# TrustworthyComputing/REDsec

Hardware: AMD Instinct MI355X
Metric: gate bootstraps/sec (N=1024) (higher is better)
Workload: dtype int32 torus; ring products in f64 (complex FFT, exact after rounding); 1 GPU; 65536 independent bootstrapped NAND gates per GPU per step, default128 (n=630 N=1024 l=3 Bgbit=7 t=8 basebit=2); gates_per_gpu=65536, total_gates=65536, params=default128, mode=fft, parallelism=gate-sharded x1

## Files before the change

### include/redsec_hip.h

```cpp
#ifndef REDSEC_HIP_H
#define REDSEC_HIP_H

#include <stddef.h>
#include <stdint.h>

#ifdef __cplusplus
extern "C" {
#endif

typedef enum rs_status {
  RS_OK = 0,
  RS_ERR_INVALID = -1,
  RS_ERR_NO_DEVICE = -2,
  RS_ERR_HIP = -3,
  RS_ERR_STATE = -4,
  RS_ERR_INEXACT = -5
} rs_status;

typedef struct rs_params {
  int32_t n;
  int32_t N;
  int32_t k;
  int32_t bk_l;
  int32_t bk_Bgbit;
// ... 49 lines not shown
int rs_pack_dev(rs_ctx* ctx, int32_t* rlwe, const int32_t* ct, size_t count,
                const int32_t* pack_key, int32_t basebit, int32_t t, void* stream);

int rs_pack_keygen_dev(rs_ctx* ctx, int32_t* body, const int32_t* lwe_key, const int32_t* tlwe_key,
                       const uint8_t* mask_seed, const uint8_t* noise_seed, int32_t basebit, int32_t t, double stdev);
int rs_pack_expand_dev(rs_ctx* ctx, int32_t* pack_key, const uint8_t* mask_seed, const int32_t* body, int32_t t, void* stream);

int rs_phase_dev(rs_ctx* ctx, int32_t* phase, const int32_t* ct, size_t B, const int32_t* key, int32_t dim);

typedef struct rs_key_audit {
  uint32_t bk_max_abs, ksk_max_abs;
  uint64_t bk_over, ksk_over;
  uint64_t ksk_zero_bad;
  uint64_t bk_words, ksk_words;
} rs_key_audit;

int rs_audit_keys_dev(rs_ctx* ctx, rs_key_audit* report, int32_t* bk_noise, int32_t* ksk_noise,
                      const int32_t* bk, const int32_t* ksk, const int32_t* lwe_key, const int32_t* tlwe_key,
                      uint32_t bk_limit, uint32_t ksk_limit);
int rs_audit_compressed_keys_dev(rs_ctx* ctx, rs_key_audit* report, int32_t* bk_noise, int32_t* ksk_noise,
                                 const uint8_t* mask_seed, const int32_t* bk_body, const int32_t* ksk_body,
                                 const int32_t* lwe_key, const int32_t* tlwe_key, uint32_t bk_limit, uint32_t ksk_limit);

typedef struct rs_pack_key_audit {
  uint32_t max_abs;
  uint64_t over;
  uint64_t words;
} rs_pack_key_audit;
int rs_audit_pack_key_dev(rs_ctx* ctx, rs_pack_key_audit* report, int32_t* noise, const int32_t* key, const uint8_t* mask_seed,
                          const int32_t* lwe_key, const int32_t* tlwe_key, int32_t basebit, int32_t t, uint32_t limit);

enum { RS_MODE_EXACT_NTT = 0, RS_MODE_FFT = 1, RS_MODE_FFT_SPLIT = 2 };
int rs_set_mode(rs_ctx* ctx, int mode);
int rs_get_mode(rs_ctx* ctx, int* mode);
int rs_split_bound(rs_ctx* ctx, double* bound);
#define RS_CERTIFICATE_LIMIT 0.25
int rs_set_certificate_limit(rs_ctx* ctx, double limit);
int rs_certify(rs_ctx* ctx, void* stream, double* max_distance, int64_t* recomputed_calls, int reset);
int rs_rounding_certificate(rs_ctx* ctx, double* max_distance, int reset);
int rs_fft_fallbacks(rs_ctx* ctx, int64_t* count);

int rs_reserve(rs_ctx* ctx, size_t max_batch);
int rs_reserve_stream(rs_ctx* ctx, size_t max_batch, void* stream);

int rs_bootstrap_dev(rs_ctx* ctx, int32_t* out, const int32_t* in, int32_t mu, size_t B, void* stream);
int rs_bootstrap(rs_ctx* ctx, int32_t* out, const int32_t* in, int32_t mu, size_t B);

int rs_bootstrap_sparse_dev(rs_ctx* ctx, int32_t* out, const int32_t* in, int32_t mu, size_t B, const int32_t* live, size_t n_live,
                            void* stream);

int rs_bootstrap_lut_dev(rs_ctx* ctx, int32_t* out, const int32_t* in, const int32_t* lut, size_t lut_count, size_t lut_first,
                         size_t B, void* stream);

int rs_gate_dev(rs_ctx* ctx, rs_gate_op op, int32_t* out, const int32_t* a, const int32_t* b, size_t B, void* stream);
int rs_gate(rs_ctx* ctx, rs_gate_op op, int32_t* out, const int32_t* a, const int32_t* b, size_t B);

int rs_gate_mu_dev(rs_ctx* ctx, rs_gate_op op, int32_t* out, const int32_t* a, const int32_t* b, int32_t mu, size_t B, void* stream);

typedef enum rs_row_op {
  RS_ROW_MAJ3  = 10,
  RS_ROW_XOR3  = 11,
  RS_ROW_MAJ3N = 12
} rs_row_op;
typedef struct rs_row_group { int32_t op; int32_t reserved; uint64_t count; } rs_row_group;

int rs_gate3_dev(rs_ctx* ctx, int op, int32_t* out, const int32_t* a, const int32_t* b, const int32_t* c, size_t B, void* stream);

int rs_gate_rows_dev(rs_ctx* ctx, int32_t* out, const int32_t* in, size_t in_rows, const int32_t* idx, const rs_row_group* groups,
                     int n_groups, int32_t mu, size_t B, void* stream);

typedef enum rs_cell_op { RS_CELL_MUX = 13 } rs_cell_op;
typedef struct rs_cell { int32_t src[3]; uint8_t op; uint8_t neg; uint16_t reserved; } rs_cell;
typedef struct rs_circuit rs_circuit;
int rs_circuit_create(rs_ctx* ctx, rs_circuit** out, const rs_cell* cells, size_t n_cells, const uint32_t* level_end, size_t n_levels,
                      size_t n_inputs);
int rs_circuit_destroy(rs_ctx* ctx, rs_circuit* circuit);
int rs_circuit_run_dev(rs_ctx* ctx, const rs_circuit* circuit, int32_t* arena, size_t lanes, void* stream);

int rs_mux_dev(rs_ctx* ctx, int32_t* out, const int32_t* a, const int32_t* b, const int32_t* c, size_t B, void* stream);
int rs_mux(rs_ctx* ctx, int32_t* out, const int32_t* a, const int32_t* b, const int32_t* c, size_t B);

int rs_bootstrap_wo_ks_dev(rs_ctx* ctx, int32_t* u, const int32_t* in, int32_t mu, size_t B, void* stream);
int rs_keyswitch_dev(rs_ctx* ctx, int32_t* out, const int32_t* u, size_t B, void* stream);

int rs_debug_polymul(rs_ctx* ctx, int32_t* out, const int32_t* a_small, const int32_t* b_torus, size_t count);
int rs_debug_cohort_table(rs_ctx* ctx, void* stream, int32_t* out);
int rs_debug_fp64_rate(rs_ctx* ctx, double* lane_ops_per_s);

int rs_linear_fc_dev(rs_ctx* ctx, int32_t* out, const int32_t* in, const uint8_t* sign, const uint8_t* zero,
                     int32_t K, int32_t M, int32_t zero_tap_b, const int32_t* bias_b, int32_t bias_depth,
                     void* stream);

typedef struct rs_conv_shape {
  int32_t H, Wd, Cin, Cout, fh, fw, stride_h, stride_w, off_h, off_w, Ho, Wo;
} rs_conv_shape;
int rs_conv_ternary_dev(rs_ctx* ctx, int32_t* out, const int32_t* in, const uint8_t* sign, const uint8_t* zero,
                        const rs_conv_shape* shape, int32_t zero_tap_b, int32_t pad_tap_b,
                        const int32_t* bias_b, int32_t bias_depth, void* stream);

typedef struct rs_pool_shape {
  int32_t H, Wd, C, win_h, win_w, stride_h, stride_w, off_h, off_w, Ho, Wo;
} rs_pool_shape;
int rs_sumpool_dev(rs_ctx* ctx, int32_t* out, const int32_t* in, const rs_pool_shape* shape,
                   const int32_t* bias_b, int32_t bias_depth, void* stream);

int rs_lincomb_dev(rs_ctx* ctx, int32_t* out, const int32_t* a, int32_t ca, const int32_t* b, int32_t cb,
                   int32_t bconst, size_t B, void* stream);

int rs_gather_rows_dev(rs_ctx* ctx, int32_t* out, const int32_t* in, const int32_t* row_index, size_t B, void* stream);

int rs_dev_alloc(rs_ctx* ctx, void** ptr, size_t bytes);
int rs_dev_free(rs_ctx* ctx, void* ptr);
int rs_copy_to_dev(rs_ctx* ctx, void* dst_dev, const void* src_host, size_t bytes);
int rs_copy_to_host(rs_ctx* ctx, void* dst_host, const void* src_dev, size_t bytes);
int rs_copy_dev_to_dev(rs_ctx* dst_ctx, void* dst_dev, rs_ctx* src_ctx, const void* src_dev, size_t bytes);
int rs_allgather_rows(rs_ctx* const* ctxs, int n_ctx, int32_t* const* bufs, size_t rows, size_t row_words);
int rs_sync(rs_ctx* ctx);
int rs_release_stream(rs_ctx* ctx, void* stream);

int rs_set_timing(rs_ctx* ctx, int enable);
int rs_last_kernel_ms(rs_ctx* ctx, float* blind_rotate_ms, float* keyswitch_ms);
int rs_last_kernel_ms_stream(rs_ctx* ctx, void* stream, float* blind_rotate_ms, float* keyswitch_ms);

int rs_last_launch(rs_ctx* ctx, void* stream, int32_t* form, int32_t* waves_per_block, int64_t* resident);
int rs_last_keyswitch(rs_ctx* ctx, void* stream, int32_t* form, int32_t* slices);
int rs_info(rs_ctx* ctx, int64_t* bk_device_bytes, int64_t* ksk_device_bytes, int32_t* waves_per_block,
            int32_t* num_cus);

#ifdef __cplusplus
}
#endif
#endif
```

### redsec_amd/backend.py

```python
import ctypes as C
import os

import numpy as np

from . import build as _build

_i32p = C.POINTER(C.c_int32)
_u8p = C.POINTER(C.c_uint8)

ABI_SYMBOLS = [
    "rs_last_error", "rs_version", "rs_params_default128", "rs_params_redsec_small_v2", "rs_create", "rs_destroy",
    "rs_load_keys", "rs_reserve", "rs_bootstrap_dev", "rs_bootstrap", "rs_gate_dev", "rs_gate", "rs_mux_dev", "rs_mux",
    "rs_gate_mu_dev", "rs_gather_rows_dev", "rs_bootstrap_wo_ks_dev", "rs_keyswitch_dev", "rs_debug_polymul", "rs_debug_cohort_table", "rs_debug_fp64_rate", "rs_linear_fc_dev", "rs_conv_ternary_dev",
    "rs_sumpool_dev", "rs_lincomb_dev", "rs_dev_alloc", "rs_dev_free", "rs_copy_to_dev", "rs_copy_to_host", "rs_sync",
    "rs_set_timing", "rs_last_kernel_ms", "rs_info", "rs_set_mode", "rs_get_mode", "rs_rounding_certificate", "rs_fft_fallbacks",
    "rs_bootstrap_lut_dev", "rs_set_certificate_limit", "rs_certify", "rs_reserve_stream", "rs_last_kernel_ms_stream", "rs_last_launch", "rs_last_keyswitch", "rs_copy_dev_to_dev",
    "rs_params_redsec_small", "rs_params_redsec_medium", "rs_params_redsec_large", "rs_split_bound",
    "rs_allgather_rows", "rs_release_stream", "rs_load_synthetic_keys", "rs_keygen_dev", "rs_load_keys_dev",
    "rs_keygen_compressed_dev", "rs_expand_keys_dev", "rs_load_compressed_keys", "rs_load_compressed_keys_dev",
    "rs_encrypt_seeded_dev", "rs_expand_ciphertexts_dev", "rs_pk_encrypt_dev", "rs_rlwe_pk_encrypt_dev", "rs_rlwe_extract_dev", "rs_pack_dev",
    "rs_pack_keygen_dev", "rs_pack_expand_dev", "rs_audit_pack_key_dev",
    "rs_phase_dev", "rs_audit_keys_dev", "rs_audit_compressed_keys_dev",
    "rs_gate3_dev", "rs_gate_rows_dev",
    "rs_circuit_create", "rs_circuit_destroy", "rs_circuit_run_dev",
    "rs_bootstrap_sparse_dev",
]

GATES = {"NAND": 0, "OR": 1, "AND": 2, "NOR": 3, "XOR": 4, "XNOR": 5, "ANDNY": 6, "ANDYN": 7, "ORNY": 8, "ORYN": 9}

ROW_OPS = dict(GATES, MAJ3=10, XOR3=11, MAJ3N=12)

CELL_OPS = dict(ROW_OPS, MUX=13)


class RedsecHipError(RuntimeError):
    pass


class RsParams(C.Structure):
    _fields_ = [("n", C.c_int32), ("N", C.c_int32), ("k", C.c_int32), ("bk_l", C.c_int32), ("bk_Bgbit", C.c_int32),
                ("ks_t", C.c_int32), ("ks_basebit", C.c_int32)]


class RsConvShape(C.Structure):
    _fields_ = [(f, C.c_int32) for f in
                ("H", "Wd", "Cin", "Cout", "fh", "fw", "stride_h", "stride_w", "off_h", "off_w", "Ho", "Wo")]


class RsPoolShape(C.Structure):
    _fields_ = [(f, C.c_int32) for f in
                ("H", "Wd", "C", "win_h", "win_w", "stride_h", "stride_w", "off_h", "off_w", "Ho", "Wo")]


class RsKeyAudit(C.Structure):
    _fields_ = [("bk_max_abs", C.c_uint32), ("ksk_max_abs", C.c_uint32), ("bk_over", C.c_uint64), ("ksk_over", C.c_uint64),
                ("ksk_zero_bad", C.c_uint64), ("bk_words", C.c_uint64), ("ksk_words", C.c_uint64)]


class RsPackKeyAudit(C.Structure):
    _fields_ = [("max_abs", C.c_uint32), ("over", C.c_uint64), ("words", C.c_uint64)]


class RsRowGroup(C.Structure):
    _fields_ = [("op", C.c_int32), ("reserved", C.c_int32), ("count", C.c_uint64)]


class RsCell(C.Structure):
    _fields_ = [("src", C.c_int32 * 3), ("op", C.c_uint8), ("neg", C.c_uint8), ("reserved", C.c_uint16)]


CELL_DTYPE = np.dtype([("src", np.int32, (3,)), ("op", np.uint8), ("neg", np.uint8), ("reserved", np.uint16)])

_lib = None


def load_library(path=None):
    global _lib
    if _lib is not None and path is None:
        return _lib
    path = path or os.environ.get("REDSEC_HIP_LIB")
    so = path or _build.build_hip()
    try:
        import torch
        if torch.cuda.is_available():
            torch.cuda.init()
    except ImportError:
        pass
    if not os.path.exists(so):
        raise RedsecHipError("libredsec_hip.so is missing: run `python -m redsec_amd.build`")
    try:
        L = C.CDLL(so)
    except OSError as e:
        raise RedsecHipError("cannot load %s: %s" % (so, e))
    L.rs_last_error.restype = C.c_char_p
    L.rs_version.restype = C.c_char_p
    P = C.POINTER(RsParams)
    vp = C.c_void_p
    L.rs_params_default128.argtypes = [P]
    L.rs_params_redsec_small_v2.argtypes = [P]
    L.rs_params_redsec_small.argtypes = [P]
    L.rs_params_redsec_medium.argtypes = [P]
    L.rs_params_redsec_large.argtypes = [P]
    L.rs_split_bound.argtypes = [vp, C.POINTER(C.c_double)]
    L.rs_create.argtypes = [C.POINTER(vp), P, C.c_int]
    L.rs_destroy.argtypes = [vp]
    L.rs_load_keys.argtypes = [vp, _i32p, _i32p]
    L.rs_load_synthetic_keys.argtypes = [vp, C.c_uint64]
    L.rs_load_keys_dev.argtypes = [vp, vp, vp]
    L.rs_keygen_dev.argtypes = [vp, vp, vp, _i32p, _i32p, C.c_char_p, C.c_double, C.c_double]
    L.rs_keygen_compressed_dev.argtypes = [vp, vp, vp, _i32p, _i32p, C.c_char_p, C.c_char_p, C.c_double, C.c_double]
    L.rs_expand_keys_dev.argtypes = [vp, vp, vp, C.c_char_p, vp, vp]
    L.rs_load_compressed_keys.argtypes = [vp, C.c_char_p, _i32p, _i32p]
    L.rs_load_compressed_keys_dev.argtypes = [vp, C.c_char_p, vp, vp]
    L.rs_encrypt_seeded_dev.argtypes = [vp, vp, vp, vp, C.c_size_t, _i32p, C.c_char_p, C.c_char_p, C.c_uint64, C.c_double]
    L.rs_expand_ciphertexts_dev.argtypes = [vp, vp, C.c_char_p, C.c_uint64, vp, C.c_size_t, vp]
    L.rs_pk_encrypt_dev.argtypes = [vp, vp, vp, C.c_size_t, vp, vp, C.c_size_t, C.c_char_p, C.c_uint64, vp]
    L.rs_rlwe_pk_encrypt_dev.argtypes = [vp, vp, vp, vp, C.c_size_t, C.c_char_p, C.c_uint64, C.c_double, vp]
    L.rs_rlwe_extract_dev.argtypes = [vp, vp, vp, C.c_size_t, vp]
    L.rs_pack_dev.argtypes = [vp, vp, vp, C.c_size_t, vp, C.c_int32, C.c_int32, vp]
    L.rs_pack_keygen_dev.argtypes = [vp, vp, _i32p, _i32p, C.c_char_p, C.c_char_p, C.c_int32, C.c_int32, C.c_double]
    L.rs_pack_expand_dev.argtypes = [vp, vp, C.c_char_p, vp, C.c_int32, vp]
    L.rs_audit_pack_key_dev.argtypes = [vp, C.POINTER(RsPackKeyAudit), vp, vp, C.c_char_p, _i32p, _i32p, C.c_int32, C.c_int32, C.c_uint32]
    L.rs_phase_dev.argtypes = [vp, vp, vp, C.c_size_t, _i32p, C.c_int32]
    L.rs_audit_keys_dev.argtypes = [vp, C.POINTER(RsKeyAudit), vp, vp, vp, vp, _i32p, _i32p, C.c_uint32, C.c_uint32]
    L.rs_audit_compressed_keys_dev.argtypes = [vp, C.POINTER(RsKeyAudit), vp, vp, C.c_char_p, vp, vp, _i32p, _i32p, C.c_uint32, C.c_uint32]
    L.rs_reserve.argtypes = [vp, C.c_size_t]
    L.rs_bootstrap_dev.argtypes = [vp, vp, vp, C.c_int32, C.c_size_t, vp]
    L.rs_bootstrap.argtypes = [vp, _i32p, _i32p, C.c_int32, C.c_size_t]
    L.rs_bootstrap_sparse_dev.argtypes = [vp, vp, vp, C.c_int32, C.c_size_t, vp, C.c_size_t, vp]
    L.rs_gate_dev.argtypes = [vp, C.c_int, vp, vp, vp, C.c_size_t, vp]
    L.rs_gate.argtypes = [vp, C.c_int, _i32p, _i32p, _i32p, C.c_size_t]
    L.rs_gate_mu_dev.argtypes = [vp, C.c_int, vp, vp, vp, C.c_int32, C.c_size_t, vp]
    L.rs_gather_rows_dev.argtypes = [vp, vp, vp, vp, C.c_size_t, vp]
    L.rs_gate3_dev.argtypes = [vp, C.c_int, vp, vp, vp, vp, C.c_size_t, vp]
    L.rs_gate_rows_dev.argtypes = [vp, vp, vp, C.c_size_t, vp, C.POINTER(RsRowGroup), C.c_int, C.c_int32, C.c_size_t, vp]
    L.rs_circuit_create.argtypes = [vp, C.POINTER(vp), vp, C.c_size_t, C.POINTER(C.c_uint32), C.c_size_t, C.c_size_t]
    L.rs_circuit_destroy.argtypes = [vp, vp]
    L.rs_circuit_run_dev.argtypes = [vp, vp, vp, C.c_size_t, vp]
    L.rs_mux_dev.argtypes = [vp, vp, vp, vp, vp, C.c_size_t, vp]
    L.rs_mux.argtypes = [vp, _i32p, _i32p, _i32p, _i32p, C.c_size_t]
    L.rs_bootstrap_wo_ks_dev.argtypes = [vp, vp, vp, C.c_int32, C.c_size_t, vp]
    L.rs_keyswitch_dev.argtypes = [vp, vp, vp, C.c_size_t, vp]
    L.rs_debug_polymul.argtypes = [vp, _i32p, _i32p, _i32p, C.c_size_t]
    L.rs_debug_cohort_table.argtypes = [vp, vp, _i32p]
    L.rs_debug_fp64_rate.argtypes = [vp, C.POINTER(C.c_double)]
    L.rs_linear_fc_dev.argtypes = [vp, vp, vp, vp, vp, C.c_int32, C.c_int32, C.c_int32, vp, C.c_int32, vp]
    L.rs_conv_ternary_dev.argtypes = [vp, vp, vp, vp, vp, C.POINTER(RsConvShape), C.c_int32, C.c_int32, vp, C.c_int32, vp]
    L.rs_sumpool_dev.argtypes = [vp, vp, vp, C.POINTER(RsPoolShape), vp, C.c_int32, vp]
    L.rs_lincomb_dev.argtypes = [vp, vp, vp, C.c_int32, vp, C.c_int32, C.c_int32, C.c_size_t, vp]
    L.rs_dev_alloc.argtypes = [vp, C.POINTER(vp), C.c_size_t]
    L.rs_dev_free.argtypes = [vp, vp]
    L.rs_copy_to_dev.argtypes = [vp, vp, vp, C.c_size_t]
    L.rs_copy_to_host.argtypes = [vp, vp, vp, C.c_size_t]
    L.rs_sync.argtypes = [vp]
    L.rs_set_timing.argtypes = [vp, C.c_int]
    L.rs_last_kernel_ms.argtypes = [vp, C.POINTER(C.c_float), C.POINTER(C.c_float)]
    L.rs_info.argtypes = [vp, C.POINTER(C.c_int64), C.POINTER(C.c_int64), C.POINTER(C.c_int32), C.POINTER(C.c_int32)]
    L.rs_set_mode.argtypes = [vp, C.c_int]
    L.rs_get_mode.argtypes = [vp, C.POINTER(C.c_int)]
    L.rs_rounding_certificate.argtypes = [vp, C.POINTER(C.c_double), C.c_int]
    L.rs_fft_fallbacks.argtypes = [vp, C.POINTER(C.c_int64)]
    L.rs_bootstrap_lut_dev.argtypes = [vp, vp, vp, vp, C.c_size_t, C.c_size_t, C.c_size_t, vp]
    L.rs_copy_dev_to_dev.argtypes = [vp, vp, vp, vp, C.c_size_t]
    L.rs_allgather_rows.argtypes = [C.POINTER(vp), C.c_int, C.POINTER(vp), C.c_size_t, C.c_size_t]
    L.rs_release_stream.argtypes = [vp, vp]
    L.rs_set_certificate_limit.argtypes = [vp, C.c_double]
    L.rs_certify.argtypes = [vp, vp, C.POINTER(C.c_double), C.POINTER(C.c_int64), C.c_int]
    L.rs_reserve_stream.argtypes = [vp, C.c_size_t, vp]
    L.rs_last_kernel_ms_stream.argtypes = [vp, vp, C.POINTER(C.c_float), C.POINTER(C.c_float)]
    L.rs_last_launch.argtypes = [vp, vp, C.POINTER(C.c_int32), C.POINTER(C.c_int32), C.POINTER(C.c_int64)]
    L.rs_last_keyswitch.argtypes = [vp, vp, C.POINTER(C.c_int32), C.POINTER(C.c_int32)]
    if path is None:
        _lib = L
    return L


def _check(L, rc):
    if rc != 0:
        raise RedsecHipError("redsec_hip error %d: %s" % (rc, (L.rs_last_error() or b"").decode()))


def params(name, n=None):
    L = load_library()
    p = RsParams()
    if name == "default128":
        _check(L, L.rs_params_default128(C.byref(p)))
    elif name == "redsec_small_v2":
        _check(L, L.rs_params_redsec_small_v2(C.byref(p)))
    elif name in ("redsec_small", "redsec_medium", "redsec_large"):
        _check(L, getattr(L, "rs_params_" + name)(C.byref(p)))
    else:
        raise KeyError(name)
    if n is not None:
        p.n = int(n)
    return p


def _np_i32(a):
    a = np.ascontiguousarray(a, dtype=np.int32)
    return a, a.ctypes.data_as(_i32p)


class Backend:

    def __init__(self, p, device=0):
        try:
            import torch
            if torch.cuda.is_available():
                torch.cuda.init()
        except ImportError:
            pass
        self.L = load_library()
        self.p = p
        self.W = p.n + 1
        self.device = device
        h = C.c_void_p()
        _check(self.L, self.L.rs_create(C.byref(h), C.byref(p), device))
        self.h = h

    @property
    def closed(self):
        return not getattr(self, "h", None)

    def close(self, check=None):
        if getattr(self, "h", None):
            h, self.h = self.h, None
            rc = self.L.rs_destroy(h)
            if check is None:
                import sys
                check = sys.exc_info()[0] is None
            if check:
                _check(self.L, rc)
            elif rc != 0:
                import warnings
                warnings.warn("rs_destroy reported error %d while another error was being handled: %s"
                              % (rc, (self.L.rs_last_error() or b"").decode()), RuntimeWarning, stacklevel=2)

    def __del__(self):
        try:
            self.close(check=False)
        except Exception:
            pass

    def load_keys(self, bk, ksk):
        bk, pbk = _np_i32(bk)
        ksk, pksk = _np_i32(ksk)
        p = self.p
        assert bk.size == p.n * 2 * p.bk_l * 2 * p.N, "bk has the wrong size"
        assert ksk.size == p.N * p.ks_t * (1 << p.ks_basebit) * (p.n + 1), "ksk has the wrong size"
        _check(self.L, self.L.rs_load_keys(self.h, pbk, pksk))

    def _key_sizes(self):
        p = self.p
        return p.n * 2 * p.bk_l * 2 * p.N, p.N * p.ks_t * (1 << p.ks_basebit) * (p.n + 1)
# ... 299 lines not shown
    def bootstrap_lut(self, x, lut, out=None, first=0):
        B = x.shape[0]
        out = self.empty(B, self.W) if out is None else out
        _check(self.L, self.L.rs_bootstrap_lut_dev(self.h, self._ck_dev(out, self.W), self._ck_dev(x, self.W),
                                                    self._ck_dev(lut, self.p.N), lut.shape[0], int(first), B, self._stream()))
        return out

    def gate(self, op, a, b, out=None):
        B = a.shape[0]
        out = self.empty(B, self.W) if out is None else out
        _check(self.L, self.L.rs_gate_dev(self.h, GATES[op], self._ck_dev(out, self.W), self._ck_dev(a, self.W),
                                           self._ck_dev(b, self.W), B, self._stream()))
        return out

    def gate_mu(self, op, a, b, mu, out=None):
        B = a.shape[0]
        out = self.empty(B, self.W) if out is None else out
        _check(self.L, self.L.rs_gate_mu_dev(self.h, GATES[op], self._ck_dev(out, self.W), self._ck_dev(a, self.W),
                                              self._ck_dev(b, self.W), int(mu), B, self._stream()))
        return out

    def gather_rows(self, x, index):
        B = index.numel()
        out = self.empty(B, self.W)
        _check(self.L, self.L.rs_gather_rows_dev(self.h, self._ck_dev(out), self._ck_dev(x, self.W), C.c_void_p(index.data_ptr()), B,
                                                  self._stream()))
        return out

    def gate3(self, op, a, b, c, out=None):
        B = a.shape[0]
        out = self.empty(B, self.W) if out is None else out
        _check(self.L, self.L.rs_gate3_dev(self.h, ROW_OPS[op] if isinstance(op, str) else int(op), self._ck_dev(out, self.W),
                                            self._ck_dev(a, self.W), self._ck_dev(b, self.W), self._ck_dev(c, self.W), B, self._stream()))
        return out

    def gate_rows(self, inp, idx, groups, mu=None, out=None):
        B = idx.numel() // 3
        assert idx.numel() == 3 * B, "idx must hold [B][3] indices"
        in_rows = inp.numel() // self.W
        out = self.empty(B, self.W) if out is None else out
        assert out.numel() == B * self.W, "out must hold [B][n+1] words"
        gs = (RsRowGroup * max(1, len(groups)))()
        for g, (op, count) in zip(gs, groups):
            g.op, g.reserved, g.count = (ROW_OPS[op] if isinstance(op, str) else int(op)), 0, int(count)
        _check(self.L, self.L.rs_gate_rows_dev(self.h, self._ck_dev(out, self.W), self._ck_dev(inp, self.W), in_rows, self._ck_dev(idx),
                                                gs, len(groups), (1 << 29) if mu is None else int(mu), B, self._stream()))
        return out

    def circuit_create(self, table, level_end, n_inputs):
        table = np.ascontiguousarray(table, dtype=CELL_DTYPE)
        level_end = np.ascontiguousarray(level_end, dtype=np.uint32)
        h = C.c_void_p()
        _check(self.L, self.L.rs_circuit_create(self.h, C.byref(h), table.ctypes.data_as(C.c_void_p), len(table),
                                                 level_end.ctypes.data_as(C.POINTER(C.c_uint32)), len(level_end), int(n_inputs)))
        return h

    def circuit_destroy(self, handle):
        _check(self.L, self.L.rs_circuit_destroy(self.h, handle))

    def circuit_run(self, handle, arena, lanes):
        assert arena.numel() % (self.W * max(1, int(lanes))) == 0, "arena must hold [wires][lanes][n+1] words"
        _check(self.L, self.L.rs_circuit_run_dev(self.h, handle, self._ck_dev(arena, self.W), int(lanes), self._stream()))
        return arena

    def mux(self, a, b, c, out=None):
        B = a.shape[0]
        out = self.empty(B, self.W) if out is None else out
        _check(self.L, self.L.rs_mux_dev(self.h, self._ck_dev(out, self.W), self._ck_dev(a, self.W), self._ck_dev(b, self.W),
                                          self._ck_dev(c, self.W), B, self._stream()))
        return out

    def bootstrap_wo_ks(self, x, mu):
        B = x.shape[0]
        u = self.empty(B, self.p.N + 1)
        _check(self.L, self.L.rs_bootstrap_wo_ks_dev(self.h, self._ck_dev(u), self._ck_dev(x, self.W), int(mu), B, self._stream()))
        return u

    def keyswitch(self, u):
        B = u.shape[0]
        out = self.empty(B, self.W)
        _check(self.L, self.L.rs_keyswitch_dev(self.h, self._ck_dev(out), self._ck_dev(u, self.p.N + 1), B, self._stream()))
        return out

    def lincomb(self, a, ca, b=None, cb=0, bconst=0):
        B = a.numel() // self.W
        out = self.empty(*a.shape)
        pb = self._ck_dev(b, self.W) if b is not None else None
        _check(self.L, self.L.rs_lincomb_dev(self.h, self._ck_dev(out), self._ck_dev(a, self.W), int(ca), pb, int(cb),
                                              int(bconst), B, self._stream()))
        return out

    def _u8(self, t):
        import torch
        if t is None:
            return None
        assert t.is_cuda and t.dtype == torch.uint8 and t.is_contiguous()
        return C.c_void_p(t.data_ptr())

    def linear_fc(self, x, sign, zero=None, zero_tap_b=0, bias_b=None):
        K = x.shape[0]
        M = sign.shape[1]
        out = self.empty(M, self.W)
        pbias = self._ck_dev(bias_b) if bias_b is not None else None
        depth = int(bias_b.numel()) if bias_b is not None else 0
        _check(self.L, self.L.rs_linear_fc_dev(self.h, self._ck_dev(out), self._ck_dev(x, self.W), self._u8(sign), self._u8(zero),
                                                K, M, int(zero_tap_b), pbias, depth, self._stream()))
        return out

    def conv_ternary(self, x, sign, zero, shape, zero_tap_b=0, pad_tap_b=0, bias_b=None):
        s = RsConvShape(**shape)
        out = self.empty(s.Ho, s.Wo, s.Cout, self.W)
        pbias = self._ck_dev(bias_b) if bias_b is not None else None
        depth = int(bias_b.numel()) if bias_b is not None else 0
        _check(self.L, self.L.rs_conv_ternary_dev(self.h, self._ck_dev(out), self._ck_dev(x, self.W), self._u8(sign),
                                                   self._u8(zero), C.byref(s), int(zero_tap_b), int(pad_tap_b), pbias, depth,
                                                   self._stream()))
        return out

    def sumpool(self, x, shape, bias_b=None):
        s = RsPoolShape(**shape)
        out = self.empty(s.Ho, s.Wo, s.C, self.W)
        pbias = self._ck_dev(bias_b) if bias_b is not None else None
        depth = int(bias_b.numel()) if bias_b is not None else 0
        _check(self.L, self.L.rs_sumpool_dev(self.h, self._ck_dev(out), self._ck_dev(x, self.W), C.byref(s), pbias, depth,
                                              self._stream()))
        return out

    def bootstrap_host(self, x, mu):
        x, px = _np_i32(x)
        out = np.empty_like(x)
        _check(self.L, self.L.rs_bootstrap(self.h, out.ctypes.data_as(_i32p), px, int(mu), x.shape[0]))
        return out

    def gate_host(self, op, a, b):
        a, pa = _np_i32(a)
        b, pb = _np_i32(b)
        out = np.empty_like(a)
        _check(self.L, self.L.rs_gate(self.h, GATES[op], out.ctypes.data_as(_i32p), pa, pb, a.shape[0]))
        return out

    def mux_host(self, a, b, c):
        a, pa = _np_i32(a)
        b, pb = _np_i32(b)
        c, pc = _np_i32(c)
        out = np.empty_like(a)
        _check(self.L, self.L.rs_mux(self.h, out.ctypes.data_as(_i32p), pa, pb, pc, a.shape[0]))
        return out

    def polymul_host(self, a_small, b_torus):
        a, pa = _np_i32(a_small)
        b, pb = _np_i32(b_torus)
        out = np.empty_like(b)
        _check(self.L, self.L.rs_debug_polymul(self.h, out.ctypes.data_as(_i32p), pa, pb, a.size // self.p.N))
        return out

    def set_mode(self, mode):
        _check(self.L, self.L.rs_set_mode(self.h, {"exact": 0, "ntt": 0, "fft": 1, "split": 2}[mode]))

    def mode(self):
        m = C.c_int()
        _check(self.L, self.L.rs_get_mode(self.h, C.byref(m)))
        return {0: "exact", 1: "fft", 2: "split"}[m.value]

    def split_bound(self):
        d = C.c_double()
        _check(self.L, self.L.rs_split_bound(self.h, C.byref(d)))
        return d.value

    def rounding_certificate(self, reset=True):
        d = C.c_double()
        _check(self.L, self.L.rs_rounding_certificate(self.h, C.byref(d), 1 if reset else 0))
        return d.value

    def fft_fallbacks(self):
        n = C.c_int64()
        _check(self.L, self.L.rs_fft_fallbacks(self.h, C.byref(n)))
        return n.value

    def set_certificate_limit(self, limit):
        _check(self.L, self.L.rs_set_certificate_limit(self.h, float(limit)))

    def certify(self, reset=True):
        d, n = C.c_double(), C.c_int64()
        _check(self.L, self.L.rs_certify(self.h, self._stream(), C.byref(d), C.byref(n), 1 if reset else 0))
        return d.value, n.value

    def last_launch(self):
        f, w, r = C.c_int32(), C.c_int32(), C.c_int64()
        _check(self.L, self.L.rs_last_launch(self.h, self._stream(), C.byref(f), C.byref(w), C.byref(r)))
        return {"form": ["per_wave", "workgroup", "duo", "coop2", "coop4", "general", "split_workgroup", "split_coop", "split_duo", "coop8", "coop8_listed"][f.value], "waves_per_block": w.value, "resident": r.value}

    def last_keyswitch(self):
        f, n = C.c_int32(), C.c_int32()
        _check(self.L, self.L.rs_last_keyswitch(self.h, self._stream(), C.byref(f), C.byref(n)))
        return {"form": ["gather", "tiled", "sliced", "wide"][f.value], "slices": n.value}

    def fp64_rate(self):
        v = C.c_double()
        _check(self.L, self.L.rs_debug_fp64_rate(self.h, C.byref(v)))
        return v.value

    def cohort_table(self):
        out = np.empty((8, 64), dtype=np.int32)
        _check(self.L, self.L.rs_debug_cohort_table(self.h, self._stream(), out.ctypes.data_as(_i32p)))
        return out

    def set_timing(self, on=True):
        _check(self.L, self.L.rs_set_timing(self.h, 1 if on else 0))

    def last_kernel_ms(self):
        a, b = C.c_float(), C.c_float()
        _check(self.L, self.L.rs_last_kernel_ms_stream(self.h, self._stream(), C.byref(a), C.byref(b)))
        return a.value, b.value

    def info(self):
        bk, ksk, wpb, cus = C.c_int64(), C.c_int64(), C.c_int32(), C.c_int32()
        _check(self.L, self.L.rs_info(self.h, C.byref(bk), C.byref(ksk), C.byref(wpb), C.byref(cus)))
        return {"bk_device_bytes": bk.value, "ksk_device_bytes": ksk.value, "waves_per_block": wpb.value, "num_cus": cus.value}

    def sync(self):
        _check(self.L, self.L.rs_sync(self.h))
```

### redsec_amd/build.py

```python
import os
import shutil
import subprocess

HERE = os.path.dirname(os.path.abspath(__file__))
ROOT = os.path.dirname(HERE)
CSRC = os.path.join(HERE, "csrc")
INCLUDE = os.path.join(ROOT, "include")

HIP_LIB = os.path.join(HERE, "libredsec_hip.so")
EMU_LIB = os.path.join(HERE, "librs_emulate.so")

HIP_SOURCES = ["rs_bootstrap.hip", "rs_bootstrap_split.hip", "rs_bootstrap_listed.hip", "rs_general.hip", "rs_kernels.hip", "rs_keyswitch_wide.hip", "rs_seeded.hip", "rs_pubkey.hip", "rs_rlwe.hip", "rs_pack.hip", "rs_packkey.hip", "rs_audit.hip", "rs_rows.hip", "rs_circuit.hip", "rs_sparse.hip", "rs_api.cpp"]
HIP_DEPS = HIP_SOURCES + ["rs_bootstrap.h", "rs_kernels.h", "rs_cohort.h", "rs_diag.h", "rs_launch_plan.h", "rs_lds_plan.h", "rs_ntt.h", "rs_fft.h", "rs_general.h", "rs_keygen.h", "rs_rlwe.h", "rs_pack.h", "rs_packkey.h", "rs_audit.h", "rs_rows.h", "rs_circuit.h", "rs_sparse.h", "rs_host.h", os.path.join(INCLUDE, "redsec_hip.h")]
HIP_COMMON_FLAGS = ["-O3", "--offload-arch=gfx950", "-std=c++17", "-ffp-contract=off", "-fPIC"]
HIP_OBJECTS = [
    ("rs_bootstrap", "rs_bootstrap.hip", ["-mllvm", "-enable-post-misched=0"]),
    ("rs_bootstrap_split", "rs_bootstrap_split.hip", ["-mllvm", "-amdgpu-sched-strategy=max-memory-clause"]),
    ("rs_bootstrap_listed", "rs_bootstrap_listed.hip", ["-mllvm", "-enable-post-misched=0"]),
    ("rs_general", "rs_general.hip", []),
    ("rs_kernels", "rs_kernels.hip", []),
    ("rs_keyswitch_wide", "rs_keyswitch_wide.hip", []),
    ("rs_seeded", "rs_seeded.hip", []),
    ("rs_pubkey", "rs_pubkey.hip", []),
    ("rs_rlwe", "rs_rlwe.hip", []),
    ("rs_pack", "rs_pack.hip", []),
    ("rs_packkey", "rs_packkey.hip", []),
    ("rs_audit", "rs_audit.hip", []),
    ("rs_rows", "rs_rows.hip", []),
    ("rs_circuit", "rs_circuit.hip", []),
    ("rs_sparse", "rs_sparse.hip", []),
    ("rs_api", "rs_api.cpp", []),
]
EMU_SOURCES = ["rs_emulate.cpp"]
EMU_DEPS = EMU_SOURCES + ["rs_launch_plan.h", "rs_lds_plan.h", "rs_ntt.h", "rs_fft.h", "rs_general.h", "rs_keygen.h", "rs_rlwe.h", "rs_pack.h", "rs_packkey.h", "rs_audit.h", "rs_rows.h", "rs_circuit.h", "rs_sparse.h", "rs_host.h"]


def _abs(paths):
    return [p if os.path.isabs(p) else os.path.join(CSRC, p) for p in paths]


def fingerprint(paths, extra=""):
    import hashlib
    h = hashlib.sha256(extra.encode())
    for p in paths:
        h.update(os.path.basename(p).encode() + b"\0")
        with open(p, "rb") as f:
            h.update(f.read())
    return h.hexdigest()


def is_stale(target, deps, extra=""):
    stamp = target + ".stamp"
    if not (os.path.exists(target) and os.path.exists(stamp)):
        return True
    try:
        return open(stamp).read().strip() != fingerprint(deps, extra)
    except OSError:
        return True


def write_stamp(target, deps, extra=""):
    with open(target + ".stamp", "w") as f:
        f.write(fingerprint(deps, extra) + "\n")


def _stale(target, deps):
    return is_stale(target, _abs(deps) + [os.path.abspath(__file__)])



def find_hipcc():
    for cand in (shutil.which("hipcc"), "/opt/rocm/bin/hipcc"):
        if cand and os.path.exists(cand):
            return cand
    return None


def _locked(name):
    import fcntl
    os.makedirs(os.path.join(ROOT, "build"), exist_ok=True)
    f = open(os.path.join(ROOT, "build", "." + name + ".lock"), "w")
    fcntl.flock(f, fcntl.LOCK_EX)
    return f


def _publish(tmp, target, deps):
    write_stamp(tmp, _abs(deps) + [os.path.abspath(__file__)])
    os.replace(tmp, target)
    os.replace(tmp + ".stamp", target + ".stamp")


def _recipe(src_root):
    path = os.path.join(src_root, "redsec_amd", "build.py")
    if os.path.realpath(path) == os.path.realpath(__file__):
        return HIP_COMMON_FLAGS, HIP_OBJECTS
    import importlib.util
    spec = importlib.util.spec_from_file_location("_redsec_build_recipe", path)
    other = importlib.util.module_from_spec(spec)
    spec.loader.exec_module(other)
    return getattr(other, "HIP_COMMON_FLAGS", HIP_COMMON_FLAGS), other.HIP_OBJECTS


def object_flags(name, src_root=ROOT):
    common, objects = _recipe(src_root)
    for obj, _, extra in objects:
        if obj == name:
            return common + ["-I" + os.path.join(src_root, "include"), "-I" + os.path.join(src_root, "redsec_amd", "csrc")] + extra
    raise KeyError("no object %r in HIP_OBJECTS (%s)" % (name, ", ".join(o[0] for o in objects)))


def build_tree(src_root, out, extra=(), per_object=None, verbose=False):
    hipcc = find_hipcc()
    if hipcc is None:
        raise RuntimeError("hipcc not found")
    per_object = per_object or {}
    _, objects = _recipe(src_root)
    unknown = set(per_object) - {o[0] for o in objects}
# ... 137 lines not shown
```

### redsec_amd/csrc/rs_api.cpp

```cpp
#include "redsec_hip.h"

#include <hip/hip_runtime.h>

#include <algorithm>
#include <cstdarg>
#include <cstdio>
#include <cstdlib>
#include <cstring>
#include <atomic>
#include <climits>
#include <map>
#include <memory>
#include <mutex>
#include <new>
#include <set>
#include <string>
#include <vector>

#include "rs_circuit.h"
#include "rs_diag.h"
#include "rs_host.h"
#include "rs_general.h"
#include "rs_kernels.h"
#include "rs_keygen.h"
#include "rs_pack.h"
#include "rs_packkey.h"
#include "rs_rlwe.h"
#include "rs_sparse.h"

namespace {

thread_local std::string g_err;

int fail(int code, const char* fmt, ...) {
  char buf[512];
  va_list ap;
  va_start(ap, fmt);
  vsnprintf(buf, sizeof buf, fmt, ap);
  va_end(ap);
  g_err = buf;
  return code;
}

#define RS_HIP(call)                                                                              \
  do {                                                                                            \
    hipError_t e_ = (call);                                                                       \
    if (e_ != hipSuccess) return fail(RS_ERR_HIP, "%s failed: %s", #call, hipGetErrorString(e_)); \
  } while (0)

}

constexpr unsigned kCertSlots = 1024;
struct Lane {
  hipStream_t stream = nullptr;
  int32_t* d_u0 = nullptr;
  int32_t* d_u1 = nullptr;
  size_t ws_batch = 0;
  size_t sample_words = rs::kN + 1;
  unsigned int* d_counter = nullptr;
  unsigned long long* d_cert = nullptr;
  unsigned slot_next = 0;
  uint32_t* d_conv_scratch = nullptr;
  size_t conv_scratch_words = 0;
  uint32_t* d_ks_scratch = nullptr;
  size_t ks_scratch_words = 0;
  int* d_progress = nullptr;
  int32_t* d_rows = nullptr;
  size_t rows_batch = 0;
  hipEvent_t ev[3] = {nullptr, nullptr, nullptr};
  bool ev_valid = false;
  rs::LaunchInfo last;
  rs::KsPlan last_ks; bool ks_ran = false;
  unsigned long long* h_split_max = nullptr;
};

struct rs_circuit {
  rs::Cell* d_cells = nullptr;
  std::vector<uint32_t> level_end, level_mux;
  size_t n_cells = 0, n_inputs = 0;
  size_t widest = 0;
};

struct rs_ctx {
  rs_params p{};
  int device = 0;
  int cfg = 0;
  rs::Tables tables;
  int mode = 1;
  double cert_limit = RS_CERTIFICATE_LIMIT;
  rs::LaunchOpts opts;
  int ks_force = rs::kKsAuto;
  double* d_tw = nullptr;
  double* d_tw_fft = nullptr;
  double* d_bk_ntt = nullptr;
  double* d_bk_fft = nullptr;
  bool general = false;
  int wgs_cfg = -1;
  int logn = 10;
  double split_bound = 0.0;
  double split_cert_limit = 0.25;
  std::atomic<bool> inexact{false};
  double* d_tw_gen = nullptr;
  double* d_bk_gen = nullptr;
  int32_t* d_ksk = nullptr;
  size_t bk_bytes = 0, ksk_bytes = 0;
  bool keys = false;
  int num_cus = 256;
  bool timing = false;
  std::mutex lanes_mu;
  std::map<hipStream_t, std::unique_ptr<Lane>> lanes;
  std::mutex host_mu;
  int32_t* d_io[4] = {nullptr, nullptr, nullptr, nullptr};
  size_t io_batch = 0;
  hipStream_t copy_stream = nullptr;
  hipEvent_t ev_slice = nullptr, ev_copied = nullptr, ev_staged = nullptr;
  bool copied_recorded = false;
  std::vector<int> peers_enabled, peers_denied;
  int32_t* h_stage = nullptr;
  size_t h_stage_bytes = 0;
  std::mutex circuits_mu;
  std::set<rs_circuit*> circuits;
};

namespace {

struct GateCoef { int32_t bconst, sa, sb; };

bool gate_coef(rs_gate_op op, GateCoef* g) {
  const int32_t e8 = 1 << 29, e4 = 1 << 30;
  switch (op) {
    case RS_NAND:  *g = {e8, -1, -1}; return true;
    case RS_OR:    *g = {e8, 1, 1}; return true;
    case RS_AND:   *g = {-e8, 1, 1}; return true;
    case RS_NOR:   *g = {-e8, -1, -1}; return true;
    case RS_XOR:   *g = {e4, 2, 2}; return true;
    case RS_XNOR:  *g = {-e4, -2, -2}; return true;
    case RS_ANDNY: *g = {-e8, -1, 1}; return true;
    case RS_ANDYN: *g = {-e8, 1, -1}; return true;
    case RS_ORNY:  *g = {e8, -1, 1}; return true;
    case RS_ORYN:  *g = {e8, 1, -1}; return true;
  }
  return false;
}

int use_device(rs_ctx* c) {
  if (!c) return fail(RS_ERR_INVALID, "null context");
  RS_HIP(hipSetDevice(c->device));
  return RS_OK;
}

void free_lane(Lane* ln) {
  if (ln->h_split_max) (void)hipHostFree(ln->h_split_max);
  (void)hipFree(ln->d_u0); (void)hipFree(ln->d_u1); (void)hipFree(ln->d_counter); (void)hipFree(ln->d_cert);
  (void)hipFree(ln->d_conv_scratch); (void)hipFree(ln->d_ks_scratch); (void)hipFree(ln->d_progress);
  (void)hipFree(ln->d_rows);
  for (auto& e : ln->ev) if (e) (void)hipEventDestroy(e);
}

int lane_of(rs_ctx* c, hipStream_t st, Lane** out) {
  std::lock_guard<std::mutex> g(c->lanes_mu);
  auto it = c->lanes.find(st);
  if (it != c->lanes.end()) { *out = it->second.get(); return RS_OK; }
  std::unique_ptr<Lane> ln(new Lane);
  ln->stream = st;
  ln->sample_words = (size_t)c->p.N + 1;
  const size_t cert_bytes = sizeof(unsigned long long) * (kCertSlots + 2);
  if (hipMalloc(&ln->d_cert, cert_bytes) != hipSuccess || hipMemset(ln->d_cert, 0, cert_bytes) != hipSuccess ||
      hipHostMalloc((void**)&ln->h_split_max, sizeof(unsigned long long), hipHostMallocDefault) != hipSuccess ||
      (!c->opts.no_persist && hipMalloc(&ln->d_counter, 256) != hipSuccess)) {
    free_lane(ln.get());
    return fail(RS_ERR_HIP, "per-stream state allocation failed");
  }
  *ln->h_split_max = 0;
  for (auto& e : ln->ev) (void)hipEventCreate(&e);
  *out = ln.get();
  c->lanes[st] = std::move(ln);
  return RS_OK;
}

int ensure_ws(Lane* ln, size_t B) {
  if (B <= ln->ws_batch) return RS_OK;
  if (ln->d_u0) { (void)hipFree(ln->d_u0); ln->d_u0 = nullptr; }
  if (ln->d_u1) { (void)hipFree(ln->d_u1); ln->d_u1 = nullptr; }
  ln->ws_batch = 0;
  const size_t bytes = B * ln->sample_words * sizeof(int32_t);
  RS_HIP(hipMalloc(&ln->d_u0, bytes));
  RS_HIP(hipMalloc(&ln->d_u1, bytes));
  ln->ws_batch = B;
  return RS_OK;
}

int ensure_rows(Lane* ln, size_t B, size_t W) {
  if (B <= ln->rows_batch) return RS_OK;
  if (ln->d_rows) { (void)hipFree(ln->d_rows); ln->d_rows = nullptr; }
  ln->rows_batch = 0;
  RS_HIP(hipMalloc(&ln->d_rows, B * W * sizeof(int32_t)));
  ln->rows_batch = B;
  return RS_OK;
}

void attach_ks_scratch(const rs_ctx* c, Lane* ln, rs::KeyswitchArgs& k) {
  const size_t need = rs::keyswitch_scratch_words(k);
  if (need == 0 || c->opts.ks_atomics) return;
  if (need > ln->ks_scratch_words) {
    if (ln->d_ks_scratch) { (void)hipFree(ln->d_ks_scratch); ln->d_ks_scratch = nullptr; ln->ks_scratch_words = 0; }
    if (hipMalloc(&ln->d_ks_scratch, need * sizeof(uint32_t)) != hipSuccess) { (void)hipGetLastError(); ln->d_ks_scratch = nullptr; return; }
    ln->ks_scratch_words = need;
  }
  k.scratch = ln->d_ks_scratch;
  k.scratch_words = ln->ks_scratch_words;
}

int* lane_progress(Lane* ln) {
  if (!ln->d_progress) {
    if (hipMalloc(&ln->d_progress, 8 * rs::kCohortSlots * sizeof(int)) != hipSuccess ||
        hipMemset(ln->d_progress, 0x7f, 8 * rs::kCohortSlots * sizeof(int)) != hipSuccess) {
      (void)hipGetLastError();
      if (ln->d_progress) (void)hipFree(ln->d_progress);
      ln->d_progress = nullptr;
    }
  }
  return ln->d_progress;
}

int ensure_io(rs_ctx* c, size_t B) {
  if (B <= c->io_batch) return RS_OK;
  for (auto& p : c->d_io) { if (p) { (void)hipFree(p); p = nullptr; } }
  c->io_batch = 0;
  const size_t bytes = B * (size_t)(c->p.n + 1) * sizeof(int32_t);
  for (auto& p : c->d_io) RS_HIP(hipMalloc(&p, bytes));
  c->io_batch = B;
  return RS_OK;
}

int ready(rs_ctx* c) {
  int rc = use_device(c);
  if (rc) return rc;
  if (!c->keys) return fail(RS_ERR_STATE, "rs_load_keys has not been called");
  return RS_OK;
}

bool split_distance_ok(const rs_ctx* c, unsigned long long bits) {
  if (rs::diag::kWrongOnPurpose) return true;
  double d;
  memcpy(&d, &bits, sizeof d);
  return d < c->split_cert_limit;
}
int inexact_error(rs_ctx* c) {
  return fail(RS_ERR_INEXACT, "split-key mode: a rounding distance of 1/4 or more was observed (a-priori bound %.3g): results of this context are not certified; "
                              "rs_certify(reset = 1) clears the flag", c->split_bound);
}

int split_check_lane(rs_ctx* c, Lane* ln) {
  if (c->mode != RS_MODE_FFT_SPLIT) return RS_OK;
  if (!split_distance_ok(c, *(volatile unsigned long long*)ln->h_split_max)) c->inexact.store(true);
  return c->inexact.load() ? inexact_error(c) : RS_OK;
}

struct Combo { const int32_t* in0; const int32_t* in1; int32_t c0, c1, bconst; int32_t* u; };

struct Lut { const int32_t* table = nullptr; size_t count = 0, first = 0; };

rs::BlindRotateArgs br_args(rs_ctx* c, Lane* ln, int mode, const Combo& x, int32_t mu, const Lut& lut, size_t B) {
  rs::BlindRotateArgs a;
  a.in0 = x.in0; a.in1 = x.in1; a.c0 = x.c0; a.c1 = x.c1; a.bconst = x.bconst; a.mu = mu;
  a.bk_x = mode == 1 ? c->d_bk_fft : c->d_bk_ntt;
  a.tw = mode == 1 ? c->d_tw_fft : c->d_tw;
  a.f = c->tables.f;
  a.n = c->p.n; a.W = c->p.n + 1; a.B = (long)B; a.u_out = x.u;
  a.counter = ln->d_counter;
  a.dev_flag = nullptr;
  a.lut = lut.table; a.lut_count = (int32_t)lut.count; a.lut_first = (int32_t)lut.first;
  return a;
}

int rotate_rows(rs_ctx* c, hipStream_t st, Lane* ln, const Combo* combos, int count, int32_t mu, const Lut& lut, size_t B) {
  const int mode = c->mode;
  Combo cs[2];
  for (int k = 0; k < count; ++k) { cs[k] = combos[k]; cs[k].u = k == 0 ? ln->d_u0 : ln->d_u1; }
  if (c->timing) RS_HIP(hipEventRecord(ln->ev[0], st));
  if (mode == RS_MODE_FFT_SPLIT) {
    if (!split_distance_ok(c, *(volatile unsigned long long*)ln->h_split_max)) c->inexact.store(true);
    if (c->inexact.load()) return inexact_error(c);
    bool split_wg = false;
    for (int k = 0; k < count; ++k) {
      if (c->wgs_cfg >= 0 && !c->opts.no_wg) {
        rs::BlindRotateArgs w = br_args(c, ln, 1, cs[k], mu, lut, B);
        w.bk_x = c->d_bk_gen; w.tw = c->d_tw_fft;
        w.progress = lane_progress(ln);
        const hipError_t e = rs::launch_blind_rotate_split_wg(c->wgs_cfg, w, c->num_cus, c->opts, st, &ln->last);
        if (e == hipSuccess) { split_wg = true; continue; }
        if (e != hipErrorNotSupported) return fail(RS_ERR_HIP, "split workgroup launch failed: %s", hipGetErrorString(e));
      }
      rs::GenArgs a;
      a.in0 = cs[k].in0; a.in1 = cs[k].in1; a.c0 = cs[k].c0; a.c1 = cs[k].c1; a.bconst = cs[k].bconst; a.mu = mu;
      a.bk_x = c->d_bk_gen; a.tw = c->d_tw_gen;
      a.n = c->p.n; a.W = c->p.n + 1; a.l = c->p.bk_l; a.bgbit = c->p.bk_Bgbit; a.B = (long)B; a.u_out = cs[k].u;
      a.lut = lut.table; a.lut_count = (int32_t)lut.count; a.lut_first = (int32_t)lut.first;
      a.dev_flag = ln->d_cert + kCertSlots;
      RS_HIP(rs::launch_gen_blind_rotate(c->logn, a, c->num_cus, st));
    }
    if (!split_wg) RS_HIP(hipMemcpyAsync(ln->h_split_max, ln->d_cert + kCertSlots, sizeof(unsigned long long), hipMemcpyDeviceToHost, st));
    if (!split_wg) {
      ln->last.form = rs::kFormGeneral; ln->last.waves_per_block = (c->p.N / 16) / 64;
      ln->last.resident = std::min<long>((long)B, rs::gen_resident_ciphertexts(c->logn, c->num_cus));
    }
  } else if (mode == RS_MODE_FFT) {
    unsigned long long* slot = ln->d_cert + (ln->slot_next++ % kCertSlots);
    RS_HIP(hipMemsetAsync(slot, 0, sizeof *slot, st));
    for (int k = 0; k < count; ++k) {
      rs::BlindRotateArgs a = br_args(c, ln, 1, cs[k], mu, lut, B);
      a.dev_flag = slot;
      a.progress = lane_progress(ln);
      RS_HIP(rs::launch_blind_rotate(c->cfg, 1, a, c->num_cus, c->opts, st, &ln->last));
    }
    unsigned long long limit_bits;
    const double lim = rs::diag::kWrongOnPurpose ? 1e300 : c->cert_limit;
    memcpy(&limit_bits, &lim, sizeof limit_bits);
    for (int k = 0; k < count; ++k) {
      rs::BlindRotateArgs a = br_args(c, ln, 0, cs[k], mu, lut, B);
      a.gate_flag = slot; a.gate_limit_bits = limit_bits;
      a.running_flag = k == 0 ? ln->d_cert + kCertSlots : nullptr;
      a.fallback_count = k == 0 ? ln->d_cert + kCertSlots + 1 : nullptr;
      RS_HIP(rs::launch_blind_rotate(c->cfg, 0, a, c->num_cus, c->opts, st, nullptr));
    }
  } else {
    for (int k = 0; k < count; ++k)
      RS_HIP(rs::launch_blind_rotate(c->cfg, 0, br_args(c, ln, 0, cs[k], mu, lut, B), c->num_cus, c->opts, st, &ln->last));
  }
  if (c->timing) RS_HIP(hipEventRecord(ln->ev[1], st));
  return RS_OK;
}

int keyswitch_rows(rs_ctx* c, hipStream_t st, Lane* ln, int32_t* out, int count, int32_t ks_bconst, size_t B) {
  rs::KeyswitchArgs k;
  k.u0 = ln->d_u0; k.u1 = count == 2 ? ln->d_u1 : nullptr; k.bconst = ks_bconst; k.ksk = c->d_ksk;
  k.W = c->p.n + 1; k.t = c->p.ks_t; k.basebit = c->p.ks_basebit; k.B = (long)B; k.out = out; k.N = c->p.N;
  attach_ks_scratch(c, ln, k);
  RS_HIP(rs::launch_keyswitch(k, st, c->num_cus, c->ks_force, &ln->last_ks));
  ln->ks_ran = true;
  return RS_OK;
}

int finish_timing(rs_ctx* c, hipStream_t st, Lane* ln) {
  if (c->timing) { RS_HIP(hipEventRecord(ln->ev[2], st)); ln->ev_valid = true; }
  return RS_OK;
}

int run_bootstrap(rs_ctx* c, hipStream_t st, int32_t* out, const Combo* combos, int count, int32_t ks_bconst, int32_t mu,
                  const Lut& lut, size_t B) {
  Lane* ln = nullptr;
  int rc = lane_of(c, st, &ln);
  if (rc) return rc;
  rc = ensure_ws(ln, B);
  if (rc) return rc;
  rc = rotate_rows(c, st, ln, combos, count, mu, lut, B);
  if (rc) return rc;
  if (out) {
    rc = keyswitch_rows(c, st, ln, out, count, ks_bconst, B);
    if (rc) return rc;
  }
  return finish_timing(c, st, ln);
}

void destroy_ctx(rs_ctx* c) {
  (void)hipFree(c->d_tw); (void)hipFree(c->d_tw_fft); (void)hipFree(c->d_bk_ntt); (void)hipFree(c->d_bk_fft); (void)hipFree(c->d_ksk);
  (void)hipFree(c->d_tw_gen); (void)hipFree(c->d_bk_gen);
  for (auto& kv : c->lanes) free_lane(kv.second.get());
  for (rs_circuit* q : c->circuits) { (void)hipFree(q->d_cells); delete q; }
  for (auto& p : c->d_io) (void)hipFree(p);
  if (c->ev_slice) (void)hipEventDestroy(c->ev_slice);
  if (c->ev_copied) (void)hipEventDestroy(c->ev_copied);
  if (c->ev_staged) (void)hipEventDestroy(c->ev_staged);
  if (c->h_stage) (void)hipHostFree(c->h_stage);
  if (c->copy_stream) (void)hipStreamDestroy(c->copy_stream);
  delete c;
}

bool env_on(const char* name) { const char* v = getenv(name); return v && *v && strcmp(v, "0") != 0; }

int pack_key_bits(const int32_t* key, int count, std::vector<uint32_t>& bits) {
  const size_t base = bits.size();
  bits.resize(base + (size_t)(count + 31) / 32, 0u);
  for (int i = 0; i < count; ++i) {
    if (key[i] != 0 && key[i] != 1) return i;
    bits[base + ((size_t)i >> 5)] |= (uint32_t)key[i] << (i & 31);
  }
  return -1;
}

template <class Run>
int with_secret_copy(std::vector<uint32_t>& words, size_t extra, Run run) {
  const size_t key_bytes = (words.size() * sizeof(uint32_t) + 15) & ~(size_t)15, bytes = key_bytes + extra;
  char* d = nullptr;
  auto body = [&]() -> int {
    RS_HIP(hipMalloc(&d, bytes));
    RS_HIP(hipMemset(d, 0, bytes));
    RS_HIP(hipMemcpy(d, words.data(), words.size() * sizeof(uint32_t), hipMemcpyHostToDevice));
    return run(reinterpret_cast<const uint32_t*>(d), d + key_bytes);
  };
  const int rc = body();
  std::fill(words.begin(), words.end(), 0u);
  if (!d) return rc;
  (void)hipDeviceSynchronize();
  const hipError_t ez = hipMemset(d, 0, bytes);
  const hipError_t es = hipDeviceSynchronize();
  (void)hipFree(d);
  if (rc != RS_OK) return rc;
  if (ez != hipSuccess || es != hipSuccess) return fail(RS_ERR_HIP, "clearing the device copy of the secret key failed");
  return RS_OK;
}

}

extern "C" {

const char* rs_last_error(void) { return g_err.c_str(); }
const char* rs_version(void) { return "redsec_hip 0.4 (gfx950; fp64 fft with on-device exact recomputation + exact fp64-carried ntt + split-key fft, N up to 8192)"; }

int rs_params_default128(rs_params* p) {
  if (!p) return fail(RS_ERR_INVALID, "null params");
  *p = {630, 1024, 1, 3, 7, 8, 2};
  return RS_OK;
}
int rs_params_redsec_small_v2(rs_params* p) {
  if (!p) return fail(RS_ERR_INVALID, "null params");
  *p = {350, 1024, 1, 10, 3, 9, 3};
  return RS_OK;
}

int rs_params_redsec_small(rs_params* p) {
  if (!p) return fail(RS_ERR_INVALID, "null params");
  *p = {500, 1024, 1, 3, 10, 18, 1};
  return RS_OK;
}
int rs_params_redsec_medium(rs_params* p) {
  if (!p) return fail(RS_ERR_INVALID, "null params");
// ... 4 lines not shown
  if (!p) return fail(RS_ERR_INVALID, "null params");
  *p = {6144, 8192, 1, 3, 10, 18, 1};
  return RS_OK;
}

int rs_create(rs_ctx** out, const rs_params* p, int device) {
  if (!out || !p) return fail(RS_ERR_INVALID, "null argument");
  *out = nullptr;
  int logn = 0;
  while ((1 << logn) < p->N) ++logn;
  if (p->k != 1 || (1 << logn) != p->N || logn < rs::kGenMinLogN || logn > rs::kGenMaxLogN)
    return fail(RS_ERR_INVALID, "unsupported ring: N=%d k=%d (need k=1 and N in {1024, 2048, 4096, 8192})", p->N, p->k);
  if (p->n < 1 || p->n > 16384) return fail(RS_ERR_INVALID, "unsupported LWE dimension n=%d", p->n);
  if (p->ks_t < 1 || p->ks_basebit < 1 || p->ks_t * p->ks_basebit > 31) return fail(RS_ERR_INVALID, "bad keyswitch parameters");
  if (p->bk_l < 1 || p->bk_Bgbit < 1 || p->bk_l * p->bk_Bgbit > 32) return fail(RS_ERR_INVALID, "bad gadget l=%d Bgbit=%d", p->bk_l, p->bk_Bgbit);
  rs::PrimeSpec ps{};
  const bool special = p->N == rs::kN && rs::prime_for(p->bk_l, p->bk_Bgbit, &ps);
  const double split_bound = rs::gen_error_bound(logn, p->bk_l, p->bk_Bgbit);
  if (!special && !(split_bound < rs::kSplitBoundOffer))
    return fail(RS_ERR_INVALID, "gadget l=%d Bgbit=%d on N=%d: split-key product bound %.3g is not below 1/2", p->bk_l, p->bk_Bgbit, p->N, split_bound);
  int count = 0;
  if (hipGetDeviceCount(&count) != hipSuccess || count <= 0) return fail(RS_ERR_NO_DEVICE, "no HIP device visible");
  if (device < 0 || device >= count) return fail(RS_ERR_NO_DEVICE, "device %d out of range (%d visible)", device, count);
  rs_ctx* c = new (std::nothrow) rs_ctx();
  if (!c) return fail(RS_ERR_INVALID, "out of host memory");
  c->p = *p;
  c->device = device;
  c->general = !special;
  c->logn = logn;
  c->split_bound = split_bound;
  c->cfg = special ? ((p->bk_l == 3) ? 0 : 1) : -1;
  if (special) {
    const unsigned fwd_mask = c->cfg == 0 ? rs::CfgDefault128::FWD_MASK : rs::CfgRedsecV2::FWD_MASK;
    const unsigned inv_mask = c->cfg == 0 ? rs::CfgDefault128::INV_MASK : rs::CfgRedsecV2::INV_MASK;
    const int fuse = c->cfg == 0 ? rs::CfgDefault128::FUSE : rs::CfgRedsecV2::FUSE;
    const bool mid = c->cfg == 0 ? rs::CfgDefault128::MID_REDUCE : rs::CfgRedsecV2::MID_REDUCE;
    c->tables = rs::make_tables(ps, fuse);
    const std::string why = rs::validate_schedule(c->tables.f.p, p->bk_l, p->bk_Bgbit, fwd_mask, inv_mask, fuse, mid);
    if (!why.empty()) { destroy_ctx(c); return fail(RS_ERR_INVALID, "transform schedule not exact: %s", why.c_str()); }
  } else {
    c->mode = RS_MODE_FFT_SPLIT;
  }
  if (hipSetDevice(device) != hipSuccess) { destroy_ctx(c); return fail(RS_ERR_NO_DEVICE, "hipSetDevice(%d) failed", device); }
  hipDeviceProp_t prop;
  if (hipGetDeviceProperties(&prop, device) == hipSuccess) {
    c->num_cus = prop.multiProcessorCount;
    if (!strstr(prop.gcnArchName, "gfx950")) {
      destroy_ctx(c);
      return fail(RS_ERR_NO_DEVICE, "device %d is %s; this library ships gfx950 code only", device, prop.gcnArchName);
    }
  }
  if (special) {
    if (hipMalloc(&c->d_tw, sizeof(double) * rs::kTwTotal) != hipSuccess ||
        hipMemcpy(c->d_tw, c->tables.tw.data(), sizeof(double) * rs::kTwTotal, hipMemcpyHostToDevice) != hipSuccess) {
      destroy_ctx(c);
      return fail(RS_ERR_HIP, "twiddle table upload failed");
    }
  }
  c->wgs_cfg = special ? c->cfg : ((p->N == rs::kN && p->bk_l == 3 && p->bk_Bgbit == 10) ? 2 : -1);
  if (special || c->wgs_cfg >= 0) {
    const std::vector<double> fft_tw = rs::make_fft_tables();
    if (hipMalloc(&c->d_tw_fft, sizeof(double) * rs::kFftTwDoubles) != hipSuccess ||
        hipMemcpy(c->d_tw_fft, fft_tw.data(), sizeof(double) * rs::kFftTwDoubles, hipMemcpyHostToDevice) != hipSuccess) {
      destroy_ctx(c);
      return fail(RS_ERR_HIP, "twiddle table upload failed");
    }
  }
  if (split_bound < rs::kSplitBoundOffer) {
    std::vector<double> gtw((size_t)p->N);
    rs::gen_make_twiddles(logn, gtw.data());
    if (hipMalloc(&c->d_tw_gen, sizeof(double) * gtw.size()) != hipSuccess ||
        hipMemcpy(c->d_tw_gen, gtw.data(), sizeof(double) * gtw.size(), hipMemcpyHostToDevice) != hipSuccess) {
      destroy_ctx(c);
      return fail(RS_ERR_HIP, "twiddle table upload failed");
    }
  }
  if (const char* m = getenv("REDSEC_MODE")) {
    if (special) c->mode = (strcmp(m, "exact") == 0 || strcmp(m, "ntt") == 0) ? RS_MODE_EXACT_NTT : (strcmp(m, "split") == 0 && c->d_tw_gen ? RS_MODE_FFT_SPLIT : RS_MODE_FFT);
  }
  if (const char* v = getenv("REDSEC_SPLIT_CERT_LIMIT")) { const double x = atof(v); if (x > 0.0 && x < 0.25) c->split_cert_limit = x; }
  c->opts.no_coop = env_on("RS_NO_COOP"); c->opts.no_wg = env_on("RS_NO_WG"); c->opts.no_duo = env_on("RS_NO_DUO");
  c->opts.no_persist = env_on("RS_NO_PERSIST"); c->opts.no_conv_tiled = env_on("RS_NO_CONV_TILED");
  c->opts.no_wg4 = env_on("RS_NO_WG4"); c->opts.no_tail = env_on("RS_NO_TAIL"); c->opts.no_coop8 = env_on("RS_NO_COOP8"); c->opts.no_coop8_listed = env_on("RS_NO_COOP8_LISTED"); c->opts.ks_atomics = env_on("RS_KS_ATOMICS"); c->opts.force_host_staged = env_on("RS_FORCE_HOST_STAGED"); c->opts.no_cohort = env_on("RS_NO_COHORT");
  if (const char* v = getenv("RS_KS_FORM")) c->ks_force = strcmp(v, "wide") == 0 ? rs::kKsWide : strcmp(v, "tiled") == 0 ? rs::kKsTiled : rs::kKsAuto;
  Lane* ln = nullptr;
  if (lane_of(c, nullptr, &ln) != RS_OK) { destroy_ctx(c); return RS_ERR_HIP; }
  *out = c;
  return RS_OK;
}

int rs_destroy(rs_ctx* c) {
  if (!c) return RS_OK;
  (void)hipSetDevice(c->device);
  (void)hipDeviceSynchronize();
  int rc = RS_OK;
  {
    std::lock_guard<std::mutex> g(c->lanes_mu);
    for (auto& kv : c->lanes) { const int r = split_check_lane(c, kv.second.get()); if (r) rc = r; }
  }
  if (rc == RS_OK && c->inexact.load()) rc = inexact_error(c);
  destroy_ctx(c);
  return rc;
}

enum class KeySource { kHost, kDevice, kSynthetic, kCompressedHost, kCompressedDevice };

static void free_keys(rs_ctx* c) {
  c->keys = false;
  if (c->d_bk_ntt) { (void)hipFree(c->d_bk_ntt); c->d_bk_ntt = nullptr; }
  if (c->d_bk_fft) { (void)hipFree(c->d_bk_fft); c->d_bk_fft = nullptr; }
  if (c->d_bk_gen) { (void)hipFree(c->d_bk_gen); c->d_bk_gen = nullptr; }
  if (c->d_ksk) { (void)hipFree(c->d_ksk); c->d_ksk = nullptr; }
  c->bk_bytes = c->ksk_bytes = 0;
}

static rs::ExpandArgs expand_args(const rs_ctx* c, const uint8_t* mask_seed) {
  rs::ExpandArgs e{};
  rs::kg_seed_words(mask_seed, e.seed);
  e.n = c->p.n; e.N = c->p.N; e.l = c->p.bk_l; e.t = c->p.ks_t; e.basebit = c->p.ks_basebit;
  return e;
}

static int load_keys_impl(rs_ctx* c, KeySource src, const int32_t* bk, const int32_t* ksk, uint64_t seed,
                          const uint8_t* mask_seed = nullptr) {
  int rc = use_device(c);
  if (rc) return rc;
  if (src != KeySource::kSynthetic && (!bk || !ksk)) return fail(RS_ERR_INVALID, "null key pointer");
  const bool compressed = src == KeySource::kCompressedHost || src == KeySource::kCompressedDevice;
  if (compressed && !mask_seed) return fail(RS_ERR_INVALID, "null mask seed");
  const rs_params& p = c->p;
  const size_t n_polys = (size_t)p.n * (size_t)(2 * p.bk_l) * 2;
  const size_t bk_words = n_polys * (size_t)p.N;
  const size_t ksk_samples = (size_t)p.N * p.ks_t * ((size_t)1 << p.ks_basebit);
  const size_t ksk_words = ksk_samples * (size_t)(p.n + 1);
  free_keys(c);
  int32_t* d_bk = nullptr;
  int32_t* d_body = nullptr;
  auto body = [&]() -> int {
    RS_HIP(hipMalloc(&d_bk, bk_words * sizeof(int32_t)));
    if (src == KeySource::kSynthetic) RS_HIP(rs::launch_synthetic_words(d_bk, seed, bk_words, nullptr));
    else if (compressed) {
      const int32_t* bk_body = bk;
      if (src == KeySource::kCompressedHost) {
        RS_HIP(hipMalloc(&d_body, bk_words / 2 * sizeof(int32_t)));
        RS_HIP(hipMemcpy(d_body, bk, bk_words / 2 * sizeof(int32_t), hipMemcpyHostToDevice));
        bk_body = d_body;
      }
      rs::ExpandArgs e = expand_args(c, mask_seed);
      e.bk = d_bk; e.bk_body = bk_body;
      RS_HIP(rs::launch_expand_bk(c->logn, e, c->num_cus, nullptr));
      RS_HIP(hipDeviceSynchronize());
      if (d_body) { RS_HIP(hipFree(d_body)); d_body = nullptr; }
    } else RS_HIP(hipMemcpy(d_bk, bk, bk_words * sizeof(int32_t), src == KeySource::kHost ? hipMemcpyHostToDevice : hipMemcpyDeviceToDevice));
    if (!c->general) {
      RS_HIP(hipMalloc(&c->d_bk_ntt, bk_words * sizeof(double)));
      RS_HIP(hipMalloc(&c->d_bk_fft, bk_words * sizeof(double)));
      RS_HIP(rs::launch_bk_transform(c->cfg, 0, d_bk, c->d_bk_ntt, c->d_tw, c->tables.f, c->tables.ninv, (long)n_polys, nullptr));
      RS_HIP(rs::launch_bk_transform(c->cfg, 1, d_bk, c->d_bk_fft, c->d_tw_fft, c->tables.f, 0.0, (long)n_polys, nullptr));
      c->bk_bytes = bk_words * sizeof(double);
    }
    if (c->d_tw_gen) {
      RS_HIP(hipMalloc(&c->d_bk_gen, 2 * bk_words * sizeof(double)));
      RS_HIP(rs::launch_gen_bk_transform(c->logn, d_bk, c->d_bk_gen, c->d_tw_gen, (long)n_polys, c->num_cus, nullptr));
      if (c->general) c->bk_bytes = 2 * bk_words * sizeof(double);
    }
    RS_HIP(hipDeviceSynchronize());
    RS_HIP(hipFree(d_bk));
    d_bk = nullptr;
    RS_HIP(hipMalloc(&c->d_ksk, ksk_words * sizeof(int32_t)));
    if (src == KeySource::kSynthetic) { RS_HIP(rs::launch_synthetic_words(c->d_ksk, seed ^ 0x6b73ull, ksk_words, nullptr)); RS_HIP(hipDeviceSynchronize()); }
    else if (src == KeySource::kHost) RS_HIP(hipMemcpy(c->d_ksk, ksk, ksk_words * sizeof(int32_t), hipMemcpyHostToDevice));
    else if (src == KeySource::kDevice) { RS_HIP(hipMemcpy(c->d_ksk, ksk, ksk_words * sizeof(int32_t), hipMemcpyDeviceToDevice)); RS_HIP(hipDeviceSynchronize()); }
    else {
      const int32_t* ksk_body = ksk;
      if (src == KeySource::kCompressedHost) {
        RS_HIP(hipMalloc(&d_body, ksk_samples * sizeof(int32_t)));
        RS_HIP(hipMemcpy(d_body, ksk, ksk_samples * sizeof(int32_t), hipMemcpyHostToDevice));
        ksk_body = d_body;
      }
      rs::ExpandArgs e = expand_args(c, mask_seed);
      e.ksk = c->d_ksk; e.ksk_body = ksk_body;
      RS_HIP(rs::launch_expand_ksk(e, c->num_cus, nullptr));
      RS_HIP(hipDeviceSynchronize());
      if (d_body) { RS_HIP(hipFree(d_body)); d_body = nullptr; }
    }
    c->ksk_bytes = ksk_words * sizeof(int32_t);
    return RS_OK;
  };
  rc = body();
  if (rc != RS_OK) {
    (void)hipDeviceSynchronize();
    if (d_bk) (void)hipFree(d_bk);
    if (d_body) (void)hipFree(d_body);
    free_keys(c);
    return rc;
  }
  c->keys = true;
  return RS_OK;
}

int rs_load_keys(rs_ctx* c, const int32_t* bk, const int32_t* ksk) {
  if (!bk || !ksk) return fail(RS_ERR_INVALID, "null key pointer");
  return load_keys_impl(c, KeySource::kHost, bk, ksk, 0);
}
int rs_load_keys_dev(rs_ctx* c, const int32_t* bk, const int32_t* ksk) {
  if (!bk || !ksk) return fail(RS_ERR_INVALID, "null key pointer");
  return load_keys_impl(c, KeySource::kDevice, bk, ksk, 0);
}
int rs_load_synthetic_keys(rs_ctx* c, uint64_t seed) { return load_keys_impl(c, KeySource::kSynthetic, nullptr, nullptr, seed); }
static int load_compressed(rs_ctx* c, KeySource src, const uint8_t* mask_seed, const int32_t* bk_body, const int32_t* ksk_body) {
  int rc = use_device(c);
  if (rc) return rc;
  if (!mask_seed || !bk_body || !ksk_body) { free_keys(c); return fail(RS_ERR_INVALID, "null pointer"); }
  return load_keys_impl(c, src, bk_body, ksk_body, 0, mask_seed);
}
int rs_load_compressed_keys(rs_ctx* c, const uint8_t* mask_seed, const int32_t* bk_body, const int32_t* ksk_body) {
  return load_compressed(c, KeySource::kCompressedHost, mask_seed, bk_body, ksk_body);
}
int rs_load_compressed_keys_dev(rs_ctx* c, const uint8_t* mask_seed, const int32_t* bk_body, const int32_t* ksk_body) {
  return load_compressed(c, KeySource::kCompressedDevice, mask_seed, bk_body, ksk_body);
}

static int keygen_impl(rs_ctx* c, int32_t* bk, int32_t* ksk, const int32_t* lwe_key, const int32_t* tlwe_key, const uint8_t* seed,
                       const uint8_t* noise_seed, double bk_stdev, double ks_stdev) {
  int rc = use_device(c);
  if (rc) return rc;
  const bool compressed = noise_seed != nullptr;
  if (!bk || !ksk || !lwe_key || !tlwe_key || !seed) return fail(RS_ERR_INVALID, "null pointer");
  if (((uintptr_t)bk & 15u) != 0) return fail(RS_ERR_INVALID, "bk must be 16-byte aligned");
  if (compressed && memcmp(seed, noise_seed, 32) == 0)
    return fail(RS_ERR_INVALID, "mask seed and noise seed are equal: the public mask seed would reveal the noise");
  if (!(std::isfinite(bk_stdev) && bk_stdev >= 0.0) || !(std::isfinite(ks_stdev) && ks_stdev >= 0.0))
    return fail(RS_ERR_INVALID, "noise deviations must be finite and non-negative (bk %g, ks %g)", bk_stdev, ks_stdev);
  if (!c->d_tw_gen) return fail(RS_ERR_INVALID, "split-key product not offered for this set: a-priori bound %.3g", c->split_bound);
  const rs_params& p = c->p;
  for (int i = 0; i < p.n; ++i)
    if (lwe_key[i] != 0 && lwe_key[i] != 1) return fail(RS_ERR_INVALID, "lwe_key[%d] = %d is not 0 or 1", i, lwe_key[i]);
  for (int i = 0; i < p.N; ++i)
    if (tlwe_key[i] != 0 && tlwe_key[i] != 1) return fail(RS_ERR_INVALID, "tlwe_key[%d] = %d is not 0 or 1", i, tlwe_key[i]);
  const size_t key_bytes = ((size_t)(p.n + p.N) * sizeof(int32_t) + 15) & ~(size_t)15;
  const size_t bytes = key_bytes + sizeof(unsigned long long);
  char* d_sec = nullptr;
  RS_HIP(hipMalloc(&d_sec, bytes));
  rs::KeygenArgs a{};
  a.bk = bk; a.ksk = ksk;
  a.lwe_key = reinterpret_cast<const int32_t*>(d_sec);
  a.tlwe_key = a.lwe_key + p.n;
  rs::kg_seed_words(seed, a.seed);
  if (compressed) rs::kg_seed_words(noise_seed, a.noise_seed);
  a.compressed = compressed ? 1 : 0;
  a.n = p.n; a.N = p.N; a.l = p.bk_l; a.bgbit = p.bk_Bgbit; a.t = p.ks_t; a.basebit = p.ks_basebit;
  a.bk_sigma = bk_stdev; a.ks_sigma = ks_stdev;
  a.dev_flag = reinterpret_cast<unsigned long long*>(d_sec + key_bytes);
  unsigned long long flag = 0;
  auto body = [&]() -> int {
    RS_HIP(hipMemcpy(d_sec, lwe_key, (size_t)p.n * sizeof(int32_t), hipMemcpyHostToDevice));
    RS_HIP(hipMemcpy(d_sec + (size_t)p.n * sizeof(int32_t), tlwe_key, (size_t)p.N * sizeof(int32_t), hipMemcpyHostToDevice));
    RS_HIP(hipMemset(a.dev_flag, 0, sizeof(unsigned long long)));
    RS_HIP(rs::launch_keygen_bk(c->logn, a, c->d_tw_gen, c->num_cus, nullptr));
    RS_HIP(rs::launch_keygen_ksk(a, c->num_cus, nullptr));
    RS_HIP(hipDeviceSynchronize());
    RS_HIP(hipMemcpy(&flag, a.dev_flag, sizeof flag, hipMemcpyDeviceToHost));
    return RS_OK;
  };
  rc = body();
  (void)hipDeviceSynchronize();
  const hipError_t ez = hipMemset(d_sec, 0, bytes);
  const hipError_t es = hipDeviceSynchronize();
  (void)hipFree(d_sec);
// ... 262 lines not shown
  int bad = pack_key_bits(lwe_key, p.n, bits);
  if (bad >= 0) { std::fill(bits.begin(), bits.end(), 0u); return fail(RS_ERR_INVALID, "lwe_key[%d] = %d is not 0 or 1", bad, lwe_key[bad]); }
  const size_t lwe_words = bits.size();
  bad = pack_key_bits(tlwe_key, p.N, bits);
  if (bad >= 0) { std::fill(bits.begin(), bits.end(), 0u); return fail(RS_ERR_INVALID, "tlwe_key[%d] = %d is not 0 or 1", bad, tlwe_key[bad]); }
  rs::AuditReportDev dev{};
  rc = with_secret_copy(bits, sizeof(rs::AuditReportDev), [&](const uint32_t* d_bits, char* d_report) -> int {
    RS_HIP(hipDeviceSynchronize());
    rs::AuditArgs a{};
    a.bk = bk; a.ksk = ksk; a.bk_noise = bk_noise; a.ksk_noise = ksk_noise;
    a.lwe_bits = d_bits; a.tlwe_bits = d_bits + lwe_words;
    if (compressed) rs::kg_seed_words(mask_seed, a.seed);
    a.n = p.n; a.N = p.N; a.l = p.bk_l; a.bgbit = p.bk_Bgbit; a.t = p.ks_t; a.basebit = p.ks_basebit;
    a.bk_limit = bk_limit; a.ksk_limit = ksk_limit;
    a.report = reinterpret_cast<rs::AuditReportDev*>(d_report);
    if (bk) RS_HIP(rs::launch_audit_bk(a, compressed, c->num_cus, nullptr));
    if (ksk) RS_HIP(rs::launch_audit_ksk(a, compressed, c->num_cus, nullptr));
    RS_HIP(hipDeviceSynchronize());
    RS_HIP(hipMemcpy(&dev, d_report, sizeof dev, hipMemcpyDeviceToHost));
    return RS_OK;
  });
  if (rc != RS_OK) return rc;
  report->bk_max_abs = dev.bk_max_abs; report->ksk_max_abs = dev.ksk_max_abs;
  report->bk_over = dev.bk_over; report->ksk_over = dev.ksk_over; report->ksk_zero_bad = dev.ksk_zero_bad;
  report->bk_words = bk ? (uint64_t)p.n * (uint64_t)(2 * p.bk_l) * (uint64_t)p.N : 0u;
  report->ksk_words = ksk ? (uint64_t)p.N * (uint64_t)p.ks_t * (((uint64_t)1 << p.ks_basebit) - 1u) : 0u;
  return RS_OK;
}

int rs_audit_keys_dev(rs_ctx* c, rs_key_audit* report, int32_t* bk_noise, int32_t* ksk_noise, const int32_t* bk, const int32_t* ksk,
                      const int32_t* lwe_key, const int32_t* tlwe_key, uint32_t bk_limit, uint32_t ksk_limit) {
  return audit_impl(c, report, bk_noise, ksk_noise, nullptr, false, bk, ksk, lwe_key, tlwe_key, bk_limit, ksk_limit);
}
int rs_audit_compressed_keys_dev(rs_ctx* c, rs_key_audit* report, int32_t* bk_noise, int32_t* ksk_noise, const uint8_t* mask_seed,
                                 const int32_t* bk_body, const int32_t* ksk_body, const int32_t* lwe_key, const int32_t* tlwe_key,
                                 uint32_t bk_limit, uint32_t ksk_limit) {
  return audit_impl(c, report, bk_noise, ksk_noise, mask_seed, true, bk_body, ksk_body, lwe_key, tlwe_key, bk_limit, ksk_limit);
}

int rs_audit_pack_key_dev(rs_ctx* c, rs_pack_key_audit* report, int32_t* noise, const int32_t* key, const uint8_t* mask_seed,
                          const int32_t* lwe_key, const int32_t* tlwe_key, int32_t basebit, int32_t t, uint32_t limit) {
  int rc = use_device(c);
  if (rc) return rc;
  if (!report || !key || !lwe_key || !tlwe_key) return fail(RS_ERR_INVALID, "null pointer");
  size_t rows = 0;
  rc = pack_key_shape(c, basebit, t, true, &rows);
  if (rc) return rc;
  const rs_params& p = c->p;
  std::vector<uint32_t> bits;
  int bad = pack_key_bits(lwe_key, p.n, bits);
  if (bad >= 0) { std::fill(bits.begin(), bits.end(), 0u); return fail(RS_ERR_INVALID, "lwe_key[%d] = %d is not 0 or 1", bad, lwe_key[bad]); }
  const size_t lwe_words = bits.size();
  bad = pack_key_bits(tlwe_key, p.N, bits);
  if (bad >= 0) { std::fill(bits.begin(), bits.end(), 0u); return fail(RS_ERR_INVALID, "tlwe_key[%d] = %d is not 0 or 1", bad, tlwe_key[bad]); }
  rs::AuditReportDev dev{};
  rc = with_secret_copy(bits, sizeof(rs::AuditReportDev), [&](const uint32_t* d_bits, char* d_report) -> int {
    RS_HIP(hipDeviceSynchronize());
    rs::AuditPackArgs a{};
    a.key = key; a.noise = noise;
    a.lwe_bits = d_bits; a.tlwe_bits = d_bits + lwe_words;
    if (mask_seed) rs::kg_seed_words(mask_seed, a.seed);
    a.n = p.n; a.N = p.N; a.t = t; a.basebit = basebit; a.limit = limit;
    a.report = reinterpret_cast<rs::AuditReportDev*>(d_report);
    RS_HIP(rs::launch_audit_pack(a, mask_seed != nullptr, c->num_cus, nullptr));
    RS_HIP(hipDeviceSynchronize());
    RS_HIP(hipMemcpy(&dev, d_report, sizeof dev, hipMemcpyDeviceToHost));
    return RS_OK;
  });
  if (rc != RS_OK) return rc;
  report->max_abs = dev.bk_max_abs;
  report->over = dev.bk_over;
  report->words = (uint64_t)rows * (uint64_t)p.N;
  return RS_OK;
}

int rs_reserve(rs_ctx* c, size_t max_batch) { return rs_reserve_stream(c, max_batch, nullptr); }

int rs_reserve_stream(rs_ctx* c, size_t max_batch, void* stream) {
  int rc = use_device(c);
  if (rc) return rc;
  Lane* ln = nullptr;
  rc = lane_of(c, (hipStream_t)stream, &ln);
  if (rc) return rc;
  return ensure_ws(ln, max_batch);
}

int rs_bootstrap_dev(rs_ctx* c, int32_t* out, const int32_t* in, int32_t mu, size_t B, void* stream) {
  int rc = ready(c);
  if (rc) return rc;
  if (B == 0) return RS_OK;
  if (!out || !in) return fail(RS_ERR_INVALID, "null ciphertext pointer");
  const Combo x{in, nullptr, 1, 0, 0, nullptr};
  return run_bootstrap(c, (hipStream_t)stream, out, &x, 1, 0, mu, Lut{}, B);
}

int rs_bootstrap_lut_dev(rs_ctx* c, int32_t* out, const int32_t* in, const int32_t* lut, size_t lut_count, size_t lut_first, size_t B,
                         void* stream) {
  int rc = ready(c);
  if (rc) return rc;
  if (B == 0) return RS_OK;
  if (!out || !in || !lut) return fail(RS_ERR_INVALID, "null pointer");
  if (lut_count < 1 || lut_count > 0x7fffffffu) return fail(RS_ERR_INVALID, "lut_count must be >= 1");
  const Combo x{in, nullptr, 1, 0, 0, nullptr};
  Lut l;
  l.table = lut; l.count = lut_count; l.first = lut_first % lut_count;
  return run_bootstrap(c, (hipStream_t)stream, out, &x, 1, 0, 0, l, B);
}

int rs_gate_mu_dev(rs_ctx* c, rs_gate_op op, int32_t* out, const int32_t* a, const int32_t* b, int32_t mu, size_t B, void* stream) {
  int rc = ready(c);
  if (rc) return rc;
  GateCoef g;
  if (!gate_coef(op, &g)) return fail(RS_ERR_INVALID, "unknown gate %d", (int)op);
  if (B == 0) return RS_OK;
  if (!out || !a || !b) return fail(RS_ERR_INVALID, "null ciphertext pointer");
  const Combo x{a, b, g.sa, g.sb, g.bconst, nullptr};
  return run_bootstrap(c, (hipStream_t)stream, out, &x, 1, 0, mu, Lut{}, B);
}

int rs_gate_dev(rs_ctx* c, rs_gate_op op, int32_t* out, const int32_t* a, const int32_t* b, size_t B, void* stream) {
  return rs_gate_mu_dev(c, op, out, a, b, 1 << 29, B, stream);
}

namespace {

int rows_ready(rs_ctx* c) {
  if (!c) {
    int count = 0;
    if (hipGetDeviceCount(&count) != hipSuccess || count <= 0) { (void)hipGetLastError(); return fail(RS_ERR_NO_DEVICE, "no HIP device visible"); }
  }
  return ready(c);
}

int run_gate_rows(rs_ctx* c, hipStream_t st, int32_t* out, rs::GateRowsArgs& a, int32_t mu) {
  Lane* ln = nullptr;
  int rc = lane_of(c, st, &ln);
  if (rc) return rc;
  rc = ensure_rows(ln, (size_t)a.B, (size_t)a.W);
  if (rc) return rc;
  a.out = ln->d_rows;
  RS_HIP(rs::launch_gate_rows(a, c->num_cus, st));
  const Combo x{ln->d_rows, nullptr, 1, 0, 0, nullptr};
  return run_bootstrap(c, st, out, &x, 1, 0, mu, Lut{}, (size_t)a.B);
}

}

int rs_gate_rows_dev(rs_ctx* c, int32_t* out, const int32_t* in, size_t in_rows, const int32_t* idx, const rs_row_group* groups,
                     int n_groups, int32_t mu, size_t B, void* stream) {
  int rc = rows_ready(c);
  if (rc) return rc;
  if (!groups) return fail(RS_ERR_INVALID, "null group list");
  if (n_groups < 1 || n_groups > rs::kRowMaxGroups) return fail(RS_ERR_INVALID, "n_groups %d outside 1..%d", n_groups, rs::kRowMaxGroups);
  rs::GateRowsArgs a{};
  uint64_t total = 0;
  for (int g = 0; g < n_groups; ++g) {
    rs::RowCoef unused;
    if (!rs::row_coef(groups[g].op, &unused)) return fail(RS_ERR_INVALID, "group %d: unknown row op %d", g, (int)groups[g].op);
    if (groups[g].reserved != 0) return fail(RS_ERR_INVALID, "group %d: reserved must be 0", g);
    if (groups[g].count > (uint64_t)B - total) return fail(RS_ERR_INVALID, "the group counts pass B = %zu", B);
    total += groups[g].count;
    a.groups.end[g] = (long)total;
    a.groups.op[g] = groups[g].op;
  }
  if (total != (uint64_t)B) return fail(RS_ERR_INVALID, "the group counts sum to %llu, not B = %zu", (unsigned long long)total, B);
  if (B == 0) return RS_OK;
  if (!out || !in || !idx) return fail(RS_ERR_INVALID, "null pointer");
// ... 54 lines not shown
  if (rc) return rc;
  RS_HIP(rs::launch_sparse_scatter(a, c->num_cus, st));
  return RS_OK;
}

static_assert(sizeof(rs_cell) == sizeof(rs::Cell) && offsetof(rs_cell, op) == offsetof(rs::Cell, op) && offsetof(rs_cell, neg) == offsetof(rs::Cell, neg) &&
              offsetof(rs_cell, reserved) == offsetof(rs::Cell, reserved), "rs_cell and rs::Cell are one layout");

namespace {

int circuit_ctx(rs_ctx* c) {
  if (!c) {
    int count = 0;
    if (hipGetDeviceCount(&count) != hipSuccess || count <= 0) { (void)hipGetLastError(); return fail(RS_ERR_NO_DEVICE, "no HIP device visible"); }
  }
  return use_device(c);
}

bool circuit_alive(rs_ctx* c, const rs_circuit* q) {
  std::lock_guard<std::mutex> g(c->circuits_mu);
  return q && c->circuits.count(const_cast<rs_circuit*>(q)) != 0;
}

}

int rs_circuit_create(rs_ctx* c, rs_circuit** out, const rs_cell* cells, size_t n_cells, const uint32_t* level_end, size_t n_levels,
                      size_t n_inputs) {
  int rc = circuit_ctx(c);
  if (rc) return rc;
  if (!out) return fail(RS_ERR_INVALID, "null pointer");
  *out = nullptr;
  const char* why = "";
  const rs::Cell* table = reinterpret_cast<const rs::Cell*>(cells);
  if (rs::circuit_check(table, n_cells, level_end, n_levels, n_inputs, &why) != 0) return fail(RS_ERR_INVALID, "circuit refused: %s", why);
  std::unique_ptr<rs_circuit> q(new rs_circuit);
  q->n_cells = n_cells; q->n_inputs = n_inputs;
  q->level_end.assign(level_end, level_end + n_levels);
  size_t lo = 0;
  for (size_t v = 0; v < n_levels; ++v) {
    size_t mux = 0;
    for (size_t i = lo; i < level_end[v]; ++i) mux += table[i].op == rs::kCellMux;
    q->level_mux.push_back((uint32_t)mux);
    q->widest = std::max(q->widest, level_end[v] - lo + mux);
    lo = level_end[v];
  }
  RS_HIP(hipMalloc((void**)&q->d_cells, n_cells * sizeof(rs::Cell)));
  if (hipMemcpy(q->d_cells, table, n_cells * sizeof(rs::Cell), hipMemcpyHostToDevice) != hipSuccess) {
    (void)hipGetLastError();
    (void)hipFree(q->d_cells);
    return fail(RS_ERR_HIP, "copying the cell table to the device failed");
  }
  std::lock_guard<std::mutex> g(c->circuits_mu);
  c->circuits.insert(q.get());
  *out = q.release();
  return RS_OK;
}

int rs_circuit_destroy(rs_ctx* c, rs_circuit* q) {
  int rc = circuit_ctx(c);
  if (rc) return rc;
  {
    std::lock_guard<std::mutex> g(c->circuits_mu);
    if (!q || c->circuits.erase(q) == 0) return fail(RS_ERR_INVALID, "not a live circuit of this context");
  }
  (void)hipFree(q->d_cells);
  delete q;
  return RS_OK;
}

int rs_circuit_run_dev(rs_ctx* c, const rs_circuit* q, int32_t* arena, size_t lanes, void* stream) {
  int rc = rows_ready(c);
  if (rc) return rc;
  if (!circuit_alive(c, q)) return fail(RS_ERR_INVALID, "not a live circuit of this context");
  if (lanes == 0) return RS_OK;
  if (!arena) return fail(RS_ERR_INVALID, "null arena");
  const size_t W = (size_t)c->p.n + 1;
  hipStream_t st = (hipStream_t)stream;
  Lane* ln = nullptr;
  rc = lane_of(c, st, &ln);
  if (rc) return rc;
  if (!rs::circuit_sizes_ok(q->n_inputs + q->n_cells, q->widest, lanes, W, ln->sample_words)) return fail(RS_ERR_INVALID, "circuit too large for this lane count");
  rc = ensure_rows(ln, q->widest * lanes, W);
  if (rc) return rc;
  rc = ensure_ws(ln, q->widest * lanes);
  if (rc) return rc;
  size_t lo = 0;
  for (size_t v = 0; v < q->level_end.size(); ++v) {
    const size_t cells = q->level_end[v] - lo, mux = q->level_mux[v], B = cells * lanes, R = B + mux * lanes;
    rs::CircuitLevelArgs a{};
    a.cells = q->d_cells; a.arena = arena; a.out = ln->d_rows;
    a.first = (long)lo; a.C = (long)cells; a.M = (long)mux; a.lanes = (long)lanes; a.W = (int)W;
    RS_HIP(rs::launch_circuit_rows(a, c->num_cus, st));
    const Combo x{ln->d_rows, nullptr, 1, 0, 0, nullptr};
    rc = rotate_rows(c, st, ln, &x, 1, 1 << 29, Lut{}, R);
    if (rc) return rc;
    rs::CircuitFoldArgs f{};
    f.u = ln->d_u0; f.B = (long)B; f.mux_rows = (long)(mux * lanes); f.words = (int)ln->sample_words;
    RS_HIP(rs::launch_circuit_fold(f, c->num_cus, st));
    rc = keyswitch_rows(c, st, ln, arena + (q->n_inputs + lo) * lanes * W, 1, 0, B);
    if (rc) return rc;
    rc = finish_timing(c, st, ln);
    if (rc) return rc;
    lo = q->level_end[v];
  }
  return RS_OK;
}

int rs_gather_rows_dev(rs_ctx* c, int32_t* out, const int32_t* in, const int32_t* row_index, size_t B, void* stream) {
  int rc = use_device(c);
  if (rc) return rc;
  if (B == 0) return RS_OK;
  if (!out || !in || !row_index) return fail(RS_ERR_INVALID, "null pointer");
  RS_HIP(rs::launch_gather_rows(out, in, row_index, c->p.n + 1, (long)B, (hipStream_t)stream));
  return RS_OK;
}

int rs_mux_dev(rs_ctx* c, int32_t* out, const int32_t* a, const int32_t* b, const int32_t* cc, size_t B, void* stream) {
  int rc = ready(c);
  if (rc) return rc;
  if (B == 0) return RS_OK;
  if (!out || !a || !b || !cc) return fail(RS_ERR_INVALID, "null ciphertext pointer");
  const int32_t e8 = 1 << 29;
  const Combo xs[2] = {{a, b, 1, 1, -e8, nullptr}, {a, cc, -1, 1, -e8, nullptr}};
  return run_bootstrap(c, (hipStream_t)stream, out, xs, 2, e8, e8, Lut{}, B);
}

int rs_bootstrap_wo_ks_dev(rs_ctx* c, int32_t* u, const int32_t* in, int32_t mu, size_t B, void* stream) {
  int rc = ready(c);
  if (rc) return rc;
  if (B == 0) return RS_OK;
  if (!u || !in) return fail(RS_ERR_INVALID, "null ciphertext pointer");
  const Combo x{in, nullptr, 1, 0, 0, nullptr};
  hipStream_t st = (hipStream_t)stream;
  rc = run_bootstrap(c, st, nullptr, &x, 1, 0, mu, Lut{}, B);
  if (rc) return rc;
  Lane* ln = nullptr;
  rc = lane_of(c, st, &ln);
  if (rc) return rc;
  RS_HIP(hipMemcpyAsync(u, ln->d_u0, B * ln->sample_words * sizeof(int32_t), hipMemcpyDeviceToDevice, st));
  return RS_OK;
}

int rs_keyswitch_dev(rs_ctx* c, int32_t* out, const int32_t* u, size_t B, void* stream) {
  int rc = ready(c);
  if (rc) return rc;
  if (B == 0) return RS_OK;
  if (!out || !u) return fail(RS_ERR_INVALID, "null ciphertext pointer");
  rs::KeyswitchArgs k;
  k.u0 = u; k.u1 = nullptr; k.bconst = 0; k.ksk = c->d_ksk;
  k.W = c->p.n + 1; k.t = c->p.ks_t; k.basebit = c->p.ks_basebit; k.B = (long)B; k.out = out; k.N = c->p.N;
  Lane* ln = nullptr;
  rc = lane_of(c, (hipStream_t)stream, &ln);
  if (rc) return rc;
  attach_ks_scratch(c, ln, k);
  RS_HIP(rs::launch_keyswitch(k, (hipStream_t)stream, c->num_cus, c->ks_force, &ln->last_ks));
  ln->ks_ran = true;
  return RS_OK;
}

static int host_roundtrip(rs_ctx* c, int32_t* out, const int32_t* const* ins, int n_in, size_t B,
                          int (*run)(rs_ctx*, int32_t*, int32_t* const*, size_t, void*), void* extra) {
  int rc = ready(c);
  if (rc) return rc;
  if (B == 0) return RS_OK;
  std::lock_guard<std::mutex> g(c->host_mu);
  rc = ensure_io(c, B);
  if (rc) return rc;
  const size_t bytes = B * (size_t)(c->p.n + 1) * sizeof(int32_t);
  for (int i = 0; i < n_in; ++i)
    if (!ins[i]) return fail(RS_ERR_INVALID, "null ciphertext pointer");
  for (int i = 0; i < n_in; ++i) RS_HIP(hipMemcpy(c->d_io[i], ins[i], bytes, hipMemcpyHostToDevice));
  rc = run(c, c->d_io[3], c->d_io, B, extra);
  if (rc) return rc;
  RS_HIP(hipStreamSynchronize(nullptr));
  {
    Lane* ln = nullptr;
    rc = lane_of(c, nullptr, &ln);
    if (rc) return rc;
    rc = split_check_lane(c, ln);
    if (rc) return rc;
  }
  RS_HIP(hipMemcpy(out, c->d_io[3], bytes, hipMemcpyDeviceToHost));
  return RS_OK;
}

int rs_bootstrap(rs_ctx* c, int32_t* out, const int32_t* in, int32_t mu, size_t B) {
  if (!out) return fail(RS_ERR_INVALID, "null output");
  const int32_t* ins[1] = {in};
  return host_roundtrip(c, out, ins, 1, B,
                        [](rs_ctx* cc, int32_t* o, int32_t* const* d, size_t b, void* ex) {
                          return rs_bootstrap_dev(cc, o, d[0], *(int32_t*)ex, b, nullptr);
                        }, &mu);
}

int rs_gate(rs_ctx* c, rs_gate_op op, int32_t* out, const int32_t* a, const int32_t* b, size_t B) {
  if (!out) return fail(RS_ERR_INVALID, "null output");
  const int32_t* ins[2] = {a, b};
  return host_roundtrip(c, out, ins, 2, B,
                        [](rs_ctx* cc, int32_t* o, int32_t* const* d, size_t bb, void* ex) {
                          return rs_gate_dev(cc, *(rs_gate_op*)ex, o, d[0], d[1], bb, nullptr);
                        }, &op);
}

int rs_mux(rs_ctx* c, int32_t* out, const int32_t* a, const int32_t* b, const int32_t* cc, size_t B) {
  if (!out) return fail(RS_ERR_INVALID, "null output");
  const int32_t* ins[3] = {a, b, cc};
  return host_roundtrip(c, out, ins, 3, B,
                        [](rs_ctx* c2, int32_t* o, int32_t* const* d, size_t bb, void*) {
                          return rs_mux_dev(c2, o, d[0], d[1], d[2], bb, nullptr);
                        }, nullptr);
}

int rs_debug_polymul(rs_ctx* c, int32_t* out, const int32_t* a_small, const int32_t* b_torus, size_t count) {
  int rc = use_device(c);
  if (rc) return rc;
  if (count == 0) return RS_OK;
  if (!out || !a_small || !b_torus) return fail(RS_ERR_INVALID, "null pointer");
  Lane* ln = nullptr;
  rc = lane_of(c, nullptr, &ln);
  if (rc) return rc;
  const size_t bytes = count * (size_t)c->p.N * sizeof(int32_t);
  int32_t *da = nullptr, *db = nullptr, *dout = nullptr;
  double* scratch = nullptr;
  RS_HIP(hipMalloc(&da, bytes)); RS_HIP(hipMalloc(&db, bytes)); RS_HIP(hipMalloc(&dout, bytes));
  RS_HIP(hipMalloc(&scratch, 2 * count * (size_t)c->p.N * sizeof(double)));
  RS_HIP(hipMemcpy(da, a_small, bytes, hipMemcpyHostToDevice));
  RS_HIP(hipMemcpy(db, b_torus, bytes, hipMemcpyHostToDevice));
  if (c->mode == RS_MODE_FFT_SPLIT) {
    RS_HIP(rs::launch_gen_polymul(c->logn, da, db, dout, scratch, c->d_tw_gen, (long)count, ln->d_cert + kCertSlots, c->num_cus, nullptr));
  } else {
    RS_HIP(rs::launch_polymul(c->cfg, c->mode, da, db, dout, scratch, c->mode == 1 ? c->d_tw_fft : c->d_tw, c->tables.f, c->tables.ninv,
                              (long)count, c->mode == 1 ? ln->d_cert + kCertSlots : nullptr, nullptr));
  }
  RS_HIP(hipDeviceSynchronize());
  RS_HIP(hipMemcpy(out, dout, bytes, hipMemcpyDeviceToHost));
  (void)hipFree(da); (void)hipFree(db); (void)hipFree(dout); (void)hipFree(scratch);
  return RS_OK;
}

// ... 263 lines not shown
  for (int d = 0; d < n; ++d) {
    RS_HIP(hipSetDevice(ctxs[d]->device));
    for (int e = 0; e < n; ++e) RS_HIP(hipStreamWaitEvent(nullptr, ctxs[e]->ev_copied, 0));
  }
  return RS_OK;
}
int rs_release_stream(rs_ctx* c, void* stream) {
  int rc = use_device(c);
  if (rc) return rc;
  if (!stream) return fail(RS_ERR_INVALID, "the default stream's state lives as long as the context");
  RS_HIP(hipStreamSynchronize((hipStream_t)stream));
  std::unique_ptr<Lane> ln;
  {
    std::lock_guard<std::mutex> g(c->lanes_mu);
    auto it = c->lanes.find((hipStream_t)stream);
    if (it == c->lanes.end()) return RS_OK;
    ln = std::move(it->second);
    c->lanes.erase(it);
  }
  rc = split_check_lane(c, ln.get());
  free_lane(ln.get());
  return rc;
}
int rs_sync(rs_ctx* c) {
  int rc = use_device(c);
  if (rc) return rc;
  RS_HIP(hipDeviceSynchronize());
  std::lock_guard<std::mutex> g(c->lanes_mu);
  for (auto& kv : c->lanes) {
    rc = split_check_lane(c, kv.second.get());
    if (rc) return rc;
  }
  return RS_OK;
}

int rs_set_timing(rs_ctx* c, int enable) {
  if (!c) return fail(RS_ERR_INVALID, "null context");
  c->timing = enable != 0;
  std::lock_guard<std::mutex> g(c->lanes_mu);
  for (auto& kv : c->lanes) kv.second->ev_valid = false;
  return RS_OK;
}

int rs_last_kernel_ms_stream(rs_ctx* c, void* stream, float* br_ms, float* ks_ms) {
  int rc = use_device(c);
  if (rc) return rc;
  Lane* ln = nullptr;
  rc = lane_of(c, (hipStream_t)stream, &ln);
  if (rc) return rc;
  if (!ln->ev_valid) return fail(RS_ERR_STATE, "no timed launch recorded on this stream");
  RS_HIP(hipEventSynchronize(ln->ev[2]));
  float a = -1.f, b = -1.f;
  RS_HIP(hipEventElapsedTime(&a, ln->ev[0], ln->ev[1]));
  RS_HIP(hipEventElapsedTime(&b, ln->ev[1], ln->ev[2]));
  if (br_ms) *br_ms = a;
  if (ks_ms) *ks_ms = b;
  return RS_OK;
}
int rs_last_kernel_ms(rs_ctx* c, float* br_ms, float* ks_ms) { return rs_last_kernel_ms_stream(c, nullptr, br_ms, ks_ms); }

int rs_last_launch(rs_ctx* c, void* stream, int32_t* form, int32_t* waves_per_block, int64_t* resident) {
  if (!c) return fail(RS_ERR_INVALID, "null context");
  Lane* ln = nullptr;
  int rc = lane_of(c, (hipStream_t)stream, &ln);
  if (rc) return rc;
  if (ln->last.form < 0) return fail(RS_ERR_STATE, "no blind rotation launched on this stream yet");
  if (form) *form = ln->last.form;
  if (waves_per_block) *waves_per_block = ln->last.waves_per_block;
  if (resident) *resident = ln->last.resident;
  return RS_OK;
}

int rs_last_keyswitch(rs_ctx* c, void* stream, int32_t* form, int32_t* slices) {
  if (!c) return fail(RS_ERR_INVALID, "null context");
  Lane* ln = nullptr;
  int rc = lane_of(c, (hipStream_t)stream, &ln);
  if (rc) return rc;
  if (!ln->ks_ran) return fail(RS_ERR_STATE, "no keyswitch launched on this stream yet");
  if (form) *form = ln->last_ks.form;
  if (slices) *slices = (int32_t)ln->last_ks.slices;
  return RS_OK;
}

int rs_debug_fp64_rate(rs_ctx* c, double* lane_ops_per_s) {
  if (!c || !lane_ops_per_s) return fail(RS_ERR_INVALID, "null argument");
  RS_HIP(hipSetDevice(c->device));
  double* d_out = nullptr;
  RS_HIP(hipMalloc(&d_out, (size_t)c->num_cus * 512 * sizeof(double)));
  hipEvent_t e0 = nullptr, e1 = nullptr;
  hipError_t err = hipEventCreate(&e0);
  if (err == hipSuccess) err = hipEventCreate(&e1);
  double ops = 0.0, best_ms = 1e30;
  for (int rep = 0; rep < 4 && err == hipSuccess; ++rep) {
    err = hipEventRecord(e0, nullptr);
    if (err == hipSuccess) err = rs::launch_fp64_rate(d_out, c->num_cus, 1 << 17, &ops, nullptr);
    if (err == hipSuccess) err = hipEventRecord(e1, nullptr);
    if (err == hipSuccess) err = hipEventSynchronize(e1);
    float ms = 0.f;
    if (err == hipSuccess) err = hipEventElapsedTime(&ms, e0, e1);
    if (err == hipSuccess && rep > 0 && ms < best_ms) best_ms = ms;
  }
  if (e0) (void)hipEventDestroy(e0);
  if (e1) (void)hipEventDestroy(e1);
  (void)hipFree(d_out);
  if (err != hipSuccess) return fail(RS_ERR_HIP, "rs_debug_fp64_rate: %s", hipGetErrorString(err));
  *lane_ops_per_s = ops / (best_ms * 1e-3);
  return RS_OK;
}

int rs_debug_cohort_table(rs_ctx* c, void* stream, int32_t* out) {
  if (!c || !out) return fail(RS_ERR_INVALID, "null argument");
  Lane* ln = nullptr;
  int rc = lane_of(c, (hipStream_t)stream, &ln);
  if (rc) return rc;
  if (!ln->d_progress) return fail(RS_ERR_STATE, "no lock-step launch with XCD cohorts on this stream yet");
  RS_HIP(hipStreamSynchronize(ln->stream));
  RS_HIP(hipMemcpy(out, ln->d_progress, 8 * rs::kCohortSlots * sizeof(int), hipMemcpyDeviceToHost));
  return RS_OK;
}

int rs_info(rs_ctx* c, int64_t* bk_bytes, int64_t* ksk_bytes, int32_t* wpb, int32_t* cus) {
  if (!c) return fail(RS_ERR_INVALID, "null context");
  if (bk_bytes) *bk_bytes = (int64_t)c->bk_bytes;
  if (ksk_bytes) *ksk_bytes = (int64_t)c->ksk_bytes;
  if (wpb) {
    Lane* ln = nullptr;
    *wpb = (lane_of(c, nullptr, &ln) == RS_OK && ln->last.form >= 0) ? ln->last.waves_per_block : 8;
  }
  if (cus) *cus = c->num_cus;
  return RS_OK;
}

}
```

### redsec_amd/csrc/rs_diag.h

```cpp
#pragma once

namespace rs {
namespace diag {
#ifdef RS_DIAG
constexpr int kBits = RS_DIAG;
#else
constexpr int kBits = 0;
#endif
constexpr bool kNoKeyProbe = (kBits & 16) != 0;
constexpr bool kHalfExchangeProbe = (kBits & 32) != 0;
constexpr bool kHalfExchangeSwaps = (kBits & 64) == 0;
constexpr bool kHalfKeyProbe = (kBits & 128) != 0;
constexpr bool kKsSampleProbe = (kBits & 512) != 0;
constexpr bool kWrongOnPurpose = kNoKeyProbe || kHalfExchangeProbe || kHalfKeyProbe || kKsSampleProbe;
#if defined(__HIPCC__)
__host__ __device__
#endif
constexpr int key_step(int i) { return kNoKeyProbe ? 0 : i; }
constexpr int kStampPhases = 8;
}
}

#ifdef RS_DIAG
#define RS_STAMPS_ON(bit) (((RS_DIAG) & (bit)) != 0)
#if defined(__HIPCC__)
namespace rs { extern __device__ unsigned long long g_rs_stamps[256 * 8 * diag::kStampPhases]; }
#endif
#define RS_STAMP_DECL_ unsigned long long st_sum_[rs::diag::kStampPhases] = {0, 0, 0, 0, 0, 0, 0, 0}; unsigned long long st_last_; \
  asm volatile("s_memtime %0\n\ts_waitcnt lgkmcnt(0)" : "=s"(st_last_) :: "memory")
#define RS_STAMP_(k) do { __builtin_amdgcn_sched_barrier(0); unsigned long long t_; \
  asm volatile("s_memtime %0\n\ts_waitcnt lgkmcnt(0)" : "=s"(t_) :: "memory"); __builtin_amdgcn_sched_barrier(0); \
  st_sum_[k] += t_ - st_last_; st_last_ = t_; } while (0)
#define RS_STAMP_FLUSH_(wave) do { if (lane == 0 && blockIdx.x < 256) { for (int k_ = 0; k_ < rs::diag::kStampPhases; ++k_) \
  rs::g_rs_stamps[((size_t)blockIdx.x * 8 + (wave)) * rs::diag::kStampPhases + k_] = st_sum_[k_]; } } while (0)
#else
#define RS_STAMPS_ON(bit) 0
#endif

#if RS_STAMPS_ON(1)
#define RS_STAMP_DECL RS_STAMP_DECL_
#define RS_STAMP(k) RS_STAMP_(k)
#define RS_STAMP_FLUSH(wave) RS_STAMP_FLUSH_(wave)
#else
#define RS_STAMP_DECL ((void)0)
#define RS_STAMP(k) ((void)0)
#define RS_STAMP_FLUSH(wave) ((void)0)
#endif
#if RS_STAMPS_ON(2)
#define RS_WGS_STAMP_DECL RS_STAMP_DECL_
#define RS_WGS_STAMP(k) RS_STAMP_(k)
#define RS_WGS_STAMP_FLUSH(wave) RS_STAMP_FLUSH_(wave)
#else
#define RS_WGS_STAMP_DECL ((void)0)
#define RS_WGS_STAMP(k) ((void)0)
#define RS_WGS_STAMP_FLUSH(wave) ((void)0)
#endif
#if RS_STAMPS_ON(4)
#define RS_DUO_STAMP_DECL RS_STAMP_DECL_
#define RS_DUO_STAMP(k) RS_STAMP_(k)
#define RS_DUO_STAMP_FLUSH(wave) RS_STAMP_FLUSH_(wave)
#else
#define RS_DUO_STAMP_DECL ((void)0)
#define RS_DUO_STAMP(k) ((void)0)
#define RS_DUO_STAMP_FLUSH(wave) ((void)0)
#endif
#if RS_STAMPS_ON(8)
#define RS_C8_STAMP_DECL RS_STAMP_DECL_
#define RS_C8_STAMP(k) RS_STAMP_(k)
#define RS_C8_STAMP_FLUSH(wave) RS_STAMP_FLUSH_(wave)
#else
#define RS_C8_STAMP_DECL ((void)0)
#define RS_C8_STAMP(k) ((void)0)
#define RS_C8_STAMP_FLUSH(wave) ((void)0)
#endif
#if RS_STAMPS_ON(256)
#define RS_C8L_STAMP_DECL RS_STAMP_DECL_
#define RS_C8L_STAMP(k) RS_STAMP_(k)
#define RS_C8L_STAMP_FLUSH(wave) RS_STAMP_FLUSH_(wave)
#else
#define RS_C8L_STAMP_DECL ((void)0)
#define RS_C8L_STAMP(k) ((void)0)
#define RS_C8L_STAMP_FLUSH(wave) ((void)0)
#endif
#if RS_STAMPS_ON(1 | 4 | 8) + RS_STAMPS_ON(2) + RS_STAMPS_ON(256) > 1
#error "RS_DIAG: stamp bits of one unit per build (1, 4, 8: rs_bootstrap.hip; 2: rs_bootstrap_split.hip; 256: rs_bootstrap_listed.hip)"
#endif
```

### redsec_amd/csrc/rs_emulate.cpp

```cpp
#include <algorithm>
#include <cstdint>
#include <cstring>
#include <type_traits>
#include <vector>

#include "rs_audit.h"
#include "rs_general.h"
#include "rs_host.h"
#include "rs_keygen.h"
#include "rs_pack.h"
#include "rs_packkey.h"
#include "rs_rlwe.h"
#include "rs_launch_plan.h"
#include "rs_lds_plan.h"
#include "rs_ntt.h"
#include "rs_circuit.h"
#include "rs_rows.h"
#include "rs_sparse.h"

namespace {

using rs::Field;
using rs::kLanes;
using rs::kN;
using rs::kRegs;

struct Wave {
  double x[kLanes][kRegs];
};

template <class C>
void emu_forward(Wave& w, const double* tw, double* buf, const Field& f) {
  for (int l = 0; l < kLanes; ++l) rs::fwd_F1<C>(l, w.x[l], tw, buf, f);
  for (int l = 0; l < kLanes; ++l) rs::fwd_F2<C>(l, w.x[l], tw, buf, f);
  for (int l = 0; l < kLanes; ++l) rs::fwd_F3(l, w.x[l], buf);
  for (int l = 0; l < kLanes; ++l) rs::fwd_F4<C>(l, w.x[l], tw, buf, f);
}
template <class C>
void emu_forward_digits(Wave& w, const int32_t (*d)[kRegs], int q, uint32_t offset, const double* tw, double* buf, const Field& f) {
  for (int l = 0; l < kLanes; ++l) rs::fwd_F1_digits<C>(l, w.x[l], d[l], q, offset, tw, buf, f);
  for (int l = 0; l < kLanes; ++l) rs::fwd_F2<C>(l, w.x[l], tw, buf, f);
  for (int l = 0; l < kLanes; ++l) rs::fwd_F3(l, w.x[l], buf);
  for (int l = 0; l < kLanes; ++l) rs::fwd_F4<C>(l, w.x[l], tw, buf, f);
}
template <class C>
void emu_inverse(Wave& w, const double* twi, double* buf, const Field& f) {
  for (int l = 0; l < kLanes; ++l) rs::inv_I1<C>(l, w.x[l], twi, buf, f);
  for (int l = 0; l < kLanes; ++l) rs::inv_I2<C>(l, w.x[l], twi, buf, f);
  for (int l = 0; l < kLanes; ++l) rs::inv_I3(l, w.x[l], buf);
  for (int l = 0; l < kLanes; ++l) rs::inv_I4<C>(l, w.x[l], twi, buf, f);
}

template <class C>
void emu_key_transform(const int32_t* poly, double* dst, const rs::Tables& t, double* buf) {
  Wave w;
  for (int l = 0; l < kLanes; ++l)
    for (int r = 0; r < kRegs; ++r) w.x[l][r] = (double)poly[l + 64 * r];
  emu_forward<C>(w, t.tw.data(), buf, t.f);
  for (int l = 0; l < kLanes; ++l)
    for (int v = 0; v < 8; ++v)
      for (int e = 0; e < 2; ++e) {
        double a = rs::f_reduce(rs::f_mulmod(rs::f_reduce(w.x[l][2 * v + e], t.f), t.ninv, t.f), t.f);
        dst[(v * 64 + l) * 2 + e] = a;
      }
}

template <class C>
int emu_polymul(const int32_t* a_small, const int32_t* b_torus, int32_t* out) {
  rs::PrimeSpec ps;
  if (!rs::prime_for(C::L, C::BGBIT, &ps)) return -1;
  rs::Tables t = rs::make_tables(ps, C::FUSE);
  std::vector<double> buf(rs::kBufDoubles), bkd(kN);
  emu_key_transform<C>(b_torus, bkd.data(), t, buf.data());
  Wave w;
  for (int l = 0; l < kLanes; ++l)
    for (int r = 0; r < kRegs; ++r) w.x[l][r] = (double)a_small[l + 64 * r];
  emu_forward<C>(w, t.tw.data(), buf.data(), t.f);
  for (int l = 0; l < kLanes; ++l)
    for (int u = 0; u < kRegs; ++u) w.x[l][u] = rs::f_mulmod(w.x[l][u], bkd[((u >> 1) * 64 + l) * 2 + (u & 1)], t.f);
  emu_inverse<C>(w, t.tw.data() + kN, buf.data(), t.f);
  for (int l = 0; l < kLanes; ++l)
    for (int r = 0; r < kRegs; ++r) out[l + 64 * r] = rs::f_to_torus32(w.x[l][r]);
  return 0;
}

template <class C>
int emu_blind_rotate(int n, const int32_t* in0, const int32_t* in1, int32_t c0, int32_t c1, int32_t bconst, int32_t mu,
                     const int32_t* bk, int32_t* u_out, int32_t* acc_out, int steps) {
  rs::PrimeSpec ps;
  if (!rs::prime_for(C::L, C::BGBIT, &ps)) return -1;
  rs::Tables t = rs::make_tables(ps, C::FUSE);
  const Field f = t.f;
// ... 830 lines not shown
      for (int w = 0; w < 4; ++w) m.wr(w, buf(broken == 1 ? (g & 1) : ((g + 1) & 1)) + w * 4096, 4096);
      if (broken != 2) m.barrier();
    } else {
      for (int w = 0; w < 4; ++w) m.rd(w, tab, bytes);
      for (int w = 0; w < 4; ++w) m.wr(w, base + w * 4096, 4096);
      if (broken == 1) for (int w = 0; w < 4; ++w) { m.rd(w, base, bytes); m.wr(w, tab + w * 4096, 4096); }
      m.barrier();
      if (broken != 1) for (int w = 0; w < 4; ++w) { m.rd(w, base, bytes); m.wr(w, tab + w * 4096, 4096); }
      if (broken != 2) m.barrier();
    }
  }
  return m.conflicts();
}
long rs_emu_lds_protocol_conflicts(int form, int broken) {
  switch (form) {
    case 0: return model_coop(2, broken);
    case 1: return model_coop(4, broken);
    case 4: return model_coops<2>(broken);
    case 5: return model_coops<4>(broken);
    case 6: return model_duo(10, broken);
    case 7: return model_duos(10, broken);
    case 8: return model_wgs(8, 3, broken);
    case 9: return model_wgs(4, 10, broken);
    case 10: return model_wg(3, broken);
    case 11: return model_coop8_atomics(10, broken);
    case 12: return model_coop8_atomics(3, broken);
    case 13: return model_keyswitch(false, broken);
    case 14: return model_keyswitch(true, broken);
  }
  return -1;
}
long rs_emu_coop8_row_split_violations(int L) {
  long bad = 0;
  std::vector<int> owner(2 * L, 0);
  for (int w = 0; w < rs::kCoop8Waves; ++w)
    for (int r = 0; r < rs::coop8_row_count(L, w); ++r) {
      const int q = rs::coop8_row_first(L, w) + r;
      if (q < 0 || q >= L) { ++bad; continue; }
      ++owner[rs::coop8_comp(L, w) * L + q];
    }
  for (int v : owner) bad += v != 1;
  int lo = 1 << 30, hi = 0;
  for (int s = 0; s < 4; ++s) {
    const int older = rs::coop8_row_count(L, s), younger = rs::coop8_row_count(L, s + 4);
    bad += rs::coop8_by_age(L) && younger > older;
    lo = std::min(lo, older + younger); hi = std::max(hi, older + younger);
  }
  bad += hi - lo > 1;
  bad += (rs::coop8_inv_a(L) & 3) == (rs::coop8_inv_b(L) & 3);
  for (int w = 0; w < rs::kCoop8Waves; ++w) bad += rs::coop8_row_count(L, w) < rs::coop8_row_count(L, rs::coop8_inv_a(L)) || rs::coop8_row_count(L, w) < rs::coop8_row_count(L, rs::coop8_inv_b(L));
  return bad;
}

long rs_emu_coop8_diff_cover_violations() {
  long bad = 0;
  std::vector<int> hits(2 * kN, 0);
  for (int t = 0; t < 64 * rs::kCoop8Waves; ++t)
    for (int m = 0; m < rs::kCoop8DiffPerThread; ++m) {
      const int c = rs::coop8_diff_comp(t >> 6), j = rs::coop8_diff_coeff(t, m);
      if (c < 0 || c > 1 || j < 0 || j >= kN) { ++bad; continue; }
      ++hits[c * kN + j];
    }
  for (int v : hits) bad += v != 1;
  return bad;
}

long rs_emu_ks_comb_violations(uint32_t aibar, int t, int basebit, int D) {
  long bad = 0;
  const int NG = (t + D - 1) / D, DL = t - (NG - 1) * D;
  for (int gq = 0; gq < NG; ++gq) {
    const int dl = gq == NG - 1 ? DL : D;
    const uint32_t comb = rs::ks_comb_index(aibar, gq, D, dl, basebit);
    bad += comb >= (1u << (basebit * dl));
    for (int k = 0; k < dl; ++k) bad += (uint32_t)rs::ks_comb_digit((int)comb, k, dl, basebit) != rs::ks_digit(aibar, gq * D + k, basebit);
  }
  return bad;
}
long rs_emu_keyswitch_slices(long B, int W, int N) { return (long)rs::keyswitch_slices(B, W, N); }
long rs_emu_keyswitch_scratch_words(long B, int W, int N) { return (long)rs::keyswitch_scratch_words_for(B, W, N); }
long rs_emu_keyswitch_form(long B, int W, int N, int t, int basebit, int num_cus, int force) {
  const rs::KsPlan p = rs::keyswitch_form(B, W, N, t, basebit, num_cus, force);
  return (long)p.form + 16L * (long)p.slices;
}
long rs_emu_exchange_plan(long rows, int n, const int* devices, const unsigned char* peer, int force_staged, long* out) {
  const std::vector<rs::ExchangeOp> ops = rs::exchange_plan((size_t)rows, n, devices, peer, force_staged != 0);
  if (out) for (size_t i = 0; i < ops.size(); ++i) {
    out[6 * i] = ops[i].kind; out[6 * i + 1] = ops[i].ctx; out[6 * i + 2] = ops[i].other; out[6 * i + 3] = ops[i].path;
    out[6 * i + 4] = (long)ops[i].lo; out[6 * i + 5] = (long)ops[i].hi;
  }
  return (long)ops.size();
}
long rs_emu_launch_plan(const int* traits, int n, long B, int num_cus, unsigned switches, int cohort_table_offered, long* out) {
  const rs::FormTraits t{traits[0] != 0, traits[1], traits[2] != 0, traits[3], traits[4] != 0};
  rs::LaunchOpts o;
  bool* const bits[9] = {&o.no_coop, &o.no_wg, &o.no_duo, &o.no_persist, &o.no_wg4, &o.no_tail, &o.no_coop8, &o.no_coop8_listed, &o.no_cohort};
  for (int k = 0; k < 9; ++k) *bits[k] = (switches >> k) & 1;
  const rs::LaunchPlan p = rs::plan_blind_rotate(t, n, B, num_cus, o, cohort_table_offered != 0);
  out[0] = p.info.form; out[1] = p.info.waves_per_block; out[2] = p.info.resident;
  for (int k = 0; k < p.steps; ++k) {
    const rs::LaunchStep& s = p.step[k];
    const long row[10] = {s.form, s.waves, s.grid, s.block, s.first, s.rows, s.persistent, s.cohort, s.cohort_every, s.cohort_lag};
    std::copy(row, row + 10, out + 3 + 10 * k);
  }
  return p.steps;
}
int rs_emu_gen_transform_errors(int logn, uint64_t seed, int amplitude, double* measured2, double* bounds2) {
  const double u = std::ldexp(1.0, -53), r2 = std::sqrt(2.0);
  bounds2[0] = std::pow(1.0 + 8.3 * u / r2, logn - 1) - 1.0;
  bounds2[1] = std::pow(1.0 + 5.8 * u / r2, logn - 1) - 1.0;
  switch (logn) {
    case 10: { GenEmu<10> e; e.transform_error_ratios(seed, amplitude, measured2); return 0; }
    case 11: { GenEmu<11> e; e.transform_error_ratios(seed, amplitude, measured2); return 0; }
    case 12: { GenEmu<12> e; e.transform_error_ratios(seed, amplitude, measured2); return 0; }
    case 13: { GenEmu<13> e; e.transform_error_ratios(seed, amplitude, measured2); return 0; }
  }
  return -1;
}
long rs_emu_gen_digit_mismatches(int l, int bgbit, uint32_t start, uint32_t step, long count) {
  long bad = 0;
  const uint32_t off = rs::gen_gadget_offset(l, bgbit);
  uint32_t d = start;
  for (long t = 0; t < count; ++t, d += step) {
    const int32_t dx = rs::gen_gadget_prepare((int32_t)d, off);
    for (int q = 0; q < l; ++q) {
      const int decal = 32 - (q + 1) * bgbit;
      const int32_t want = (int32_t)(((d + off) >> decal) & ((1u << bgbit) - 1u)) - (1 << (bgbit - 1));
      bad += rs::gen_gadget_digit(dx, q, bgbit) != want;
    }
  }
  return bad;
}

void rs_emu_chacha_block(const uint32_t* key8, uint32_t domain, uint64_t row, uint32_t block, uint32_t* out16) {
  uint32_t key[8], out[16];
  for (int k = 0; k < 8; ++k) key[k] = key8[k];
  rs::kg_chacha_block(key, domain, row, block, out);
  for (int k = 0; k < 16; ++k) out16[k] = out[k];
}
void rs_emu_keygen_uniforms(const uint32_t* w4, double* u1u2) {
  u1u2[0] = rs::kg_u1(w4[0], w4[1]);
  u1u2[1] = rs::kg_u2(w4[2], w4[3]);
}
int32_t rs_emu_keygen_noise(const uint32_t* w4, double sigma) { return rs::kg_noise32(w4[0], w4[1], w4[2], w4[3], sigma); }

void rs_emu_expand_bk_row(const uint8_t* mask_seed, int N, uint64_t row, const int32_t* body_row, int32_t* out) {
  uint32_t key[8];
  rs::kg_seed_words(mask_seed, key);
  const int T = N / 16;
  for (int t = 0; t < T; ++t) {
    uint32_t w[16];
    rs::kg_bk_mask_block(key, row, t, w);
    for (int k = 0; k < 16; ++k) out[16 * t + k] = (int32_t)w[k];
    for (int r = 0; r < 16; ++r) out[N + t + T * r] = body_row[t + T * r];
  }
}
void rs_emu_expand_ksk_sample(const uint8_t* mask_seed, int n, int basebit, uint64_t s, int32_t body, int32_t* out) {
  if ((s & ((1ull << basebit) - 1)) == 0) {
    for (int k = 0; k <= n; ++k) out[k] = 0;
    return;
  }
  uint32_t key[8];
  rs::kg_seed_words(mask_seed, key);
  std::vector<uint32_t> buf(rs::kKgChunk);
  for (int k0 = 0; k0 < n; k0 += rs::kKgChunk) {
    for (int lane = 0; lane < 64; ++lane) {
      uint32_t w[16] = {};
// ... 461 lines not shown
```

### redsec_amd/csrc/rs_host.h

```cpp
#pragma once

#include <cmath>
#include <cstdint>
#include <string>
#include <vector>

#include "rs_fft.h"
#include "rs_ntt.h"

namespace rs {

typedef unsigned __int128 u128_t;

struct PrimeSpec {
  uint64_t p;
  uint64_t psi;
};

inline bool prime_for(int l, int bgbit, PrimeSpec* out) {
  if (l == 3 && bgbit == 7) { *out = {1722626857492481ull, 1197309855254028ull}; return true; }
  if (l == 10 && bgbit == 3) { *out = {358880595312641ull, 57304311327783ull}; return true; }
  return false;
}

struct SliceCopy { int dst, src, round; size_t lo, hi; };
inline void slice_range(size_t total, int d, int D, size_t* lo, size_t* hi) {
  const size_t base = total / (size_t)D, rem = total % (size_t)D;
  *lo = (size_t)d * base + ((size_t)d < rem ? (size_t)d : rem);
  *hi = *lo + base + ((size_t)d < rem ? 1 : 0);
}
inline std::vector<SliceCopy> exchange_schedule(size_t rows, int n) {
  std::vector<SliceCopy> out;
  for (int d = 0; d < n; ++d)
    for (int k = 1; k < n; ++k) {
      const int e = (d + k) % n;
      SliceCopy c{d, e, k, 0, 0};
      slice_range(rows, e, n, &c.lo, &c.hi);
      if (c.hi > c.lo) out.push_back(c);
    }
  return out;
}

#ifndef RS_HD
#ifdef __HIPCC__
#define RS_HD __host__ __device__ inline
#else
#define RS_HD inline
#endif
#endif
RS_HD constexpr uint32_t ks_digit(uint32_t aibar, int j, int basebit) { return (aibar >> (32 - (j + 1) * basebit)) & ((1u << basebit) - 1u); }
RS_HD constexpr uint32_t ks_comb_index(uint32_t aibar, int gq, int D, int dl, int basebit) {
  return (aibar >> (32 - (gq * D + dl) * basebit)) & ((1u << (basebit * dl)) - 1u);
}
RS_HD constexpr int ks_comb_digit(int comb, int k, int dl, int basebit) { return (comb >> (basebit * (dl - 1 - k))) & ((1 << basebit) - 1); }

inline unsigned keyswitch_slices(long B, int W, int N) {
  if (B <= 0) return 1;
  const unsigned gx = (unsigned)((B + 255) / 256), gy = (unsigned)((W + 31) / 32);
  unsigned split = 1;
  constexpr unsigned kWantWorkgroups = 1024;
  while (split < 64 && gx * gy * split < kWantWorkgroups && N / (int)(2 * split) >= 4) split *= 2;
  return split;
}
inline size_t keyswitch_scratch_words_for(long B, int W, int N) {
  const unsigned split = keyswitch_slices(B, W, N);
  return split > 1 ? (size_t)split * (size_t)W * (size_t)B : 0;
}

enum KsForm { kKsAuto = -1, kKsGather = 0, kKsTiled = 1, kKsSliced = 2, kKsWide = 3 };
constexpr int kKsWideTile = 1024;
constexpr int kKsWideMinTilesPerCu = 1;
struct KsPlan { int form = kKsGather; unsigned slices = 1; };
inline bool ks_tiled_shape(int t, int basebit) { return (t == 8 && basebit == 2) || (t == 9 && basebit == 3) || (t == 18 && basebit == 1); }
inline bool ks_wide_shape(int t, int basebit) { return (t == 8 && basebit == 2) || (t == 9 && basebit == 3); }
inline KsPlan keyswitch_form(long B, int W, int N, int t, int basebit, int num_cus, int force = kKsAuto) {
  KsPlan p;
  if (B <= 0 || !ks_tiled_shape(t, basebit)) return p;
  if (force == kKsWide && ks_wide_shape(t, basebit)) { p.form = kKsWide; return p; }
  p.slices = keyswitch_slices(B, W, N);
  p.form = p.slices > 1 ? kKsSliced : kKsTiled;
  const long columns = (W + 31) / 32;
  if (force == kKsAuto && p.slices == 1 && ks_wide_shape(t, basebit) && (B / kKsWideTile) * columns >= (long)kKsWideMinTilesPerCu * num_cus)
    p.form = kKsWide;
  return p;
}

enum CopyPath { kPathSameDevice = 0, kPathPeer = 1, kPathHostStaged = 2 };
inline CopyPath choose_copy_path(int dst_device, int src_device, bool peer_access, bool force_staged) {
  if (force_staged) return kPathHostStaged;
  if (dst_device == src_device) return kPathSameDevice;
  return peer_access ? kPathPeer : kPathHostStaged;
}
enum { kOpWaitSlice = 0, kOpWaitCopied = 1, kOpStageOut = 2, kOpWaitStaged = 3, kOpCopy = 4, kOpRecordCopied = 5 };
struct ExchangeOp { int kind, ctx, other, path; size_t lo, hi; };
inline std::vector<ExchangeOp> exchange_plan(size_t rows, int n, const int* devices, const unsigned char* peer, bool force_staged) {
  std::vector<ExchangeOp> ops;
  const std::vector<SliceCopy> copies = exchange_schedule(rows, n);
  auto path_of = [&](const SliceCopy& c) { return choose_copy_path(devices[c.dst], devices[c.src], peer[c.dst * n + c.src] != 0, force_staged); };
  for (int s = 0; s < n; ++s) {
    bool staged = false;
    size_t lo = 0, hi = 0;
    for (const SliceCopy& c : copies) if (c.src == s && path_of(c) == kPathHostStaged) { staged = true; lo = c.lo; hi = c.hi; }
    if (!staged) continue;
    ops.push_back({kOpWaitSlice, s, s, 0, 0, 0});
    for (int e = 0; e < n; ++e) ops.push_back({kOpWaitCopied, s, e, 0, 0, 0});
    ops.push_back({kOpStageOut, s, s, kPathHostStaged, lo, hi});
  }
  for (int d = 0; d < n; ++d) {
    ops.push_back({kOpWaitSlice, d, d, 0, 0, 0});
    for (const SliceCopy& c : copies) {
      if (c.dst != d) continue;
      const CopyPath path = path_of(c);
      ops.push_back({path == kPathHostStaged ? kOpWaitStaged : kOpWaitSlice, d, c.src, 0, 0, 0});
      ops.push_back({kOpCopy, d, c.src, (int)path, c.lo, c.hi});
    }
    ops.push_back({kOpRecordCopied, d, d, 0, 0, 0});
  }
  return ops;
}

inline uint64_t mulmod_u64(uint64_t a, uint64_t b, uint64_t p) { return (uint64_t)((u128_t)a * b % p); }
inline uint64_t powmod_u64(uint64_t b, uint64_t e, uint64_t p) {
  uint64_t r = 1;
  while (e) { if (e & 1) r = mulmod_u64(r, b, p); b = mulmod_u64(b, b, p); e >>= 1; }
  return r;
}
inline double centered(uint64_t v, uint64_t p) { return v > p / 2 ? -(double)(p - v) : (double)v; }
inline uint32_t bitrev10(uint32_t x) {
  uint32_t r = 0;
  for (int i = 0; i < 10; ++i) { r = (r << 1) | (x & 1); x >>= 1; }
  return r;
}

struct Tables {
  Field f;
  std::vector<double> tw;
  double ninv;
// ... 103 lines not shown
```

### redsec_amd/csrc/rs_kernels.h

```cpp
#pragma once

#include <hip/hip_runtime.h>

#include <cstdint>

#include "rs_launch_plan.h"
#include "rs_ntt.h"
#include "rs_rows.h"

namespace rs {

struct BlindRotateArgs {
  const int32_t* in0;
  const int32_t* in1;
  int32_t c0, c1;
  int32_t bconst;
  int32_t mu;
  const double* bk_x;
  const double* tw;
  Field f;
  int32_t n;
  int32_t W;
  long B;
  int32_t* u_out;
  unsigned int* counter;
  unsigned long long* dev_flag;
  const int32_t* lut = nullptr;
  int32_t lut_count = 0;
  int32_t lut_first = 0;
  const unsigned long long* gate_flag = nullptr;
  unsigned long long gate_limit_bits = 0;
  unsigned long long* running_flag = nullptr;
  unsigned long long* fallback_count = nullptr;
  int* progress = nullptr;
  int32_t cohort_every = 0, cohort_lag = 0;
};

struct KeyswitchArgs {
  const int32_t* u0;
  const int32_t* u1;
  int32_t bconst;
  const int32_t* ksk;
  int32_t W, t, basebit;
  long B;
  int32_t* out;
  int32_t N = kN;
  uint32_t* scratch = nullptr;
  size_t scratch_words = 0;
};
size_t keyswitch_scratch_words(const KeyswitchArgs& a);

struct GenArgs {
  const int32_t* in0;
  const int32_t* in1;
  int32_t c0, c1, bconst, mu;
  const double* bk_x;
  const double* tw;
  int32_t n, W, l, bgbit;
  long B;
  int32_t* u_out;
  const int32_t* lut = nullptr;
  int32_t lut_count = 0, lut_first = 0;
  unsigned long long* dev_flag = nullptr;
};

struct ConvShape { int32_t H, Wd, Cin, Cout, fh, fw, stride_h, stride_w, off_h, off_w, Ho, Wo; };
struct PoolShape { int32_t H, Wd, C, win_h, win_w, stride_h, stride_w, off_h, off_w, Ho, Wo; };

hipError_t launch_blind_rotate(int cfg, int mode, const BlindRotateArgs& a, int num_cus, const LaunchOpts& opts, hipStream_t st,
                               LaunchInfo* info = nullptr);
hipError_t launch_blind_rotate_split_wg(int cfg, const BlindRotateArgs& a, int num_cus, const LaunchOpts& opts, hipStream_t st, LaunchInfo* info);
hipError_t launch_bk_transform(int cfg, int mode, const int32_t* bk, double* bk_x, const double* tw, Field f, double scale,
                               long n_polys, hipStream_t st);
struct KsPlan;
hipError_t launch_keyswitch(const KeyswitchArgs& a, hipStream_t st, int num_cus, int force = -1, KsPlan* ran = nullptr);
hipError_t launch_keyswitch_wide(const KeyswitchArgs& a, hipStream_t st);
hipError_t launch_gen_blind_rotate(int logn, const GenArgs& a, int num_cus, hipStream_t st);
long gen_resident_ciphertexts(int logn, int num_cus);
hipError_t launch_gen_bk_transform(int logn, const int32_t* bk, double* bk_x, const double* tw, long n_polys, int num_cus, hipStream_t st);
hipError_t launch_gen_polymul(int logn, const int32_t* a_small, const int32_t* b_torus, int32_t* out, double* scratch, const double* tw,
                              long count, unsigned long long* dev_flag, int num_cus, hipStream_t st);
struct KeygenArgs {
  int32_t* bk; int32_t* ksk;
  const int32_t* lwe_key; const int32_t* tlwe_key;
  uint32_t seed[8];
  uint32_t noise_seed[8];
  int compressed;
  int n, N, l, bgbit, t, basebit;
  double bk_sigma, ks_sigma;
  unsigned long long* dev_flag;
};
hipError_t launch_keygen_bk(int logn, const KeygenArgs& a, const double* tw, int num_cus, hipStream_t st);
hipError_t launch_keygen_ksk(const KeygenArgs& a, int num_cus, hipStream_t st);
struct ExpandArgs {
  int32_t* bk; int32_t* ksk;
  const int32_t* bk_body; const int32_t* ksk_body;
  uint32_t seed[8];
  int n, N, l, t, basebit;
};
hipError_t launch_expand_bk(int logn, const ExpandArgs& a, int num_cus, hipStream_t st);
hipError_t launch_expand_ksk(const ExpandArgs& a, int num_cus, hipStream_t st);
struct SeededArgs {
  int32_t* ct;
  int32_t* body;
  const int32_t* mu;
  const uint32_t* key_bits;
  uint32_t seed[8];
  uint32_t noise_seed[8];
  uint64_t first;
  long B;
  int n, tile;
  double sigma;
};
hipError_t launch_encrypt_seeded(const SeededArgs& a, int num_cus, hipStream_t st);
hipError_t launch_expand_ciphertexts(const SeededArgs& a, int num_cus, hipStream_t st);
struct PkArgs {
  int32_t* ct;
  const int32_t* pk;
  const int32_t* mu;
  const int32_t* base;
  uint32_t seed[8];
  uint64_t first;
  long B, m;
  int n;
};
hipError_t launch_pk_encrypt(const PkArgs& a, hipStream_t st);
struct RlweEncArgs {
  int32_t* rlwe;
  const int32_t* pk;
  const int32_t* mu;
  uint32_t seed[8];
  uint64_t first;
  long count;
  int N;
  double sigma;
};
hipError_t launch_rlwe_pk_encrypt(const RlweEncArgs& a, hipStream_t st);
struct RlweExtractArgs {
  int32_t* u;
  const int32_t* rlwe;
  long count;
  int N;
};
hipError_t launch_rlwe_extract(const RlweExtractArgs& x, hipStream_t st);
struct PackArgs {
  int32_t* rlwe;
  const int32_t* ct;
  const int32_t* key;
  long count;
  int n, N, basebit, t;
};
hipError_t launch_pack(const PackArgs& a, hipStream_t st);
struct PackKeygenArgs {
  int32_t* body;
  const uint32_t* lwe_bits; const uint32_t* tlwe_bits;
  uint32_t seed[8];
  uint32_t noise_seed[8];
  int n, N, basebit, t;
  double sigma;
// ... 69 lines not shown
```

### redsec_amd/csrc/rs_kernels.hip

```cpp
#include <hip/hip_runtime.h>

#include <cstdlib>

#include "rs_host.h"
#include "rs_kernels.h"
#include "rs_ntt.h"

namespace rs {

constexpr int KS_THREADS = 256;
constexpr int KS_MAXR = 4;

__global__ __launch_bounds__(KS_THREADS) void keyswitch_kernel(KeyswitchArgs a) {
  const long ct = blockIdx.x;
  const int tid = threadIdx.x;
  const int N = a.N, w_base = (int)blockIdx.y * KS_THREADS * KS_MAXR;
  const int32_t* u0 = a.u0 + ct * (N + 1);
  const int32_t* u1 = a.u1 ? a.u1 + ct * (N + 1) : nullptr;
  uint32_t acc[KS_MAXR];
#pragma unroll
  for (int k = 0; k < KS_MAXR; ++k) acc[k] = 0;
  const int W = a.W, t = a.t, basebit = a.basebit;
  const uint32_t prec_offset = 1u << (32 - (1 + basebit * t));
  const uint32_t mask = (1u << basebit) - 1u;
// ... 415 lines not shown
  masks[2 * i] = nz;
  masks[2 * i + 1] = ng;
}
__global__ __launch_bounds__(256) void conv_negtotal_kernel(uint32_t* __restrict__ negtotal, const uint32_t* __restrict__ masks, int K, int Cpad) {
  const int od = blockIdx.x * 256 + threadIdx.x;
  if (od >= Cpad) return;
  uint32_t n = 0;
  for (int k = 0; k < K; ++k) n += masks[2 * ((size_t)k * Cpad + od) + 1] & 1u;
  negtotal[od] = n;
}

__global__ __launch_bounds__(128) void conv_ternary_tiled_kernel(int32_t* __restrict__ out, const int32_t* __restrict__ in,
                                                                 const uint32_t* __restrict__ masks, const uint32_t* __restrict__ negtotal,
                                                                 ConvShape s, int Cpad, int W, const int32_t* __restrict__ bias_b, int bias_depth) {
  const int w = blockIdx.x * 128 + threadIdx.x;
  const int od0 = blockIdx.y * kConvTile;
  const int pix = blockIdx.z;
  const int oh = pix / s.Wo, ow = pix % s.Wo;
  const int wc = w < W ? w : W - 1;
  uint32_t acc[kConvTile];
#pragma unroll
  for (int c = 0; c < kConvTile; ++c) acc[c] = 0;
  const uint32_t* mrow = masks + 2 * (size_t)od0;
  for (int fh = 0; fh < s.fh; ++fh) {
    const int ih = fh + oh * s.stride_h - s.off_h;
    for (int fw = 0; fw < s.fw; ++fw) {
      const int iw = fw + ow * s.stride_w - s.off_w;
      const bool oob = (unsigned)ih >= (unsigned)s.H || (unsigned)iw >= (unsigned)s.Wd;
      const int32_t* src = in + (((size_t)(oob ? 0 : ih) * s.Wd + (oob ? 0 : iw)) * s.Cin) * W + wc;
      for (int di = 0; di < s.Cin; ++di) {
        const uint32_t v = oob ? 0u : (uint32_t)src[(size_t)di * W];
        const uint32_t* m = mrow + 2 * (size_t)((fh * s.fw + fw) * s.Cin + di) * Cpad;
#pragma unroll
        for (int c = 0; c < kConvTile; ++c) {
          const uint32_t t = v & m[2 * c];
          asm("v_xad_u32 %0, %1, %2, %0" : "+v"(acc[c]) : "v"(t), "s"(m[2 * c + 1]));
        }
      }
    }
  }
  if (w >= W) return;
#pragma unroll
  for (int c = 0; c < kConvTile; ++c) {
    const int od = od0 + c;
    if (od >= s.Cout) break;
    uint32_t r = acc[c] + negtotal[od];
    if (w == W - 1 && bias_b) r += (uint32_t)bias_b[od % bias_depth];
    out[(((size_t)oh * s.Wo + ow) * s.Cout + od) * W + w] = (int32_t)r;
  }
}

__global__ __launch_bounds__(256) void sumpool_kernel(int32_t* __restrict__ out, const int32_t* __restrict__ in, PoolShape s, int W,
                                                      const int32_t* __restrict__ bias_b, int bias_depth) {
  const int w = blockIdx.x * 256 + threadIdx.x;
  const int c = blockIdx.y;
  const int pix = blockIdx.z;
  if (w >= W) return;
  const int oh = pix / s.Wo, ow = pix % s.Wo;
  uint32_t acc = 0;
  for (int fh = 0; fh < s.win_h; ++fh) {
    const int ih = oh * s.stride_h - s.off_h + fh;
    if (ih < 0 || ih >= s.H) continue;
    for (int fw = 0; fw < s.win_w; ++fw) {
      const int iw = ow * s.stride_w - s.off_w + fw;
      if (iw < 0 || iw >= s.Wd) continue;
      acc += (uint32_t)in[(((size_t)ih * s.Wd + iw) * s.C + c) * W + w];
    }
  }
  if (w == W - 1 && bias_b) acc += (uint32_t)bias_b[c % bias_depth];
  out[(((size_t)oh * s.Wo + ow) * s.C + c) * W + w] = (int32_t)acc;
}

static bool ks_tiled_shape(const KeyswitchArgs& a) { return ks_tiled_shape(a.t, a.basebit); }
static_assert(KS_TILE_THREADS == 256 && KS_CH == 32, "rs_host.h keyswitch_slices() restates this grid");
static unsigned ks_slices(const KeyswitchArgs& a) {
  if (!ks_tiled_shape(a) || a.B <= 0) return 1;
  return keyswitch_slices(a.B, a.W, a.N);
}
size_t keyswitch_scratch_words(const KeyswitchArgs& a) {
  const unsigned split = ks_slices(a);
  return split > 1 ? (size_t)split * (size_t)a.W * (size_t)a.B : 0;
}

hipError_t launch_keyswitch(const KeyswitchArgs& a_in, hipStream_t st, int num_cus, int force, KsPlan* ran) {
  if (a_in.B <= 0) return hipSuccess;
  KeyswitchArgs a = a_in;
  const KsPlan plan = keyswitch_form(a.B, a.W, a.N, a.t, a.basebit, num_cus, force);
  if (ran) *ran = plan;
  if (plan.form == kKsWide) return launch_keyswitch_wide(a, st);
  dim3 grid((unsigned)((a.B + KS_TILE_THREADS - 1) / KS_TILE_THREADS), (unsigned)((a.W + KS_CH - 1) / KS_CH), 1);
  const bool tiled = plan.form != kKsGather;
  const unsigned split = plan.slices;
  grid.z = split;
  const bool two_step = split > 1 && a.scratch && a.scratch_words >= keyswitch_scratch_words(a);
  if (!two_step) a.scratch = nullptr;
  if (split > 1 && !two_step) {
    hipError_t e = hipMemsetAsync(a.out, 0, (size_t)a.B * a.W * sizeof(int32_t), st);
    if (e != hipSuccess) return e;
  }
  if (tiled && a.t == 8) {
    hipLaunchKernelGGL((keyswitch_tiled_comb_kernel<8, 2, 4, 2>), grid, dim3(KS_TILE_THREADS), 0, st, a);
  } else if (tiled && a.t == 9) {
    hipLaunchKernelGGL((keyswitch_tiled_kernel<9, 3, 2>), grid, dim3(KS_TILE_THREADS), 0, st, a);
  } else if (tiled) {
    hipLaunchKernelGGL((keyswitch_tiled_comb_kernel<18, 1, 4, 4>), grid, dim3(KS_TILE_THREADS), 0, st, a);
  } else {
    const unsigned wy = (unsigned)((a.W + KS_THREADS * KS_MAXR - 1) / (KS_THREADS * KS_MAXR));
    hipLaunchKernelGGL(keyswitch_kernel, dim3((unsigned)a.B, wy), dim3(KS_THREADS), 0, st, a);
  }
  if (hipError_t e = hipGetLastError(); e != hipSuccess) return e;
  if (two_step) {
    const dim3 rgrid((unsigned)((a.B + KS_RT - 1) / KS_RT), (unsigned)((a.W + KS_RT - 1) / KS_RT));
    hipLaunchKernelGGL(keyswitch_reduce_kernel, rgrid, dim3(KS_RT * KS_RT), 0, st, a, (int)split);
  }
  return hipGetLastError();
}

hipError_t launch_lincomb(int32_t* out, const int32_t* x, int32_t cx, const int32_t* y, int32_t cy, int32_t bconst, int W, long B,
                          hipStream_t st) {
  const long total = B * W;
  if (total <= 0) return hipSuccess;
  long blocks = (total + 255) / 256;
  if (blocks > 8192) blocks = 8192;
  hipLaunchKernelGGL(lincomb_kernel, dim3((unsigned)blocks), dim3(256), 0, st, out, x, cx, y, cy, bconst, W, total);
  return hipGetLastError();
}

hipError_t launch_synthetic_words(int32_t* out, uint64_t seed, size_t total, hipStream_t st) {
  if (total == 0) return hipSuccess;
  size_t blocks = (total + 255) / 256;
  if (blocks > 16384) blocks = 16384;
  hipLaunchKernelGGL(synthetic_words_kernel, dim3((unsigned)blocks), dim3(256), 0, st, out, seed, total);
  return hipGetLastError();
}

hipError_t launch_gather_rows(int32_t* out, const int32_t* in, const int32_t* idx, int W, long B, hipStream_t st) {
  const long total = B * W;
  if (total <= 0) return hipSuccess;
  long blocks = (total + 255) / 256;
  if (blocks > 8192) blocks = 8192;
  hipLaunchKernelGGL(gather_rows_kernel, dim3((unsigned)blocks), dim3(256), 0, st, out, in, idx, W, total);
  return hipGetLastError();
}

hipError_t launch_linear_fc(int32_t* out, const int32_t* in, const uint8_t* sign, const uint8_t* zero, int K, int M, int W,
                            int32_t zero_tap_b, const int32_t* bias_b, int bias_depth, hipStream_t st) {
  const int wblocks = (W + FC_WORDS - 1) / FC_WORDS;
  long S = (1024 + (long)wblocks * M - 1) / ((long)wblocks * M);
  const long max_s = (K + 4 * FC_KL - 1) / (4 * FC_KL);
  if (S > max_s) S = max_s;
  if (S < 1) S = 1;
  int kslice = (int)((K + S - 1) / S);
  kslice = (kslice + FC_KL - 1) / FC_KL * FC_KL;
  if (kslice < FC_KL) kslice = FC_KL;
  S = (K + kslice - 1) / kslice;
  if (S < 1) S = 1;
  if (S > 1) {
    hipError_t e = hipMemsetAsync(out, 0, sizeof(int32_t) * (size_t)M * W, st);
    if (e != hipSuccess) return e;
  }
  hipLaunchKernelGGL(linear_fc_kernel, dim3(wblocks, M, (unsigned)S), dim3(FC_WORDS * FC_KL), 0, st, out, in, sign, zero, K, M, W,
                     zero_tap_b, bias_b, bias_depth, kslice);
  return hipGetLastError();
}

hipError_t launch_conv_ternary(int32_t* out, const int32_t* in, const uint8_t* sign, const uint8_t* zero, const ConvShape& s, int W,
                               int32_t zero_tap_b, int32_t pad_tap_b, const int32_t* bias_b, int bias_depth, hipStream_t st) {
  hipLaunchKernelGGL(conv_ternary_kernel, dim3((W + 255) / 256, s.Cout, s.Ho * s.Wo), dim3(256), 0, st, out, in, sign, zero, s, W,
                     zero_tap_b, pad_tap_b, bias_b, bias_depth);
  return hipGetLastError();
}

// ... 44 lines not shown
```

### redsec_amd/csrc/rs_keyswitch_wide.hip

```cpp
#include <hip/hip_runtime.h>

#include "rs_diag.h"
#include "rs_host.h"
#include "rs_kernels.h"

namespace rs {

constexpr int KSW_CH = 32;
constexpr int KSW_CHP = KSW_CH + 4;
constexpr int KSW_THREADS = kKsWideTile;

template <int T, int BASEBIT, int KS_IG, int D, bool TWO>
__global__ __launch_bounds__(KSW_THREADS) void keyswitch_wide_kernel(KeyswitchArgs a) {
  constexpr int BASE = 1 << BASEBIT;
  constexpr int NG = (T + D - 1) / D;
  constexpr int RG = 1 << (BASEBIT * D);
  constexpr int DL = T - (NG - 1) * D;
  constexpr bool kBuild = D > 1;
  constexpr int BROWS = KS_IG * T * BASE, TROWS = KS_IG * NG * RG;
  constexpr int LEAD = kBuild ? 2 : 1;
  __shared__ __attribute__((aligned(16))) int32_t s_tab[2][TROWS * KSW_CHP];
  __shared__ __attribute__((aligned(16))) int32_t s_base[2][kBuild ? BROWS * KSW_CHP : 4];
  __shared__ __attribute__((aligned(16))) int32_t s_idle[4];
  static_assert(sizeof(int32_t) * (2 * (TROWS + (kBuild ? BROWS : 0)) * KSW_CHP + 8) <= 111 * 1024, "one workgroup per CU, <= 111 KB");
  const int tid = threadIdx.x;
  const long ct = (long)blockIdx.x * KSW_THREADS + tid;
  const bool live = ct < a.B;
  const int w0 = (int)blockIdx.y * KSW_CH;
  const int W = a.W, N = a.N;
  const int32_t* u0 = a.u0 + (live ? ct : 0) * (size_t)(N + 1);
  const int32_t* u1 = TWO ? a.u1 + (live ? ct : 0) * (size_t)(N + 1) : nullptr;
  constexpr int STAGE_WORDS = BROWS * KSW_CHP;
  int32_t* const s_stage = kBuild ? &s_base[0][0] : &s_tab[0][0];
  for (int e = tid; e < 2 * STAGE_WORDS; e += KSW_THREADS) s_stage[e] = 0;

  uint32_t acc[KSW_CH];
#pragma unroll
  for (int k = 0; k < KSW_CH; ++k) acc[k] = 0;
  constexpr uint32_t prec_offset = 1u << (32 - (1 + BASEBIT * T));
  constexpr int SEGS = KS_IG * T * (BASE - 1);
  static_assert(SEGS * 8 <= KSW_THREADS, "one 16-byte piece per thread at most");
  int32_t st[4];
  const int s_seg = tid >> 3, s_part = tid & 7;
  const int s_v = s_seg % (BASE - 1) + 1, s_ij = s_seg / (BASE - 1);
  const bool s_on = tid < SEGS * 8;
  const int s_row = ((s_on ? s_ij : 0) * BASE + s_v) * W;
  int s_off[4];
#pragma unroll
  for (int e = 0; e < 4; ++e) s_off[e] = s_row + (w0 + s_part * 4 + e < W ? w0 + s_part * 4 + e : W - 1);
  auto stage_load = [&](int i0) {
    const int32_t* src = a.ksk + (size_t)i0 * T * BASE * (size_t)W;
#pragma unroll
    for (int e = 0; e < 4; ++e) st[e] = src[s_off[e]];
  };
  int32_t* const s_dst = s_on ? &s_stage[(s_ij * BASE + s_v) * KSW_CHP + s_part * 4] : &s_idle[0];
  auto stage_store = [&](int buf) {
    *reinterpret_cast<int4*>(s_dst + (s_on ? buf * STAGE_WORDS : 0)) = make_int4(st[0], st[1], st[2], st[3]);
  };
  constexpr int NB = (TROWS * 8 + KSW_THREADS - 1) / KSW_THREADS;
  constexpr int NL = KS_IG * NG;
  static_assert(!kBuild || (TROWS * 8 % KSW_THREADS == 0 && NL % NB == 0), "the build is dealt out evenly between the lookups");
  auto build_item = [&](int buf, int item) {
    const int part = item & 7, r = item >> 3;
    const int comb = r % RG, igq = r / RG, gq = igq % NG, ii = igq / NG;
    const int dl = gq == NG - 1 ? DL : D;
    if (comb >> (BASEBIT * dl)) return;
    int4 sum = make_int4(0, 0, 0, 0);
#pragma unroll
    for (int k = 0; k < D; ++k) {
      if (k < dl) {
        const int dgt = ks_comb_digit(comb, k, dl, BASEBIT);
        const int4 v = *reinterpret_cast<const int4*>(&s_base[buf][((ii * T + gq * D + k) * BASE + dgt) * KSW_CHP + part * 4]);
        sum.x += v.x; sum.y += v.y; sum.z += v.z; sum.w += v.w;
      }
    }
    *reinterpret_cast<int4*>(&s_tab[buf][r * KSW_CHP + part * 4]) = sum;
  };

  auto load_words = [&](int g, uint32_t (&dst)[KS_IG]) {
#pragma unroll
    for (int ii = 0; ii < KS_IG; ++ii) {
      const int i = g * KS_IG + ii;
      uint32_t v = (uint32_t)u0[i];
      if (TWO) v += (uint32_t)u1[i];
      if (diag::kKsSampleProbe) v = ((uint32_t)ct * 2654435761u + (uint32_t)i * 40503u) * 2246822519u;
      dst[ii] = live ? v + prec_offset : 0u;
    }
  };

  const int G = N / KS_IG;
  uint32_t ai[KS_IG], un[KS_IG];
  load_words(0, un);
  __syncthreads();
  stage_load(0);
  stage_store(0);
  if (kBuild) {
    if (G > 1) { stage_load(KS_IG); stage_store(1); }
    __syncthreads();
#pragma unroll
    for (int h = 0; h < NB; ++h) build_item(0, tid + h * KSW_THREADS);
  }
  __syncthreads();
  for (int g = 0; g < G; ++g) {
    const int buf = g & 1;
#pragma unroll
    for (int ii = 0; ii < KS_IG; ++ii) ai[ii] = un[ii];
    load_words(g + 1 < G ? g + 1 : g, un);
    if (g + LEAD < G) stage_load((g + LEAD) * KS_IG);
    constexpr int HQ = KSW_CH / 8;
    constexpr int NS = 2 * NL;
    int4 r[2][HQ];
    auto fetch = [&](int s, int4 (&dst)[HQ]) {
      const int l = s / 2, ii = l / NG, gq = l % NG;
      const int dl = gq == NG - 1 ? DL : D;
      const uint32_t comb = ks_comb_index(ai[ii], gq, D, dl, BASEBIT);
      const int4* row = reinterpret_cast<const int4*>(&s_tab[buf][((ii * NG + gq) * RG + (int)comb) * KSW_CHP]) + (s % 2) * HQ;
#pragma unroll
      for (int q = 0; q < HQ; ++q) dst[q] = row[q];
    };
    fetch(0, r[0]);
#pragma unroll
    for (int s = 0; s < NS; ++s) {
      if (kBuild && s % (NS / NB) == 0) build_item(buf ^ 1, tid + (s / (NS / NB)) * KSW_THREADS);
      if (s + 1 < NS) fetch(s + 1, r[(s + 1) & 1]);
      const int k0 = (s % 2) * (KSW_CH / 2);
#pragma unroll
      for (int q = 0; q < HQ; ++q) {
        acc[k0 + 4 * q + 0] += (uint32_t)r[s & 1][q].x;
        acc[k0 + 4 * q + 1] += (uint32_t)r[s & 1][q].y;
        acc[k0 + 4 * q + 2] += (uint32_t)r[s & 1][q].z;
        acc[k0 + 4 * q + 3] += (uint32_t)r[s & 1][q].w;
      }
#pragma unroll
      for (int k = 0; k < KSW_CH / 2; ++k) asm volatile("" : "+v"(acc[k0 + k]));
      __builtin_amdgcn_sched_barrier(0);
    }
    if (g + LEAD < G) stage_store(kBuild ? buf : buf ^ 1);
    __syncthreads();
  }
  if (!live) return;
  uint32_t bw = (uint32_t)u0[N];
  if (TWO) bw += (uint32_t)u1[N];
  bw += (uint32_t)a.bconst;
  int32_t* out = a.out + ct * W + w0;
#pragma unroll
  for (int k = 0; k < KSW_CH; ++k) {
    const int w = w0 + k;
    if (w < W) out[k] = (int32_t)((w == W - 1 ? bw : 0u) - acc[k]);
  }
}

hipError_t launch_keyswitch_wide(const KeyswitchArgs& a, hipStream_t st) {
  if (a.B <= 0) return hipSuccess;
  if (!ks_wide_shape(a.t, a.basebit) || a.N % 4 != 0) return hipErrorNotSupported;
  const dim3 grid((unsigned)((a.B + KSW_THREADS - 1) / KSW_THREADS), (unsigned)((a.W + KSW_CH - 1) / KSW_CH), 1);
  if (a.t == 8 && !a.u1) hipLaunchKernelGGL((keyswitch_wide_kernel<8, 2, 4, 2, false>), grid, dim3(KSW_THREADS), 0, st, a);
  else if (a.t == 8) hipLaunchKernelGGL((keyswitch_wide_kernel<8, 2, 4, 2, true>), grid, dim3(KSW_THREADS), 0, st, a);
  else if (!a.u1) hipLaunchKernelGGL((keyswitch_wide_kernel<9, 3, 2, 1, false>), grid, dim3(KSW_THREADS), 0, st, a);
  else hipLaunchKernelGGL((keyswitch_wide_kernel<9, 3, 2, 1, true>), grid, dim3(KSW_THREADS), 0, st, a);
  return hipGetLastError();
}

}
```

Measured before the change: 214,300 bootstraps/s.

## Precompute keyswitch digit planes and precombined key tables for wide keyswitch

Adds a pre-pass kernel that rounds each ciphertext coefficient once and packs the decomposition digits into compact plane words in a tile-major layout. The wide keyswitch kernel then reads these planes instead of the raw u rows. At key-load time a precombined key table is also built, so the wide kernel loads ready-made combination rows rather than building them in LDS for every group. This aims to cut per-group table construction and redundant global reads, at the cost of an extra kernel launch, extra device memory for the planes and the precombined key, and more templated code paths.

```diff
diff --git a/include/redsec_hip.h b/include/redsec_hip.h
--- a/include/redsec_hip.h
+++ b/include/redsec_hip.h
@@ -155,6 +155,7 @@
 
 int rs_bootstrap_wo_ks_dev(rs_ctx* ctx, int32_t* u, const int32_t* in, int32_t mu, size_t B, void* stream);
 int rs_keyswitch_dev(rs_ctx* ctx, int32_t* out, const int32_t* u, size_t B, void* stream);
+int rs_keyswitch_sum_dev(rs_ctx* ctx, int32_t* out, const int32_t* u, const int32_t* u1, int32_t bconst, size_t B, void* stream);
 
 int rs_debug_polymul(rs_ctx* ctx, int32_t* out, const int32_t* a_small, const int32_t* b_torus, size_t count);
 int rs_debug_cohort_table(rs_ctx* ctx, void* stream, int32_t* out);
@@ -197,6 +198,7 @@
 
 int rs_last_launch(rs_ctx* ctx, void* stream, int32_t* form, int32_t* waves_per_block, int64_t* resident);
 int rs_last_keyswitch(rs_ctx* ctx, void* stream, int32_t* form, int32_t* slices);
+int rs_last_keyswitch_samples(rs_ctx* ctx, void* stream, int32_t* planes, int32_t* precombined);
 int rs_info(rs_ctx* ctx, int64_t* bk_device_bytes, int64_t* ksk_device_bytes, int32_t* waves_per_block,
             int32_t* num_cus);
 
diff --git a/redsec_amd/backend.py b/redsec_amd/backend.py
--- a/redsec_amd/backend.py
+++ b/redsec_amd/backend.py
@@ -11,10 +11,10 @@
 ABI_SYMBOLS = [
     "rs_last_error", "rs_version", "rs_params_default128", "rs_params_redsec_small_v2", "rs_create", "rs_destroy",
     "rs_load_keys", "rs_reserve", "rs_bootstrap_dev", "rs_bootstrap", "rs_gate_dev", "rs_gate", "rs_mux_dev", "rs_mux",
-    "rs_gate_mu_dev", "rs_gather_rows_dev", "rs_bootstrap_wo_ks_dev", "rs_keyswitch_dev", "rs_debug_polymul", "rs_debug_cohort_table", "rs_debug_fp64_rate", "rs_linear_fc_dev", "rs_conv_ternary_dev",
+    "rs_gate_mu_dev", "rs_gather_rows_dev", "rs_bootstrap_wo_ks_dev", "rs_keyswitch_dev", "rs_keyswitch_sum_dev", "rs_debug_polymul", "rs_debug_cohort_table", "rs_debug_fp64_rate", "rs_linear_fc_dev", "rs_conv_ternary_dev",
     "rs_sumpool_dev", "rs_lincomb_dev", "rs_dev_alloc", "rs_dev_free", "rs_copy_to_dev", "rs_copy_to_host", "rs_sync",
     "rs_set_timing", "rs_last_kernel_ms", "rs_info", "rs_set_mode", "rs_get_mode", "rs_rounding_certificate", "rs_fft_fallbacks",
-    "rs_bootstrap_lut_dev", "rs_set_certificate_limit", "rs_certify", "rs_reserve_stream", "rs_last_kernel_ms_stream", "rs_last_launch", "rs_last_keyswitch", "rs_copy_dev_to_dev",
+    "rs_bootstrap_lut_dev", "rs_set_certificate_limit", "rs_certify", "rs_reserve_stream", "rs_last_kernel_ms_stream", "rs_last_launch", "rs_last_keyswitch", "rs_last_keyswitch_samples", "rs_copy_dev_to_dev",
     "rs_params_redsec_small", "rs_params_redsec_medium", "rs_params_redsec_large", "rs_split_bound",
     "rs_allgather_rows", "rs_release_stream", "rs_load_synthetic_keys", "rs_keygen_dev", "rs_load_keys_dev",
     "rs_keygen_compressed_dev", "rs_expand_keys_dev", "rs_load_compressed_keys", "rs_load_compressed_keys_dev",
@@ -141,6 +141,7 @@
     L.rs_mux.argtypes = [vp, _i32p, _i32p, _i32p, _i32p, C.c_size_t]
     L.rs_bootstrap_wo_ks_dev.argtypes = [vp, vp, vp, C.c_int32, C.c_size_t, vp]
     L.rs_keyswitch_dev.argtypes = [vp, vp, vp, C.c_size_t, vp]
+    L.rs_keyswitch_sum_dev.argtypes = [vp, vp, vp, vp, C.c_int32, C.c_size_t, vp]
     L.rs_debug_polymul.argtypes = [vp, _i32p, _i32p, _i32p, C.c_size_t]
     L.rs_debug_cohort_table.argtypes = [vp, vp, _i32p]
     L.rs_debug_fp64_rate.argtypes = [vp, C.POINTER(C.c_double)]
@@ -170,6 +171,7 @@
     L.rs_last_kernel_ms_stream.argtypes = [vp, vp, C.POINTER(C.c_float), C.POINTER(C.c_float)]
     L.rs_last_launch.argtypes = [vp, vp, C.POINTER(C.c_int32), C.POINTER(C.c_int32), C.POINTER(C.c_int64)]
     L.rs_last_keyswitch.argtypes = [vp, vp, C.POINTER(C.c_int32), C.POINTER(C.c_int32)]
+    L.rs_last_keyswitch_samples.argtypes = [vp, vp, C.POINTER(C.c_int32), C.POINTER(C.c_int32)]
     if path is None:
         _lib = L
     return L
@@ -635,6 +637,13 @@
         _check(self.L, self.L.rs_keyswitch_dev(self.h, self._ck_dev(out), self._ck_dev(u, self.p.N + 1), B, self._stream()))
         return out
 
+    def keyswitch_sum(self, u0, u1=None, bconst=0):
+        B = u0.shape[0]
+        out = self.empty(B, self.W)
+        p1 = self._ck_dev(u1, self.p.N + 1) if u1 is not None else None
+        _check(self.L, self.L.rs_keyswitch_sum_dev(self.h, self._ck_dev(out), self._ck_dev(u0, self.p.N + 1), p1, int(bconst), B, self._stream()))
+        return out
+
     def lincomb(self, a, ca, b=None, cb=0, bconst=0):
         B = a.numel() // self.W
         out = self.empty(*a.shape)
@@ -748,6 +757,16 @@
         _check(self.L, self.L.rs_last_keyswitch(self.h, self._stream(), C.byref(f), C.byref(n)))
         return {"form": ["gather", "tiled", "sliced", "wide"][f.value], "slices": n.value}
 
+    def last_keyswitch_samples(self):
+        v = C.c_int32()
+        _check(self.L, self.L.rs_last_keyswitch_samples(self.h, self._stream(), C.byref(v), None))
+        return "planes" if v.value else "rows"
+
+    def last_keyswitch_tables(self):
+        v = C.c_int32()
+        _check(self.L, self.L.rs_last_keyswitch_samples(self.h, self._stream(), None, C.byref(v)))
+        return "precombined" if v.value else "built"
+
     def fp64_rate(self):
         v = C.c_double()
         _check(self.L, self.L.rs_debug_fp64_rate(self.h, C.byref(v)))
diff --git a/redsec_amd/build.py b/redsec_amd/build.py
--- a/redsec_amd/build.py
+++ b/redsec_amd/build.py
@@ -10,8 +10,8 @@
 HIP_LIB = os.path.join(HERE, "libredsec_hip.so")
 EMU_LIB = os.path.join(HERE, "librs_emulate.so")
 
-HIP_SOURCES = ["rs_bootstrap.hip", "rs_bootstrap_split.hip", "rs_bootstrap_listed.hip", "rs_general.hip", "rs_kernels.hip", "rs_keyswitch_wide.hip", "rs_seeded.hip", "rs_pubkey.hip", "rs_rlwe.hip", "rs_pack.hip", "rs_packkey.hip", "rs_audit.hip", "rs_rows.hip", "rs_circuit.hip", "rs_sparse.hip", "rs_api.cpp"]
-HIP_DEPS = HIP_SOURCES + ["rs_bootstrap.h", "rs_kernels.h", "rs_cohort.h", "rs_diag.h", "rs_launch_plan.h", "rs_lds_plan.h", "rs_ntt.h", "rs_fft.h", "rs_general.h", "rs_keygen.h", "rs_rlwe.h", "rs_pack.h", "rs_packkey.h", "rs_audit.h", "rs_rows.h", "rs_circuit.h", "rs_sparse.h", "rs_host.h", os.path.join(INCLUDE, "redsec_hip.h")]
+HIP_SOURCES = ["rs_bootstrap.hip", "rs_bootstrap_split.hip", "rs_bootstrap_listed.hip", "rs_general.hip", "rs_kernels.hip", "rs_keyswitch_wide.hip", "rs_keyswitch_digits.hip", "rs_seeded.hip", "rs_pubkey.hip", "rs_rlwe.hip", "rs_pack.hip", "rs_packkey.hip", "rs_audit.hip", "rs_rows.hip", "rs_circuit.hip", "rs_sparse.hip", "rs_api.cpp"]
+HIP_DEPS = HIP_SOURCES + ["rs_bootstrap.h", "rs_kernels.h", "rs_cohort.h", "rs_diag.h", "rs_launch_plan.h", "rs_lds_plan.h", "rs_ntt.h", "rs_fft.h", "rs_general.h", "rs_keygen.h", "rs_rlwe.h", "rs_pack.h", "rs_packkey.h", "rs_audit.h", "rs_rows.h", "rs_circuit.h", "rs_sparse.h", "rs_ks_planes.h", "rs_host.h", os.path.join(INCLUDE, "redsec_hip.h")]
 HIP_COMMON_FLAGS = ["-O3", "--offload-arch=gfx950", "-std=c++17", "-ffp-contract=off", "-fPIC"]
 HIP_OBJECTS = [
     ("rs_bootstrap", "rs_bootstrap.hip", ["-mllvm", "-enable-post-misched=0"]),
@@ -20,6 +20,7 @@
     ("rs_general", "rs_general.hip", []),
     ("rs_kernels", "rs_kernels.hip", []),
     ("rs_keyswitch_wide", "rs_keyswitch_wide.hip", []),
+    ("rs_keyswitch_digits", "rs_keyswitch_digits.hip", []),
     ("rs_seeded", "rs_seeded.hip", []),
     ("rs_pubkey", "rs_pubkey.hip", []),
     ("rs_rlwe", "rs_rlwe.hip", []),
@@ -32,7 +33,7 @@
     ("rs_api", "rs_api.cpp", []),
 ]
 EMU_SOURCES = ["rs_emulate.cpp"]
-EMU_DEPS = EMU_SOURCES + ["rs_launch_plan.h", "rs_lds_plan.h", "rs_ntt.h", "rs_fft.h", "rs_general.h", "rs_keygen.h", "rs_rlwe.h", "rs_pack.h", "rs_packkey.h", "rs_audit.h", "rs_rows.h", "rs_circuit.h", "rs_sparse.h", "rs_host.h"]
+EMU_DEPS = EMU_SOURCES + ["rs_launch_plan.h", "rs_lds_plan.h", "rs_ntt.h", "rs_fft.h", "rs_general.h", "rs_keygen.h", "rs_rlwe.h", "rs_pack.h", "rs_packkey.h", "rs_audit.h", "rs_rows.h", "rs_circuit.h", "rs_sparse.h", "rs_ks_planes.h", "rs_host.h"]
 
 
 def _abs(paths):
diff --git a/redsec_amd/csrc/rs_api.cpp b/redsec_amd/csrc/rs_api.cpp
--- a/redsec_amd/csrc/rs_api.cpp
+++ b/redsec_amd/csrc/rs_api.cpp
@@ -23,6 +23,7 @@
 #include "rs_general.h"
 #include "rs_kernels.h"
 #include "rs_keygen.h"
+#include "rs_ks_planes.h"
 #include "rs_pack.h"
 #include "rs_packkey.h"
 #include "rs_rlwe.h"
@@ -64,6 +65,7 @@
   size_t conv_scratch_words = 0;
   uint32_t* d_ks_scratch = nullptr;
   size_t ks_scratch_words = 0;
+  rs::KsPlanes ks_planes;
   int* d_progress = nullptr;
   int32_t* d_rows = nullptr;
   size_t rows_batch = 0;
@@ -71,6 +73,7 @@
   bool ev_valid = false;
   rs::LaunchInfo last;
   rs::KsPlan last_ks; bool ks_ran = false;
+  bool last_ks_planes = false, last_ks_pre = false;
   unsigned long long* h_split_max = nullptr;
 };
 
@@ -90,6 +93,7 @@
   double cert_limit = RS_CERTIFICATE_LIMIT;
   rs::LaunchOpts opts;
   int ks_force = rs::kKsAuto;
+  bool ks_rows = false;
   double* d_tw = nullptr;
   double* d_tw_fft = nullptr;
   double* d_bk_ntt = nullptr;
@@ -103,6 +107,8 @@
   double* d_tw_gen = nullptr;
   double* d_bk_gen = nullptr;
   int32_t* d_ksk = nullptr;
+  int32_t* d_ksk_pre = nullptr;
+  bool ks_no_pre = false;
   size_t bk_bytes = 0, ksk_bytes = 0;
   bool keys = false;
   int num_cus = 256;
@@ -153,7 +159,7 @@
   if (ln->h_split_max) (void)hipHostFree(ln->h_split_max);
   (void)hipFree(ln->d_u0); (void)hipFree(ln->d_u1); (void)hipFree(ln->d_counter); (void)hipFree(ln->d_cert);
   (void)hipFree(ln->d_conv_scratch); (void)hipFree(ln->d_ks_scratch); (void)hipFree(ln->d_progress);
-  (void)hipFree(ln->d_rows);
+  (void)hipFree(ln->d_rows); (void)hipFree(ln->ks_planes.planes); (void)hipFree(ln->ks_planes.b);
   for (auto& e : ln->ev) if (e) (void)hipEventDestroy(e);
 }
 
@@ -178,7 +184,23 @@
   return RS_OK;
 }
 
-int ensure_ws(Lane* ln, size_t B) {
+int ensure_ks_planes(const rs_ctx* c, Lane* ln, size_t B) {
+  const int W = c->p.n + 1, N = c->p.N, t = c->p.ks_t, bb = c->p.ks_basebit;
+  if (!rs::ks_wide_uses_planes(rs::keyswitch_form((long)B, W, N, t, bb, c->num_cus, c->ks_force), N, t, bb, c->ks_rows)) return RS_OK;
+  rs::KsPlanes& k = ln->ks_planes;
+  const size_t words = rs::ks_plane_words((long)B, N, t, bb);
+  if (words <= k.words && B <= k.b_words) return RS_OK;
+  if (k.planes) { (void)hipFree(k.planes); k.planes = nullptr; }
+  if (k.b) { (void)hipFree(k.b); k.b = nullptr; }
+  k.words = k.b_words = 0;
+  RS_HIP(hipMalloc(&k.planes, words * sizeof(uint2)));
+  RS_HIP(hipMalloc(&k.b, B * sizeof(int32_t)));
+  k.words = words; k.b_words = B;
+  return RS_OK;
+}
+
+int ensure_ws(const rs_ctx* c, Lane* ln, size_t B) {
+  if (int rc = ensure_ks_planes(c, ln, B)) return rc;
   if (B <= ln->ws_batch) return RS_OK;
   if (ln->d_u0) { (void)hipFree(ln->d_u0); ln->d_u0 = nullptr; }
   if (ln->d_u1) { (void)hipFree(ln->d_u1); ln->d_u1 = nullptr; }
@@ -337,8 +359,10 @@
   k.u0 = ln->d_u0; k.u1 = count == 2 ? ln->d_u1 : nullptr; k.bconst = ks_bconst; k.ksk = c->d_ksk;
   k.W = c->p.n + 1; k.t = c->p.ks_t; k.basebit = c->p.ks_basebit; k.B = (long)B; k.out = out; k.N = c->p.N;
   attach_ks_scratch(c, ln, k);
-  RS_HIP(rs::launch_keyswitch(k, st, c->num_cus, c->ks_force, &ln->last_ks));
+  ln->ks_planes.pre = c->d_ksk_pre;
+  RS_HIP(rs::launch_keyswitch(k, st, c->num_cus, c->ks_force, &ln->last_ks, c->ks_rows ? nullptr : &ln->ks_planes, &ln->last_ks_planes));
   ln->ks_ran = true;
+  ln->last_ks_pre = ln->last_ks_planes && c->d_ksk_pre != nullptr;
   return RS_OK;
 }
 
@@ -352,7 +376,7 @@
   Lane* ln = nullptr;
   int rc = lane_of(c, st, &ln);
   if (rc) return rc;
-  rc = ensure_ws(ln, B);
+  rc = ensure_ws(c, ln, B);
   if (rc) return rc;
   rc = rotate_rows(c, st, ln, combos, count, mu, lut, B);
   if (rc) return rc;
@@ -523,7 +547,11 @@
   c->opts.no_coop = env_on("RS_NO_COOP"); c->opts.no_wg = env_on("RS_NO_WG"); c->opts.no_duo = env_on("RS_NO_DUO");
   c->opts.no_persist = env_on("RS_NO_PERSIST"); c->opts.no_conv_tiled = env_on("RS_NO_CONV_TILED");
   c->opts.no_wg4 = env_on("RS_NO_WG4"); c->opts.no_tail = env_on("RS_NO_TAIL"); c->opts.no_coop8 = env_on("RS_NO_COOP8"); c->opts.no_coop8_listed = env_on("RS_NO_COOP8_LISTED"); c->opts.ks_atomics = env_on("RS_KS_ATOMICS"); c->opts.force_host_staged = env_on("RS_FORCE_HOST_STAGED"); c->opts.no_cohort = env_on("RS_NO_COHORT");
-  if (const char* v = getenv("RS_KS_FORM")) c->ks_force = strcmp(v, "wide") == 0 ? rs::kKsWide : strcmp(v, "tiled") == 0 ? rs::kKsTiled : rs::kKsAuto;
+  if (const char* v = getenv("RS_KS_FORM")) {
+    c->ks_rows = strcmp(v, "rows") == 0 || strcmp(v, "wide_rows") == 0;
+    c->ks_no_pre = strcmp(v, "build") == 0 || strcmp(v, "wide_build") == 0;
+    c->ks_force = strcmp(v, "wide") == 0 || strcmp(v, "wide_rows") == 0 || strcmp(v, "wide_build") == 0 ? rs::kKsWide : strcmp(v, "tiled") == 0 ? rs::kKsTiled : rs::kKsAuto;
+  }
   Lane* ln = nullptr;
   if (lane_of(c, nullptr, &ln) != RS_OK) { destroy_ctx(c); return RS_ERR_HIP; }
   *out = c;
@@ -552,6 +580,7 @@
   if (c->d_bk_fft) { (void)hipFree(c->d_bk_fft); c->d_bk_fft = nullptr; }
   if (c->d_bk_gen) { (void)hipFree(c->d_bk_gen); c->d_bk_gen = nullptr; }
   if (c->d_ksk) { (void)hipFree(c->d_ksk); c->d_ksk = nullptr; }
+  if (c->d_ksk_pre) { (void)hipFree(c->d_ksk_pre); c->d_ksk_pre = nullptr; }
   c->bk_bytes = c->ksk_bytes = 0;
 }
 
@@ -626,6 +655,15 @@
       if (d_body) { RS_HIP(hipFree(d_body)); d_body = nullptr; }
     }
     c->ksk_bytes = ksk_words * sizeof(int32_t);
+    if (rs::ks_pre_shape(p.ks_t, p.ks_basebit) && p.N % rs::kKsPreIg == 0 && !c->ks_no_pre && !c->ks_rows && c->ks_force != rs::kKsTiled) {
+      const size_t pre_bytes = rs::ks_pre_words(p.N, p.n + 1, p.ks_t, p.ks_basebit, rs::kKsPreD, rs::kKsPreIg) * sizeof(int32_t);
+      if (hipMalloc(&c->d_ksk_pre, pre_bytes) != hipSuccess) { (void)hipGetLastError(); c->d_ksk_pre = nullptr; }
+      else {
+        RS_HIP(rs::launch_ks_precombine(c->d_ksk_pre, c->d_ksk, p.N, p.n + 1, p.ks_t, p.ks_basebit, nullptr));
+        RS_HIP(hipDeviceSynchronize());
+        c->ksk_bytes += pre_bytes;
+      }
+    }
     return RS_OK;
   };
   rc = body();
@@ -1054,7 +1092,7 @@
   Lane* ln = nullptr;
   rc = lane_of(c, (hipStream_t)stream, &ln);
   if (rc) return rc;
-  return ensure_ws(ln, max_batch);
+  return ensure_ws(c, ln, max_batch);
 }
 
 int rs_bootstrap_dev(rs_ctx* c, int32_t* out, const int32_t* in, int32_t mu, size_t B, void* stream) {
@@ -1275,7 +1313,7 @@
   if (!rs::circuit_sizes_ok(q->n_inputs + q->n_cells, q->widest, lanes, W, ln->sample_words)) return fail(RS_ERR_INVALID, "circuit too large for this lane count");
   rc = ensure_rows(ln, q->widest * lanes, W);
   if (rc) return rc;
-  rc = ensure_ws(ln, q->widest * lanes);
+  rc = ensure_ws(c, ln, q->widest * lanes);
   if (rc) return rc;
   size_t lo = 0;
   for (size_t v = 0; v < q->level_end.size(); ++v) {
@@ -1335,19 +1373,27 @@
 }
 
 int rs_keyswitch_dev(rs_ctx* c, int32_t* out, const int32_t* u, size_t B, void* stream) {
+  return rs_keyswitch_sum_dev(c, out, u, nullptr, 0, B, stream);
+}
+
+int rs_keyswitch_sum_dev(rs_ctx* c, int32_t* out, const int32_t* u, const int32_t* u1, int32_t bconst, size_t B, void* stream) {
   int rc = ready(c);
   if (rc) return rc;
   if (B == 0) return RS_OK;
   if (!out || !u) return fail(RS_ERR_INVALID, "null ciphertext pointer");
   rs::KeyswitchArgs k;
-  k.u0 = u; k.u1 = nullptr; k.bconst = 0; k.ksk = c->d_ksk;
+  k.u0 = u; k.u1 = u1; k.bconst = bconst; k.ksk = c->d_ksk;
   k.W = c->p.n + 1; k.t = c->p.ks_t; k.basebit = c->p.ks_basebit; k.B = (long)B; k.out = out; k.N = c->p.N;
   Lane* ln = nullptr;
   rc = lane_of(c, (hipStream_t)stream, &ln);
   if (rc) return rc;
   attach_ks_scratch(c, ln, k);
-  RS_HIP(rs::launch_keyswitch(k, (hipStream_t)stream, c->num_cus, c->ks_force, &ln->last_ks));
+  rc = ensure_ks_planes(c, ln, B);
+  if (rc) return rc;
+  ln->ks_planes.pre = c->d_ksk_pre;
+  RS_HIP(rs::launch_keyswitch(k, (hipStream_t)stream, c->num_cus, c->ks_force, &ln->last_ks, c->ks_rows ? nullptr : &ln->ks_planes, &ln->last_ks_planes));
   ln->ks_ran = true;
+  ln->last_ks_pre = ln->last_ks_planes && c->d_ksk_pre != nullptr;
   return RS_OK;
 }
 
@@ -1777,6 +1823,17 @@
   return RS_OK;
 }
 
+int rs_last_keyswitch_samples(rs_ctx* c, void* stream, int32_t* planes, int32_t* precombined) {
+  if (!c) return fail(RS_ERR_INVALID, "null context");
+  Lane* ln = nullptr;
+  int rc = lane_of(c, (hipStream_t)stream, &ln);
+  if (rc) return rc;
+  if (!ln->ks_ran) return fail(RS_ERR_STATE, "no keyswitch launched on this stream yet");
+  if (planes) *planes = ln->last_ks_planes ? 1 : 0;
+  if (precombined) *precombined = ln->last_ks_pre ? 1 : 0;
+  return RS_OK;
+}
+
 int rs_debug_fp64_rate(rs_ctx* c, double* lane_ops_per_s) {
   if (!c || !lane_ops_per_s) return fail(RS_ERR_INVALID, "null argument");
   RS_HIP(hipSetDevice(c->device));
diff --git a/redsec_amd/csrc/rs_diag.h b/redsec_amd/csrc/rs_diag.h
--- a/redsec_amd/csrc/rs_diag.h
+++ b/redsec_amd/csrc/rs_diag.h
@@ -12,7 +12,8 @@
 constexpr bool kHalfExchangeSwaps = (kBits & 64) == 0;
 constexpr bool kHalfKeyProbe = (kBits & 128) != 0;
 constexpr bool kKsSampleProbe = (kBits & 512) != 0;
-constexpr bool kWrongOnPurpose = kNoKeyProbe || kHalfExchangeProbe || kHalfKeyProbe || kKsSampleProbe;
+constexpr bool kKsNoBuildProbe = (kBits & 1024) != 0;
+constexpr bool kWrongOnPurpose = kNoKeyProbe || kHalfExchangeProbe || kHalfKeyProbe || kKsSampleProbe || kKsNoBuildProbe;
 #if defined(__HIPCC__)
 __host__ __device__
 #endif
diff --git a/redsec_amd/csrc/rs_emulate.cpp b/redsec_amd/csrc/rs_emulate.cpp
--- a/redsec_amd/csrc/rs_emulate.cpp
+++ b/redsec_amd/csrc/rs_emulate.cpp
@@ -8,6 +8,7 @@
 #include "rs_general.h"
 #include "rs_host.h"
 #include "rs_keygen.h"
+#include "rs_ks_planes.h"
 #include "rs_pack.h"
 #include "rs_packkey.h"
 #include "rs_rlwe.h"
@@ -1004,6 +1005,65 @@
   const rs::KsPlan p = rs::keyswitch_form(B, W, N, t, basebit, num_cus, force);
   return (long)p.form + 16L * (long)p.slices;
 }
+long rs_emu_ks_plane_words(long B, int N, int t, int basebit) { return (long)rs::ks_plane_words(B, N, t, basebit); }
+long rs_emu_ks_plane_group(int t, int basebit) { return rs::ks_plane_group(t, basebit); }
+long rs_emu_ks_plane_slot(long ct, int g, int G) { return (long)rs::ks_plane_slot(ct, g, G); }
+void rs_emu_ks_plane_slots(long B, int N, int t, int basebit, long* out) {
+  const int G = N / rs::ks_plane_group(t, basebit);
+  const long cts = (B + rs::kKsWideTile - 1) / rs::kKsWideTile * rs::kKsWideTile;
+  for (long ct = 0; ct < cts; ++ct)
+    for (int g = 0; g < G; ++g) out[ct * G + g] = (long)rs::ks_plane_slot(ct, g, G);
+}
+long rs_emu_ks_wide_uses_planes(long B, int W, int N, int t, int basebit, int num_cus, int force, int rows) {
+  const rs::KsPlan p = rs::keyswitch_form(B, W, N, t, basebit, num_cus, force);
+  return (long)p.form + 16L * (rs::ks_wide_uses_planes(p, N, t, basebit, rows != 0) ? 1 : 0);
+}
+void rs_emu_ks_digits(const int32_t* u0, const int32_t* u1, long B, int N, int t, int basebit, uint32_t* planes, int32_t* b) {
+  rs::ks_digits_host(u0, u1, B, N, t, basebit, reinterpret_cast<rs::KsPlaneWord*>(planes), b);
+}
+void rs_emu_ks_plane_unpack(const uint32_t* planes, long B, int N, int t, int basebit, uint32_t* abar) {
+  const int kg = rs::ks_plane_group(t, basebit), G = N / kg;
+  const rs::KsPlaneWord* pl = reinterpret_cast<const rs::KsPlaneWord*>(planes);
+  for (long ct = 0; ct < B; ++ct)
+    for (int i = 0; i < N; ++i) abar[ct * N + i] = rs::ks_plane_word(pl[rs::ks_plane_slot(ct, i / kg, G)], i % kg, kg);
+}
+void rs_emu_ks_from_planes(const uint32_t* planes, const int32_t* b, int32_t bconst, const int32_t* ksk, long B, int N, int W, int t,
+                           int basebit, int32_t* out) {
+  rs::ks_from_planes_host(reinterpret_cast<const rs::KsPlaneWord*>(planes), b, bconst, ksk, B, N, W, t, basebit, out);
+}
+long rs_emu_ks_pre_words(int N, int W, int t, int basebit) { return (long)rs::ks_pre_words(N, W, t, basebit, rs::kKsPreD, rs::kKsPreIg); }
+long rs_emu_ks_pre_chunk_words(int t, int basebit) { return (long)rs::ks_pre_chunk_words(t, basebit, rs::kKsPreD, rs::kKsPreIg); }
+void rs_emu_ks_pre_table(const int32_t* ksk, int N, int W, int t, int basebit, int32_t* pre) {
+  const int columns = (W + rs::kKsPreCh - 1) / rs::kKsPreCh;
+  const size_t chunk_words = rs::ks_pre_chunk_words(t, basebit, rs::kKsPreD, rs::kKsPreIg), words = rs::ks_pre_words(N, W, t, basebit, rs::kKsPreD, rs::kKsPreIg);
+  for (size_t e = 0; e < words; ++e) {
+    const size_t chunk = e / chunk_words;
+    const int in_chunk = (int)(e % chunk_words);
+    pre[e] = rs::ks_pre_word(ksk, W, t, basebit, rs::kKsPreD, rs::kKsPreIg, (int)(chunk / columns), (int)(chunk % columns), in_chunk / rs::kKsPrePitch,
+                             in_chunk % rs::kKsPrePitch);
+  }
+}
+void rs_emu_ks_from_planes_pre(const uint32_t* planes, const int32_t* b, int32_t bconst, const int32_t* pre, long B, int N, int W, int t,
+                               int basebit, int32_t* out) {
+  const int D = rs::kKsPreD, ig = rs::kKsPreIg, NG = (t + D - 1) / D, RG = 1 << (basebit * D), DL = t - (NG - 1) * D;
+  const int kg = rs::ks_plane_group(t, basebit), G = N / kg, columns = (W + rs::kKsPreCh - 1) / rs::kKsPreCh;
+  const size_t chunk_words = rs::ks_pre_chunk_words(t, basebit, D, ig);
+  const rs::KsPlaneWord* pl = reinterpret_cast<const rs::KsPlaneWord*>(planes);
+  for (long ct = 0; ct < B; ++ct) {
+    uint32_t* o = reinterpret_cast<uint32_t*>(out + ct * (size_t)W);
+    for (int w = 0; w < W; ++w) o[w] = 0;
+    o[W - 1] = (uint32_t)b[ct] + (uint32_t)bconst;
+    for (int i = 0; i < N; ++i) {
+      const uint32_t abar = rs::ks_plane_word(pl[rs::ks_plane_slot(ct, i / kg, G)], i % kg, kg);
+      for (int gq = 0; gq < NG; ++gq) {
+        const int dl = gq == NG - 1 ? DL : D;
+        const int row = ((i % ig) * NG + gq) * RG + (int)rs::ks_comb_index(abar, gq, D, dl, basebit);
+        for (int w = 0; w < W; ++w)
+          o[w] -= (uint32_t)pre[((size_t)(i / ig) * columns + w / rs::kKsPreCh) * chunk_words + (size_t)row * rs::kKsPrePitch + w % rs::kKsPreCh];
+      }
+    }
+  }
+}
 long rs_emu_exchange_plan(long rows, int n, const int* devices, const unsigned char* peer, int force_staged, long* out) {
   const std::vector<rs::ExchangeOp> ops = rs::exchange_plan((size_t)rows, n, devices, peer, force_staged != 0);
   if (out) for (size_t i = 0; i < ops.size(); ++i) {
diff --git a/redsec_amd/csrc/rs_host.h b/redsec_amd/csrc/rs_host.h
--- a/redsec_amd/csrc/rs_host.h
+++ b/redsec_amd/csrc/rs_host.h
@@ -53,6 +53,30 @@
   return (aibar >> (32 - (gq * D + dl) * basebit)) & ((1u << (basebit * dl)) - 1u);
 }
 RS_HD constexpr int ks_comb_digit(int comb, int k, int dl, int basebit) { return (comb >> (basebit * (dl - 1 - k))) & ((1 << basebit) - 1); }
+
+constexpr int kKsPreCh = 32, kKsPrePitch = 36;
+RS_HD constexpr size_t ks_pre_chunk_words(int t, int basebit, int D, int ig) {
+  return (size_t)ig * (size_t)((t + D - 1) / D) * ((size_t)1 << (basebit * D)) * kKsPrePitch;
+}
+RS_HD constexpr size_t ks_pre_words(int N, int W, int t, int basebit, int D, int ig) {
+  return (size_t)(N / ig) * (size_t)((W + kKsPreCh - 1) / kKsPreCh) * ks_pre_chunk_words(t, basebit, D, ig);
+}
+RS_HD int32_t ks_pre_word(const int32_t* ksk, int W, int t, int basebit, int D, int ig, int g, int column, int r, int k) {
+  const int NG = (t + D - 1) / D, RG = 1 << (basebit * D), DL = t - (NG - 1) * D;
+  const int w = column * kKsPreCh + k;
+  if (k >= kKsPreCh || w >= W) return 0;
+  const int comb = r % RG, igq = r / RG, gq = igq % NG, ii = igq / NG;
+  const int dl = gq == NG - 1 ? DL : D;
+  if (comb >> (basebit * dl)) return 0;
+  uint32_t sum = 0;
+  for (int kd = 0; kd < dl; ++kd) {
+    const int dgt = ks_comb_digit(comb, kd, dl, basebit);
+    if (dgt) sum += (uint32_t)ksk[((((size_t)g * ig + ii) * t + gq * D + kd) * ((size_t)1 << basebit) + dgt) * (size_t)W + w];
+  }
+  return (int32_t)sum;
+}
+inline bool ks_pre_shape(int t, int basebit) { return t == 8 && basebit == 2; }
+constexpr int kKsPreD = 2, kKsPreIg = 4;
 
 inline unsigned keyswitch_slices(long B, int W, int N) {
   if (B <= 0) return 1;
diff --git a/redsec_amd/csrc/rs_kernels.h b/redsec_amd/csrc/rs_kernels.h
--- a/redsec_amd/csrc/rs_kernels.h
+++ b/redsec_amd/csrc/rs_kernels.h
@@ -49,6 +49,20 @@
   size_t scratch_words = 0;
 };
 size_t keyswitch_scratch_words(const KeyswitchArgs& a);
+struct KsPlanes {
+  uint2* planes = nullptr;
+  int32_t* b = nullptr;
+  size_t words = 0, b_words = 0;
+  const int32_t* pre = nullptr;
+};
+struct KsDigitsArgs {
+  const int32_t* u0;
+  const int32_t* u1;
+  uint2* planes;
+  int32_t* b;
+  long B;
+  int32_t N, t, basebit;
+};
 
 struct GenArgs {
   const int32_t* in0;
@@ -73,8 +87,11 @@
 hipError_t launch_bk_transform(int cfg, int mode, const int32_t* bk, double* bk_x, const double* tw, Field f, double scale,
                                long n_polys, hipStream_t st);
 struct KsPlan;
-hipError_t launch_keyswitch(const KeyswitchArgs& a, hipStream_t st, int num_cus, int force = -1, KsPlan* ran = nullptr);
-hipError_t launch_keyswitch_wide(const KeyswitchArgs& a, hipStream_t st);
+hipError_t launch_keyswitch(const KeyswitchArgs& a, hipStream_t st, int num_cus, int force = -1, KsPlan* ran = nullptr,
+                            const KsPlanes* planes = nullptr, bool* ran_planes = nullptr);
+hipError_t launch_keyswitch_wide(const KeyswitchArgs& a, hipStream_t st, const KsPlanes* planes = nullptr, bool* ran_planes = nullptr);
+hipError_t launch_keyswitch_digits(const KsDigitsArgs& a, hipStream_t st);
+hipError_t launch_ks_precombine(int32_t* pre, const int32_t* ksk, int N, int W, int t, int basebit, hipStream_t st);
 hipError_t launch_gen_blind_rotate(int logn, const GenArgs& a, int num_cus, hipStream_t st);
 long gen_resident_ciphertexts(int logn, int num_cus);
 hipError_t launch_gen_bk_transform(int logn, const int32_t* bk, double* bk_x, const double* tw, long n_polys, int num_cus, hipStream_t st);
diff --git a/redsec_amd/csrc/rs_kernels.hip b/redsec_amd/csrc/rs_kernels.hip
--- a/redsec_amd/csrc/rs_kernels.hip
+++ b/redsec_amd/csrc/rs_kernels.hip
@@ -521,12 +521,14 @@
   return split > 1 ? (size_t)split * (size_t)a.W * (size_t)a.B : 0;
 }
 
-hipError_t launch_keyswitch(const KeyswitchArgs& a_in, hipStream_t st, int num_cus, int force, KsPlan* ran) {
+hipError_t launch_keyswitch(const KeyswitchArgs& a_in, hipStream_t st, int num_cus, int force, KsPlan* ran, const KsPlanes* planes,
+                            bool* ran_planes) {
+  if (ran_planes) *ran_planes = false;
   if (a_in.B <= 0) return hipSuccess;
   KeyswitchArgs a = a_in;
   const KsPlan plan = keyswitch_form(a.B, a.W, a.N, a.t, a.basebit, num_cus, force);
   if (ran) *ran = plan;
-  if (plan.form == kKsWide) return launch_keyswitch_wide(a, st);
+  if (plan.form == kKsWide) return launch_keyswitch_wide(a, st, planes, ran_planes);
   dim3 grid((unsigned)((a.B + KS_TILE_THREADS - 1) / KS_TILE_THREADS), (unsigned)((a.W + KS_CH - 1) / KS_CH), 1);
   const bool tiled = plan.form != kKsGather;
   const unsigned split = plan.slices;
diff --git a/redsec_amd/csrc/rs_keyswitch_digits.hip b/redsec_amd/csrc/rs_keyswitch_digits.hip
--- /dev/null
+++ b/redsec_amd/csrc/rs_keyswitch_digits.hip
@@ -0,0 +1,72 @@
+#include <hip/hip_runtime.h>
+
+#include "rs_kernels.h"
+#include "rs_ks_planes.h"
+
+namespace rs {
+
+constexpr int KSD_CT = 64, KSD_COEF = 128, KSD_THREADS = 256;
+constexpr int KSD_PITCH = KSD_COEF + 1;
+static_assert(kKsWideTile % KSD_CT == 0, "a patch lies inside one ciphertext tile of the planes");
+
+template <int T, int BASEBIT, bool TWO>
+__global__ __launch_bounds__(KSD_THREADS) void keyswitch_digits_kernel(KsDigitsArgs a) {
+  constexpr int KG = ks_plane_group(T, BASEBIT);
+  constexpr int GP = KSD_COEF / KG;
+  static_assert(KSD_COEF % KG == 0 && (GP * KSD_CT) % KSD_THREADS == 0, "whole groups, dealt out evenly");
+  __shared__ uint32_t s_cut[KSD_CT * KSD_PITCH];
+  const int tid = threadIdx.x;
+  const long ct0 = (long)blockIdx.x * KSD_CT;
+  const int c0 = (int)blockIdx.y * KSD_COEF;
+  const int N = a.N;
+  const size_t pitch = (size_t)N + 1;
+  {
+    const int col = tid % KSD_COEF, r0 = tid / KSD_COEF;
+    constexpr int RSTEP = KSD_THREADS / KSD_COEF;
+    const size_t coef = (size_t)(c0 + col < N ? c0 + col : N - 1);
+#pragma unroll 8
+    for (int k = 0; k < KSD_CT / RSTEP; ++k) {
+      const int r = r0 + k * RSTEP;
+      const long ct = ct0 + r < a.B ? ct0 + r : a.B - 1;
+      uint32_t v = (uint32_t)a.u0[(size_t)ct * pitch + coef];
+      if (TWO) v += (uint32_t)a.u1[(size_t)ct * pitch + coef];
+      s_cut[r * KSD_PITCH + col] = ks_plane_cut(v, T, BASEBIT);
+    }
+  }
+  if (blockIdx.y == 0 && tid < KSD_CT && ct0 + tid < a.B) {
+    const long ct = ct0 + tid;
+    uint32_t bw = (uint32_t)a.u0[(size_t)ct * pitch + (size_t)N];
+    if (TWO) bw += (uint32_t)a.u1[(size_t)ct * pitch + (size_t)N];
+    a.b[ct] = (int32_t)bw;
+  }
+  __syncthreads();
+  const int lane_ct = tid % KSD_CT;
+  const long ct = ct0 + lane_ct;
+  const int G = N / KG;
+  if (ct >= a.B) return;
+  constexpr int GSTEP = KSD_THREADS / KSD_CT;
+#pragma unroll
+  for (int k = 0; k < GP / GSTEP; ++k) {
+    const int gl = tid / KSD_CT + k * GSTEP;
+    const int g = c0 / KG + gl;
+    if (g >= G) continue;
+    uint32_t d[4] = {0, 0, 0, 0};
+#pragma unroll
+    for (int ii = 0; ii < KG; ++ii) d[ii] = s_cut[lane_ct * KSD_PITCH + gl * KG + ii];
+    const KsPlaneWord w = ks_plane_pack(d, KG);
+    a.planes[ks_plane_slot(ct, g, G)] = make_uint2(w.x, w.y);
+  }
+}
+
+hipError_t launch_keyswitch_digits(const KsDigitsArgs& a, hipStream_t st) {
+  if (a.B <= 0) return hipSuccess;
+  if (!ks_wide_shape(a.t, a.basebit) || a.N % ks_plane_group(a.t, a.basebit) != 0 || !a.planes || !a.b) return hipErrorNotSupported;
+  const dim3 grid((unsigned)((a.B + KSD_CT - 1) / KSD_CT), (unsigned)((a.N + KSD_COEF - 1) / KSD_COEF), 1);
+  if (a.t == 8 && !a.u1) hipLaunchKernelGGL((keyswitch_digits_kernel<8, 2, false>), grid, dim3(KSD_THREADS), 0, st, a);
+  else if (a.t == 8) hipLaunchKernelGGL((keyswitch_digits_kernel<8, 2, true>), grid, dim3(KSD_THREADS), 0, st, a);
+  else if (!a.u1) hipLaunchKernelGGL((keyswitch_digits_kernel<9, 3, false>), grid, dim3(KSD_THREADS), 0, st, a);
+  else hipLaunchKernelGGL((keyswitch_digits_kernel<9, 3, true>), grid, dim3(KSD_THREADS), 0, st, a);
+  return hipGetLastError();
+}
+
+}
diff --git a/redsec_amd/csrc/rs_keyswitch_wide.hip b/redsec_amd/csrc/rs_keyswitch_wide.hip
--- a/redsec_amd/csrc/rs_keyswitch_wide.hip
+++ b/redsec_amd/csrc/rs_keyswitch_wide.hip
@@ -3,6 +3,7 @@
 #include "rs_diag.h"
 #include "rs_host.h"
 #include "rs_kernels.h"
+#include "rs_ks_planes.h"
 
 namespace rs {
 
@@ -10,13 +11,18 @@
 constexpr int KSW_CHP = KSW_CH + 4;
 constexpr int KSW_THREADS = kKsWideTile;
 
-template <int T, int BASEBIT, int KS_IG, int D, bool TWO>
-__global__ __launch_bounds__(KSW_THREADS) void keyswitch_wide_kernel(KeyswitchArgs a) {
+static_assert(KSW_CH == kKsPreCh && KSW_CHP == kKsPrePitch, "rs_host.h ks_pre_word() restates the rows of the LDS table");
+
+template <int T, int BASEBIT, int KS_IG, int D, bool TWO, bool PLANES, bool PRE>
+__global__ __launch_bounds__(KSW_THREADS) void keyswitch_wide_kernel(KeyswitchArgs a, const uint2* __restrict__ planes, const int32_t* __restrict__ bwords,
+                                                                      const int32_t* __restrict__ pre) {
+  static_assert(!PLANES || (KS_IG == ks_plane_group(T, BASEBIT) && !TWO), "a group of the kernel is one 8-byte word of the planes");
+  static_assert(!PRE || (D > 1 && PLANES), "pre-combined tables: shapes with combined digits, on planes");
   constexpr int BASE = 1 << BASEBIT;
   constexpr int NG = (T + D - 1) / D;
   constexpr int RG = 1 << (BASEBIT * D);
   constexpr int DL = T - (NG - 1) * D;
-  constexpr bool kBuild = D > 1;
+  constexpr bool kBuild = D > 1 && !PRE;
   constexpr int BROWS = KS_IG * T * BASE, TROWS = KS_IG * NG * RG;
   constexpr int LEAD = kBuild ? 2 : 1;
   __shared__ __attribute__((aligned(16))) int32_t s_tab[2][TROWS * KSW_CHP];
@@ -30,14 +36,16 @@
   const int W = a.W, N = a.N;
   const int32_t* u0 = a.u0 + (live ? ct : 0) * (size_t)(N + 1);
   const int32_t* u1 = TWO ? a.u1 + (live ? ct : 0) * (size_t)(N + 1) : nullptr;
+  const uint2* pl = PLANES ? planes + ks_plane_slot(ct, 0, N / KS_IG) : nullptr;
   constexpr int STAGE_WORDS = BROWS * KSW_CHP;
   int32_t* const s_stage = kBuild ? &s_base[0][0] : &s_tab[0][0];
-  for (int e = tid; e < 2 * STAGE_WORDS; e += KSW_THREADS) s_stage[e] = 0;
+  if (!PRE)
+    for (int e = tid; e < 2 * STAGE_WORDS; e += KSW_THREADS) s_stage[e] = 0;
 
   uint32_t acc[KSW_CH];
 #pragma unroll
   for (int k = 0; k < KSW_CH; ++k) acc[k] = 0;
-  constexpr uint32_t prec_offset = 1u << (32 - (1 + BASEBIT * T));
+  constexpr uint32_t prec_offset = ks_prec_offset(T, BASEBIT);
   constexpr int SEGS = KS_IG * T * (BASE - 1);
   static_assert(SEGS * 8 <= KSW_THREADS, "one 16-byte piece per thread at most");
   int32_t st[4];
@@ -65,6 +73,7 @@
     const int comb = r % RG, igq = r / RG, gq = igq % NG, ii = igq / NG;
     const int dl = gq == NG - 1 ? DL : D;
     if (comb >> (BASEBIT * dl)) return;
+    if (diag::kKsNoBuildProbe) return;
     int4 sum = make_int4(0, 0, 0, 0);
 #pragma unroll
     for (int k = 0; k < D; ++k) {
@@ -88,25 +97,61 @@
     }
   };
 
+  constexpr int CHUNK_WORDS = TROWS * KSW_CHP, PIECE_WORDS = 256, PIECES = CHUNK_WORDS / PIECE_WORDS, WAVES = KSW_THREADS / 64;
+  static_assert(!PRE || (CHUNK_WORDS % PIECE_WORDS == 0 && (size_t)CHUNK_WORDS == ks_pre_chunk_words(T, BASEBIT, D, KS_IG)), "whole pieces of the chunk rs_host.h lays out");
+  const int wave = __builtin_amdgcn_readfirstlane(tid >> 6);
+  auto pre_load = [&](int g, int buf) {
+    const int32_t* src = pre + ((size_t)g * gridDim.y + blockIdx.y) * CHUNK_WORDS + (tid & 63) * 4;
+#pragma unroll
+    for (int k = 0; k < (PIECES + WAVES - 1) / WAVES; ++k) {
+      const int piece = k * WAVES + wave;
+      if (piece < PIECES) {
+        const unsigned lds_dst = (unsigned)(size_t)(__attribute__((address_space(3))) void*)&s_tab[buf][piece * PIECE_WORDS];
+        const int32_t* gsrc = src + piece * PIECE_WORDS;
+        unsigned keep;
+        asm volatile("s_mov_b32 %0, m0\n\ts_mov_b32 m0, %2\n\ts_nop 0\n\tglobal_load_lds_dwordx4 %1, off\n\ts_mov_b32 m0, %0"
+                     : "=&s"(keep) : "v"(gsrc), "s"(lds_dst) : "memory");
+      }
+    }
+  };
   const int G = N / KS_IG;
   uint32_t ai[KS_IG], un[KS_IG];
-  load_words(0, un);
+  constexpr bool kHold = PLANES && D > 1;
+  auto plane_words = [&](int g, uint32_t (&dst)[KS_IG]) {
+    const uint2 w = pl[(size_t)g * kKsPlaneGroupStride];
+#pragma unroll
+    for (int ii = 0; ii < KS_IG; ++ii) dst[ii] = live ? ks_plane_word(KsPlaneWord{w.x, w.y}, ii, KS_IG) : 0u;
+  };
+  uint2 pw = make_uint2(0, 0);
+  if (kHold) pw = pl[0];
+  else if (PLANES) plane_words(0, un);
+  else load_words(0, un);
   __syncthreads();
-  stage_load(0);
-  stage_store(0);
+  if (PRE) pre_load(0, 0);
+  if (!PRE) {
+    stage_load(0);
+    stage_store(0);
+  }
   if (kBuild) {
     if (G > 1) { stage_load(KS_IG); stage_store(1); }
     __syncthreads();
 #pragma unroll
     for (int h = 0; h < NB; ++h) build_item(0, tid + h * KSW_THREADS);
   }
+  if (PRE) asm volatile("s_waitcnt vmcnt(0)" ::: "memory");
   __syncthreads();
   for (int g = 0; g < G; ++g) {
     const int buf = g & 1;
 #pragma unroll
-    for (int ii = 0; ii < KS_IG; ++ii) ai[ii] = un[ii];
-    load_words(g + 1 < G ? g + 1 : g, un);
-    if (g + LEAD < G) stage_load((g + LEAD) * KS_IG);
+    for (int ii = 0; ii < KS_IG; ++ii) ai[ii] = kHold ? (live ? ks_plane_word(KsPlaneWord{pw.x, pw.y}, ii, KS_IG) : 0u) : un[ii];
+    if (PRE) {
+      asm volatile("" : "+v"(ai[0]));
+      if (g + 1 < G) pre_load(g + 1, buf ^ 1);
+    }
+    if (kHold) pw = pl[(size_t)(g + 1 < G ? g + 1 : g) * kKsPlaneGroupStride];
+    else if (PLANES) plane_words(g + 1 < G ? g + 1 : g, un);
+    else load_words(g + 1 < G ? g + 1 : g, un);
+    if (!PRE && g + LEAD < G) stage_load((g + LEAD) * KS_IG);
     constexpr int HQ = KSW_CH / 8;
     constexpr int NS = 2 * NL;
     int4 r[2][HQ];
@@ -135,11 +180,12 @@
       for (int k = 0; k < KSW_CH / 2; ++k) asm volatile("" : "+v"(acc[k0 + k]));
       __builtin_amdgcn_sched_barrier(0);
     }
-    if (g + LEAD < G) stage_store(kBuild ? buf : buf ^ 1);
+    if (!PRE && g + LEAD < G) stage_store(kBuild ? buf : buf ^ 1);
+    if (PRE) asm volatile("s_waitcnt vmcnt(0)" ::: "memory");
     __syncthreads();
   }
   if (!live) return;
-  uint32_t bw = (uint32_t)u0[N];
+  uint32_t bw = PLANES ? (uint32_t)bwords[ct] : (uint32_t)u0[N];
   if (TWO) bw += (uint32_t)u1[N];
   bw += (uint32_t)a.bconst;
   int32_t* out = a.out + ct * W + w0;
@@ -150,14 +196,49 @@
   }
 }
 
-hipError_t launch_keyswitch_wide(const KeyswitchArgs& a, hipStream_t st) {
+__global__ __launch_bounds__(256) void ks_precombine_kernel(int32_t* __restrict__ pre, const int32_t* __restrict__ ksk, int W, int t, int basebit, size_t words) {
+  const size_t e = (size_t)blockIdx.x * 256 + threadIdx.x;
+  if (e >= words) return;
+  const int columns = (W + kKsPreCh - 1) / kKsPreCh;
+  const size_t chunk_words = ks_pre_chunk_words(t, basebit, kKsPreD, kKsPreIg);
+  const size_t chunk = e / chunk_words;
+  const int in_chunk = (int)(e % chunk_words);
+  pre[e] = ks_pre_word(ksk, W, t, basebit, kKsPreD, kKsPreIg, (int)(chunk / columns), (int)(chunk % columns), in_chunk / kKsPrePitch, in_chunk % kKsPrePitch);
+}
+
+hipError_t launch_ks_precombine(int32_t* pre, const int32_t* ksk, int N, int W, int t, int basebit, hipStream_t st) {
+  if (!ks_pre_shape(t, basebit) || N % kKsPreIg != 0) return hipErrorNotSupported;
+  const size_t words = ks_pre_words(N, W, t, basebit, kKsPreD, kKsPreIg);
+  hipLaunchKernelGGL(ks_precombine_kernel, dim3((unsigned)((words + 255) / 256)), dim3(256), 0, st, pre, ksk, W, t, basebit, words);
+  return hipGetLastError();
+}
+
+hipError_t launch_keyswitch_wide(const KeyswitchArgs& a, hipStream_t st, const KsPlanes* planes, bool* ran_planes) {
+  if (ran_planes) *ran_planes = false;
   if (a.B <= 0) return hipSuccess;
   if (!ks_wide_shape(a.t, a.basebit) || a.N % 4 != 0) return hipErrorNotSupported;
   const dim3 grid((unsigned)((a.B + KSW_THREADS - 1) / KSW_THREADS), (unsigned)((a.W + KSW_CH - 1) / KSW_CH), 1);
-  if (a.t == 8 && !a.u1) hipLaunchKernelGGL((keyswitch_wide_kernel<8, 2, 4, 2, false>), grid, dim3(KSW_THREADS), 0, st, a);
-  else if (a.t == 8) hipLaunchKernelGGL((keyswitch_wide_kernel<8, 2, 4, 2, true>), grid, dim3(KSW_THREADS), 0, st, a);
-  else if (!a.u1) hipLaunchKernelGGL((keyswitch_wide_kernel<9, 3, 2, 1, false>), grid, dim3(KSW_THREADS), 0, st, a);
-  else hipLaunchKernelGGL((keyswitch_wide_kernel<9, 3, 2, 1, true>), grid, dim3(KSW_THREADS), 0, st, a);
+  const int32_t* no_pre = nullptr;
+  KsPlan wide;
+  wide.form = kKsWide;
+  if (planes && planes->planes && planes->b && planes->words >= ks_plane_words(a.B, a.N, a.t, a.basebit) && planes->b_words >= (size_t)a.B &&
+      ks_wide_uses_planes(wide, a.N, a.t, a.basebit, false)) {
+    KsDigitsArgs d;
+    d.u0 = a.u0; d.u1 = a.u1; d.planes = planes->planes; d.b = planes->b; d.B = a.B; d.N = a.N; d.t = a.t; d.basebit = a.basebit;
+    if (hipError_t e = launch_keyswitch_digits(d, st); e != hipSuccess) return e;
+    const bool pre = planes->pre && ks_pre_shape(a.t, a.basebit) && a.N % kKsPreIg == 0;
+    if (pre) hipLaunchKernelGGL((keyswitch_wide_kernel<8, 2, 4, 2, false, true, true>), grid, dim3(KSW_THREADS), 0, st, a, planes->planes, planes->b, planes->pre);
+    else if (a.t == 8) hipLaunchKernelGGL((keyswitch_wide_kernel<8, 2, 4, 2, false, true, false>), grid, dim3(KSW_THREADS), 0, st, a, planes->planes, planes->b, no_pre);
+    else hipLaunchKernelGGL((keyswitch_wide_kernel<9, 3, 2, 1, false, true, false>), grid, dim3(KSW_THREADS), 0, st, a, planes->planes, planes->b, no_pre);
+    if (ran_planes) *ran_planes = true;
+    return hipGetLastError();
+  }
+  const uint2* none = nullptr;
+  const int32_t* no_b = nullptr;
+  if (a.t == 8 && !a.u1) hipLaunchKernelGGL((keyswitch_wide_kernel<8, 2, 4, 2, false, false, false>), grid, dim3(KSW_THREADS), 0, st, a, none, no_b, no_pre);
+  else if (a.t == 8) hipLaunchKernelGGL((keyswitch_wide_kernel<8, 2, 4, 2, true, false, false>), grid, dim3(KSW_THREADS), 0, st, a, none, no_b, no_pre);
+  else if (!a.u1) hipLaunchKernelGGL((keyswitch_wide_kernel<9, 3, 2, 1, false, false, false>), grid, dim3(KSW_THREADS), 0, st, a, none, no_b, no_pre);
+  else hipLaunchKernelGGL((keyswitch_wide_kernel<9, 3, 2, 1, true, false, false>), grid, dim3(KSW_THREADS), 0, st, a, none, no_b, no_pre);
   return hipGetLastError();
 }
 
diff --git a/redsec_amd/csrc/rs_ks_planes.h b/redsec_amd/csrc/rs_ks_planes.h
--- /dev/null
+++ b/redsec_amd/csrc/rs_ks_planes.h
@@ -0,0 +1,67 @@
+#pragma once
+
+#include <cstddef>
+#include <cstdint>
+
+#include "rs_host.h"
+
+namespace rs {
+
+struct KsPlaneWord { uint32_t x, y; };
+
+RS_HD constexpr int ks_plane_group(int t, int basebit) { return t * basebit <= 16 ? 4 : 2; }
+RS_HD constexpr uint32_t ks_prec_offset(int t, int basebit) { return 1u << (32 - (1 + basebit * t)); }
+RS_HD constexpr uint32_t ks_plane_cut(uint32_t u, int t, int basebit) {
+  return (u + ks_prec_offset(t, basebit)) & ~((1u << (32 - basebit * t)) - 1u);
+}
+RS_HD constexpr KsPlaneWord ks_plane_pack(const uint32_t* d, int kg) {
+  return kg == 4 ? KsPlaneWord{(d[0] >> 16) | (d[1] & 0xFFFF0000u), (d[2] >> 16) | (d[3] & 0xFFFF0000u)} : KsPlaneWord{d[0], d[1]};
+}
+RS_HD constexpr uint32_t ks_plane_word(KsPlaneWord w, int ii, int kg) {
+  return kg == 4 ? ((ii & 1) ? ((ii & 2) ? w.y : w.x) & 0xFFFF0000u : ((ii & 2) ? w.y : w.x) << 16) : (ii ? w.y : w.x);
+}
+constexpr size_t kKsPlaneGroupStride = kKsWideTile;
+RS_HD constexpr size_t ks_plane_slot(long ct, int g, int G) {
+  return ((size_t)(ct / kKsWideTile) * (size_t)G + (size_t)g) * kKsPlaneGroupStride + (size_t)(ct % kKsWideTile);
+}
+RS_HD constexpr size_t ks_plane_words(long B, int N, int t, int basebit) {
+  return B <= 0 ? 0 : (size_t)((B + kKsWideTile - 1) / kKsWideTile) * (size_t)(N / ks_plane_group(t, basebit)) * kKsPlaneGroupStride;
+}
+
+inline bool ks_wide_uses_planes(const KsPlan& p, int N, int t, int basebit, bool rows) {
+  return p.form == kKsWide && !rows && ks_wide_shape(t, basebit) && N % ks_plane_group(t, basebit) == 0;
+}
+
+inline void ks_digits_host(const int32_t* u0, const int32_t* u1, long B, int N, int t, int basebit, KsPlaneWord* planes, int32_t* b) {
+  const int kg = ks_plane_group(t, basebit), G = N / kg;
+  for (long ct = 0; ct < B; ++ct) {
+    const int32_t* r0 = u0 + ct * (size_t)(N + 1);
+    const int32_t* r1 = u1 ? u1 + ct * (size_t)(N + 1) : nullptr;
+    for (int g = 0; g < G; ++g) {
+      uint32_t d[4] = {0, 0, 0, 0};
+      for (int ii = 0; ii < kg; ++ii) d[ii] = ks_plane_cut((uint32_t)r0[g * kg + ii] + (r1 ? (uint32_t)r1[g * kg + ii] : 0u), t, basebit);
+      planes[ks_plane_slot(ct, g, G)] = ks_plane_pack(d, kg);
+    }
+    b[ct] = (int32_t)((uint32_t)r0[N] + (r1 ? (uint32_t)r1[N] : 0u));
+  }
+}
+inline void ks_from_planes_host(const KsPlaneWord* planes, const int32_t* b, int32_t bconst, const int32_t* ksk, long B, int N, int W,
+                                int t, int basebit, int32_t* out) {
+  const int kg = ks_plane_group(t, basebit), G = N / kg, base = 1 << basebit;
+  for (long ct = 0; ct < B; ++ct) {
+    uint32_t* o = reinterpret_cast<uint32_t*>(out + ct * (size_t)W);
+    for (int w = 0; w < W; ++w) o[w] = 0;
+    o[W - 1] = (uint32_t)b[ct] + (uint32_t)bconst;
+    for (int i = 0; i < N; ++i) {
+      const uint32_t abar = ks_plane_word(planes[ks_plane_slot(ct, i / kg, G)], i % kg, kg);
+      for (int j = 0; j < t; ++j) {
+        const uint32_t v = ks_digit(abar, j, basebit);
+        if (v == 0) continue;
+        const int32_t* row = ksk + (((size_t)i * t + j) * base + v) * (size_t)W;
+        for (int w = 0; w < W; ++w) o[w] -= (uint32_t)row[w];
+      }
+    }
+  }
+}
+
+}
```

Measured after the change: 215,400 bootstraps/s (median of 6 runs). No clear change (+0.5%).
